# mx-mark/VideoTransformer-pytorch

Measured on AMD Instinct MI355X. Metric: clips/sec TimeSformer-B divided_space_time 8x3x224x224 fwd+bwd (whole job), higher is better.
Workload: dtype bf16

## Files before the change

__graft_entry__.py:

```python
import os
import subprocess
import sys

ROOT = os.path.dirname(os.path.abspath(__file__))
PKG = os.path.join(ROOT, 'videotransformer-pytorch_amd')
for p in (ROOT, PKG):
    if p not in sys.path:
        sys.path.insert(0, p)


def _build_oracle_c():
    src = os.path.join(ROOT, 'oracle', 'hog_ref.c')
    out_dir = os.path.join(ROOT, 'oracle', '_build')
    os.makedirs(out_dir, exist_ok=True)
    so = os.path.join(out_dir, 'libhogref.so')
    if not os.path.exists(so) or os.path.getmtime(so) < os.path.getmtime(src):
        subprocess.run(['gcc', '-O2', '-ffp-contract=off', '-shared', '-fPIC', '-o', so, src, '-lm'], check=True)
    return so


def ensure_built():
    so = os.path.join(PKG, 'libvtx.so')
    hipcc = os.environ.get('HIPCC', '/opt/rocm/bin/hipcc')
    if os.path.exists(so) and not os.path.exists(hipcc):
        return so
    sys.path.insert(0, os.path.join(PKG, 'csrc'))
    import build as vtx_build
    return vtx_build.build(verbose=False)


def build():
    sys.path.insert(0, os.path.join(PKG, 'csrc'))
    import build as vtx_build
    vtx_build.build(force=False, verbose=True)
    _build_oracle_c()
    import vtx
    lib = vtx.load()
    assert lib.vtx_version() >= 100
    import transformer, video_transformer
    print('libvtx', lib.vtx_version(), 'symbols bound:', len(vtx._lib.SIGNATURES))
    assert vtx._lib.load_ragged().vtx_ragged_version() >= 100
    print('libvtx_ragged', vtx._lib.load_ragged().vtx_ragged_version(), 'symbols bound:', len(vtx._lib.RAGGED_SIGNATURES))
    assert vtx._lib.load_dropout().vtx_dropout_version() >= 100
    print('libvtx_dropout', vtx._lib.load_dropout().vtx_dropout_version(), 'symbols bound:', len(vtx._lib.DROPOUT_SIGNATURES))


def smoke():
    import ctypes
    import numpy as np
    import torch
    ensure_built()
    import vtx
    import video_transformer as V
    from oracle import synth, vt_oracle as O, hog_oracle as H
    assert torch.cuda.is_available(), 'smoke() needs a GPU'
    buf = ctypes.create_string_buffer(16384)
    fails = vtx.load().vtx_selftest(buf, len(buf))
    print(buf.value.decode())
    assert fails == 0, 'instruction layout self-test failed'
    dev = torch.device('cuda:0')
    cfg = dict(num_frames=4, img_size=64, patch_size=16, embed_dims=128, num_heads=2, num_transformer_layers=2)
    m = V.TimeSformer(**cfg)
    sd = synth.synth_state_dict(synth.shapes_of(m), 3)
    m.load_state_dict(sd)
    m.to(dev).train()
    x = synth.synth_clip(2, 4, 3, 64, 64, seed=2)
    sdo = {k: v.clone().requires_grad_(True) for k, v in sd.items()}
    torch.manual_seed(1)
    yo = O.timesformer_forward(sdo, x, 4, heads=2, layers=2, training=True)
    yo.sum().backward()
    for prec, tol, gtol in (('fp32', 1e-3, 1e-3), ('bf16', 1.5e-2, 2e-2), ('bf16 + exact stream', 1.5e-2, 2e-2)):
        vtx.set_precision(prec.split()[0])
        vtx.set_stream('fp32+grad' if 'exact' in prec else 'bf16')
        m.zero_grad()
        torch.manual_seed(1)
        y = m(x.to(dev))
        y.sum().backward()
        torch.cuda.synchronize()
        e = (y.cpu() - yo.detach()).abs().max().item() / yo.abs().max().item()
        g = m.transformer_layers.layers[1].attentions[0].temporal_fc.weight.grad.cpu()
        go = sdo['transformer_layers.layers.1.attentions.0.temporal_fc.weight'].grad
        eg = (g - go).abs().max().item() / go.abs().max().item()
        print(f'smoke {prec}: out rel err {e:.2e}, temporal_fc grad rel err {eg:.2e}')
        assert e < tol and eg < gtol, (prec, e, eg)
    vtx.set_precision('auto')
    vtx.set_stream('bf16')
    frame = np.random.RandomState(5).randint(0, 256, (1, 224, 224, 3)).astype(np.uint8)
    f = vtx.ops.hog_fwd(torch.from_numpy(frame).to(dev)).cpu().numpy()[0]
    assert np.array_equal(f, H.extract_hog_features(frame[0])), 'HOG not bit-exact'
    rs = np.random.RandomState(6)
    clips = [torch.from_numpy(rs.randint(0, 256, shp).astype(np.uint8)).to(dev) for shp in ((5, 40, 56, 3), (3, 56, 40, 3))]
    ev, fr = vtx.aug.ClipEval(img_size=32), [[4, 0], [2, 1]]
    both = ev(clips, frames=fr)
    assert both.shape == (2, 2, 32, 32, 3) and all(torch.equal(both[b], ev(clips[b][None], frames=[fr[b]])[0]) for b in range(2)), 'ragged views differ'
    print('smoke ok')


if __name__ == '__main__':
    build()
    if len(sys.argv) > 1 and sys.argv[1] == 'smoke':
        smoke()
```

include/vtx.h:

```cpp
#ifndef VTX_H_
#define VTX_H_

#include <stddef.h>
#include <stdint.h>

#ifdef __cplusplus
extern "C" {
#endif

#define VTX_OK 0
#define VTX_EINVAL (-1)
#define VTX_EALIGN (-2)
#define VTX_ELAUNCH (-3)
#define VTX_EWS (-4)

#define VTX_F32 0
#define VTX_BF16 1
#define VTX_BF16_X32 3

typedef struct {
  int grp;
  int skip;
  int base;
  const int* tab;
} vtx_rowmap;

int vtx_version(void);
const char* vtx_last_error_string(void);
int vtx_set_option(const char* name, const char* value);

int vtx_layernorm_fwd(int dtype, int rows, int D, const void* x, long ldx, vtx_rowmap xmap,
                      const float* gamma, const float* beta, float eps,
                      void* y, long ldy, vtx_rowmap ymap, float* mean, float* rstd, void* stream);
int vtx_layernorm_acc_fwd(int rows, int D, const float* xs, const void* d, long lds, vtx_rowmap smap, float* xo, long ldo,
                          vtx_rowmap omap, const float* gamma, const float* beta, float eps, void* y, long ldy, vtx_rowmap ymap,
                          float* mean, float* rstd, void* stream);
size_t vtx_layernorm_bwd_workspace(int rows, int D);
int vtx_layernorm_bwd(int dtype, int rows, int D, const void* dy, long lddy, vtx_rowmap dymap,
                      const void* x, long ldx, vtx_rowmap xmap, const float* mean, const float* rstd,
                      const float* gamma, const void* dres, void* dx, long lddx,
                      float* dgamma, float* dbeta, void* workspace, size_t ws_bytes, void* stream);
int vtx_layernorm_bwd_g32(int rows, int D, const void* dy, long lddy, vtx_rowmap dymap, const float* x, long ldx, vtx_rowmap xmap,
                          const float* mean, const float* rstd, const float* gamma, const float* dres32, float* dx32,
                          void* dx, long lddx, float* dgamma, float* dbeta, void* workspace, size_t ws_bytes, void* stream);

typedef struct {
  int dtype;
  int M, N, K;
  const void* A; long lda; vtx_rowmap amap;
  const void* B; long ldb;
  void* C; long ldc; vtx_rowmap cmap;
  const float* bias;
  int act;
  void* C2; long ldc2;
  const void* dgelu_in; long ld_dgelu;
  int dgelu_kind;
  const float* row_scale;
  int rs_d1, rs_m1, rs_d2, rs_m2;
  const void* R; long ldr; vtx_rowmap rmap; int r_period;
  int split_row; void* Csplit; long ldsplit;
  void* workspace; size_t ws_bytes;
} vtx_gemm_desc;
size_t vtx_gemm_nt_workspace(void);
int vtx_gemm_nt(const vtx_gemm_desc* d, void* stream);

typedef struct {
  int dtype;
  int M, N1, N2;
  const void* A; long lda; vtx_rowmap amap;
  const void* B; long ldb; vtx_rowmap bmap;
  float* C; long ldc; int accumulate;
  void* workspace; size_t ws_bytes;
  float* colsum; int colsum_accumulate;
} vtx_gemm_tn_desc;
size_t vtx_gemm_tn_workspace(int M, int N1, int N2);
int vtx_gemm_tn(const vtx_gemm_tn_desc* d, void* stream);

typedef struct {
  int N1, N2, K;
  const float* A; long a_rs, a_ks;
  const float* B; long b_ks, b_cs;
  float alpha;
  float* C; long ldc; int accumulate;
  const float* u; const float* v;
  const float* x; float* y;
  float alpha_y; const float* z; float beta_z; int y_accumulate;
} vtx_wprod_desc;
int vtx_wprod(const vtx_wprod_desc* d, void* stream);

size_t vtx_colsum_workspace(int M, int N);
int vtx_colsum(int dtype, int M, int N, const void* A, long lda, vtx_rowmap amap,
               float* out, int accumulate, void* workspace, size_t ws_bytes, void* stream);

#define VTX_ATTN_CONTIG 0
#define VTX_ATTN_SPACE 1
#define VTX_ATTN_TIME_CLS 2
#define VTX_ATTN_SPACE_NOCLS 3
typedef struct {
  int dtype, mode;
  int S, L, H, hd;
  int B, T, P;
  const void* qkv; long ld_qkv;
  void* out; long ld_out;
  float* lse;
  float* probs;
  float scale;
} vtx_attn_desc;
int vtx_attn_fwd(const vtx_attn_desc* d, void* stream);

typedef struct {
  vtx_attn_desc f;
  const void* dout; long ld_dout;
  void* dqkv; long ld_dqkv;
  void* dqkv_cls;
  float* delta;
} vtx_attn_bwd_desc;
int vtx_attn_bwd(const vtx_attn_bwd_desc* d, void* stream);

int vtx_cls_mean_fwd(int dtype, int B, int T, int D, const void* a_cls, long lda,
                     const void* x, void* out, long ld_tok, long rows_per_clip, void* stream);
int vtx_fact_glue_fwd(int dtype, int B, int T, int P, int D, const void* x, const float* time_embed, void* h, void* stream);
int vtx_fact_glue_bwd(int dtype, int B, int T, int P, int D, const void* dh, void* dx, float* d_time_embed, int accumulate,
                      void* stream);
int vtx_space_grad_prep(int dtype, int B, int T, int P, int D, const void* dout, long ld,
                        const float* s, void* da, long ldda, void* stream);
int vtx_cls_qkv_reduce(int dtype, int B, int T, int W, const void* dqkv_cls, long ldc,
                       void* dqkv, long ld, long rows_per_clip, void* stream);
int vtx_row_scale_copy(int dtype, int rows, int D, const void* src, long lds, vtx_rowmap smap,
                       void* dst, long ldd, vtx_rowmap dmap, const float* s,
                       int rs_d1, int rs_m1, int rs_d2, int rs_m2, void* stream);
int vtx_dropped_rows_fix(int dtype, long M, int D, int group_rows, const float* s, const void* x, long ldx,
                         vtx_rowmap xmap, const float* bias, void* out, long ldo, vtx_rowmap omap, void* zero,
                         long ldz, void* stream);
int vtx_dropped_rows_colsum(int dtype, long M, int D, int group_rows, const float* s, const void* src, long lds,
                            vtx_rowmap smap, float* part, int nparts, void* stream);
int vtx_reduce_rows(int in_dtype, int nj, int ni, int D, const void* in, long ld, long base,
                    long si, long sj, float* out, long ldo, float scale, int accumulate, void* stream);
int vtx_gelu_grad_mul(int dtype, size_t n, const void* dy, const void* h, void* out, void* stream);
int vtx_cast_transpose(int dtype, int R, int C, const float* W, void* Wc, void* WcT, void* stream);
typedef struct {
  const float* src;
  void* dst_c;
  void* dst_t;
  int rows, cols;
} vtx_ct_tensor;
int vtx_mt_cast_transpose(int dtype, const vtx_ct_tensor* tab, const int* tile_start, int n_tensors, int n_tiles, void* stream);
int vtx_cast_from_f32(int dtype, size_t n, const float* src, void* dst, void* stream);
int vtx_cast_to_f32(int dtype, size_t n, const void* src, float* dst, void* stream);

int vtx_patch_rows(int dtype, int B, int T, int C, int H, int W, int ps, int ts,
                   const float* clip, void* rows, long ldr, int frame_major, void* stream);
int vtx_patch_rows_u8(int dtype, int B, int T, int H, int W, int ps, int ts,
                      const unsigned char* clip, const float* host_mean3, const float* host_std3,
                      void* rows, long ldr, int frame_major, void* stream);
int vtx_embed_table(int dtype, int P, int T, int D, const float* bias, const float* pos,
                    const float* time_embed, const float* cls, void* E, void* cls_row,
                    int frame_major, void* stream);

size_t vtx_hog_table_bytes(void);
int vtx_hog_build_table(double* host_table);
int vtx_hog_fwd(const uint8_t* frames, int F, int H, int W, const double* table, size_t table_bytes,
                double* out, int32_t* bins, void* stream);

int vtx_maskfeat_blend_fwd(int dtype, int B, int Tq, int Hq, int Wq, int C, int g,
                           const void* x, const uint8_t* mask, const float* mask_token,
                           void* out, void* stream);
int vtx_maskfeat_blend_bwd(int dtype, int B, int Tq, int Hq, int Wq, int C, int g,
                           const void* dy, const uint8_t* mask, void* dx, float* dtoken,
                           void* stream);
int vtx_maskfeat_loss_fwd(int dtype, int B, int Tq, int ts, int g, int Cf, const void* pred, long ldp,
                          const double* target, const uint8_t* cmask, double* loss_out, void* stream);
int vtx_maskfeat_loss_bwd(int dtype, int B, int Tq, int ts, int g, int Cf, const void* pred, long ldp,
                          const double* target, const uint8_t* cmask, const double* loss_out,
                          float gloss, void* dpred, long lddp, void* stream);

typedef struct { int dtype, B, T, H, W, heads, hd, sh, sw; } vtx_pool_desc;
int vtx_pool_conv_ln_fwd(const vtx_pool_desc* d, const void* x, const float* w, const float* gamma, const float* beta,
                         float eps, void* pre, void* y, float* mean, float* rstd, void* stream);
size_t vtx_pool_conv_ln_bwd_workspace(const vtx_pool_desc* d);
int vtx_pool_conv_ln_bwd(const vtx_pool_desc* d, const void* dy, const void* x, const void* pre, const float* mean,
                         const float* rstd, const float* w, const float* gamma, void* dpre, void* dx, float* dw,
                         float* dgamma, float* dbeta, void* workspace, size_t ws_bytes, void* stream);
int vtx_maxpool_skip_fwd(int dtype, int B, int T, int H, int W, int C, const void* x, void* y, uint8_t* arg, void* stream);
int vtx_maxpool_skip_bwd(int dtype, int B, int T, int H, int W, int C, const void* dy, const uint8_t* arg, void* dx, void* stream);
int vtx_pos_encoding_fwd(int dtype, int B, int T, int HW, int C, const void* x, const float* cls, const float* pos_class,
                         const float* spatial, const float* temporal, void* out, void* stream);
int vtx_im2col3d(int dtype, int B, int T, int C, int H, int W, const int* k3, const int* s3, const int* p3, int Kp,
                 const float* clip, void* rows, void* stream);
typedef struct {
  int dtype, B, Lq, Lk, heads, hd;
  float scale;
  const void* q; const void* k; const void* v;
  void* out; float* lse;
} vtx_xattn_desc;
int vtx_xattn_fwd(const vtx_xattn_desc* d, void* stream);
size_t vtx_xattn_bwd_workspace(const vtx_xattn_desc* d);
int vtx_xattn_bwd(const vtx_xattn_desc* d, const void* dout, float* delta, void* dq, void* dk, void* dv, void* workspace,
                  size_t ws_bytes, void* stream);

int vtx_mixup_batch(float* x, int B, long per_clip, float lam, float one_minus_lam, void* stream);
int vtx_cutmix_batch(float* x, int B, int planes, int H, int W, int yl, int yh, int xl, int xh, void* stream);
int vtx_mixup_target(const long* labels, int B, int C, float on_value, float off_value, float lam, float one_minus_lam,
                     float* out, void* stream);
int vtx_softmax_xent_fwd(const float* logits, const float* soft_targets, const long* labels, int B, int C, float* loss_rows,
                         float* lse, float* loss_mean, void* stream);
int vtx_softmax_xent_bwd(const float* logits, const float* soft_targets, const long* labels, const float* lse, int B, int C,
                         float grad_scale, const float* grad_loss, const float* count, float* dlogits, void* stream);
int vtx_topk_correct(const float* scores, const long* labels, int B, int C, int k, int* correct, void* stream);

typedef struct {
  void* p;
  const void* g;
  void* s1;
  void* s2;
  long n;
  float lr, wd;
} vtx_mt_tensor;
int vtx_mt_chunks(long numel);
int vtx_mt_grad_norms(const vtx_mt_tensor* tab, const int* chunk_start, int n_tensors, int n_chunks,
                      float* partial, float* norms, void* stream);
int vtx_mt_sgd_step(const vtx_mt_tensor* tab, const int* chunk_start, int n_tensors, int n_chunks, const float* norms,
                    float clip, float momentum, int nesterov, int first_step, void* stream);
int vtx_mt_adamw_step(const vtx_mt_tensor* tab, const int* chunk_start, int n_tensors, int n_chunks, const float* norms,
                      float clip, float beta1, float beta2, float eps, int step, void* stream);


int vtx_selftest(char* report, size_t report_bytes);

#ifdef __cplusplus
}
#endif
#endif
```

videotransformer-pytorch_amd/csrc/api.hip:

```cpp
#include <limits.h>
#include <stdarg.h>
#include <stdlib.h>
#include <string.h>
#include <string>
#include <vector>
#include "common.h"

namespace vtx {

static thread_local char g_err[512] = "";

void set_error(const char* fmt, ...) {
  va_list ap;
  va_start(ap, fmt);
  vsnprintf(g_err, sizeof(g_err), fmt, ap);
  va_end(ap);
}

int check_launch(const char* what) {
  hipError_t e = hipGetLastError();
  if (e != hipSuccess) {
    set_error("%s: launch failed: %s", what, hipGetErrorString(e));
    return VTX_ELAUNCH;
  }
  return VTX_OK;
}

static const char* const kNtNames[] = {"auto", "pp256", "dma2", "ring128x3", "ring128x4k32", "ring256x3", "ring256x3k32", "ring256x4k32"};
static const char* const kAttnF32Names[] = {"valu", "mfma"};
static const char* const kTnNames[] = {"auto", "pp256", "ring", "dma2", "w4"};

enum OptKind { OPT_FLAG, OPT_INT, OPT_CLAMP, OPT_ENUM, OPT_ADDR };
struct OptRow { const char* id[2]; OptKind kind; int Options::*field; int lo, hi, mult; const char* const* names; };
#define VTX_ENUM(names) 0, (int)(sizeof(names) / sizeof(*names)) - 1, 1, names
static const OptRow kOptions[] = {
    {{"VTX_GEMM_NT", "gemm_nt"}, OPT_ENUM, &Options::gemm_nt, VTX_ENUM(kNtNames)},
    {{"VTX_GEMM_TN", "gemm_tn"}, OPT_ENUM, &Options::gemm_tn, VTX_ENUM(kTnNames)},
    {{"VTX_GEMM_NODMA", "gemm_nodma"}, OPT_FLAG, &Options::gemm_nodma},
    {{"VTX_TN_SAFE", "tn_safe"}, OPT_FLAG, &Options::tn_safe},
    {{"VTX_TN_CUS", "tn_cus"}, OPT_INT, &Options::tn_cus, 32, 1024, 1},
    {{"VTX_ATTN_VALU", "attn_valu"}, OPT_FLAG, &Options::attn_valu},
    {{"VTX_ATTN_LONG", "attn_long"}, OPT_FLAG, &Options::attn_long},
    {{"VTX_ATTN_F32", "attn_f32"}, OPT_ENUM, &Options::attn_f32, VTX_ENUM(kAttnF32Names)},
    {{"VTX_ATTN_HW_FWD", "attn_hw_fwd"}, OPT_INT, &Options::attn_hw_fwd, 0, INT_MAX, 1},
    {{"VTX_ATTN_HW_BWD", "attn_hw_bwd"}, OPT_INT, &Options::attn_hw_bwd, 0, INT_MAX, 1},
    {{"VTX_ATTN_FUSED", "attn_fused"}, OPT_CLAMP, &Options::attn_fused, 0, 2},
    {{"VTX_ATTN_FWD_STREAM", "attn_fwd_stream"}, OPT_FLAG, &Options::attn_fwd_stream},
    {{"VTX_ATTN_DKV", "attn_dkv"}, OPT_INT, &Options::attn_dkv, 0, 4, 1},
    {{"VTX_GEMM_PP_GRID", "pp_grid"}, OPT_INT, &Options::pp_grid, 8, 4096, 8},
    {{"VTX_GEMM_PP_CG", "pp_cg"}, OPT_INT, &Options::pp_cg, 0, INT_MAX, 1},
    {{"VTX_GEMM_PP_EPI", "pp_epi"}, OPT_INT, &Options::pp_epi, INT_MIN, INT_MAX, 1},
    {{"VTX_GEMM_PP_CONT", "pp_cont"}, OPT_FLAG, &Options::pp_cont},
    {{"VTX_LN_ROWS", "ln_rows"}, OPT_INT, &Options::ln_rows, 1, 4, 1},
    {{nullptr, "pp_trace"}, OPT_ADDR, nullptr}};
#undef VTX_ENUM

static int set_option(Options& o, const char* name, const char* value) {
  if (!name || !value) return VTX_EINVAL;
  for (const OptRow& r : kOptions) {
    if (strcmp(name, r.id[1]) != 0) continue;
    if (r.kind == OPT_ADDR) { o.pp_trace = strtoull(value, nullptr, 0); return VTX_OK; }
    int v = atoi(value);
    if (r.kind == OPT_ENUM)
      for (v = r.hi; v >= 0 && strcmp(value, r.names[v]) != 0;) --v;
    if (r.kind == OPT_FLAG) v = v != 0;
    if (r.kind == OPT_CLAMP) v = v < r.lo ? r.lo : v > r.hi ? r.hi : v;
    if ((r.kind == OPT_INT || r.kind == OPT_ENUM) && (v < r.lo || v > r.hi || v % r.mult)) return VTX_EINVAL;
    o.*r.field = v;
    return VTX_OK;
  }
  return VTX_EINVAL;
}

Options& options() {
  static Options o = [] {
    Options d;
    for (const OptRow& r : kOptions) {
      const char* v = r.id[0] ? getenv(r.id[0]) : nullptr;
      if (v && *v) set_option(d, r.id[1], v);
    }
    return d;
  }();
  return o;
}

__global__ void probe_mfma_bf16(const float* A, const float* B, float* D) {
  const int l = threadIdx.x;
  union { bf16x8 v; bf16raw s[8]; } a, b;
  for (int j = 0; j < 8; ++j) {
    a.s[j] = f2bf(A[(l & 31) * 16 + 8 * (l >> 5) + j]);
    b.s[j] = f2bf(B[(8 * (l >> 5) + j) * 32 + (l & 31)]);
  }
  f32x16 acc;
  for (int r = 0; r < 16; ++r) acc[r] = 0.f;
  acc = __builtin_amdgcn_mfma_f32_32x32x16_bf16(a.v, b.v, acc, 0, 0, 0);
  for (int r = 0; r < 16; ++r) D[((r & 3) + 8 * (r >> 2) + 4 * (l >> 5)) * 32 + (l & 31)] = acc[r];
}
__global__ void probe_mfma_f32(const float* A, const float* B, float* D) {
  const int l = threadIdx.x;
  f32x16 acc;
  for (int r = 0; r < 16; ++r) acc[r] = 0.f;
  acc = __builtin_amdgcn_mfma_f32_32x32x2f32(A[(l & 31) * 2 + (l >> 5)], B[(l >> 5) * 32 + (l & 31)], acc, 0, 0, 0);
  for (int r = 0; r < 16; ++r) D[((r & 3) + 8 * (r >> 2) + 4 * (l >> 5)) * 32 + (l & 31)] = acc[r];
}
__global__ void probe_tr(unsigned short* out) {
  __shared__ __attribute__((aligned(16))) unsigned short lds[16 * 160];
  const int l = threadIdx.x;
  for (int e = l; e < 16 * 160; e += 64) lds[e] = (unsigned short)e;
  __syncthreads();
  const int row = 8 * (l >> 5) + ((l & 15) >> 2), col = 16 * ((l >> 4) & 1) + 4 * (l & 3);
  s16x4 v = __builtin_amdgcn_ds_read_tr16_b64_v4i16((s16x4 __attribute__((address_space(3)))*)(lds + row * 160 + col));
  for (int j = 0; j < 4; ++j) out[l * 4 + j] = (unsigned short)v[j];
}

int hog_selftest(int* bad_mag, int* bad_bin);

}

using namespace vtx;

extern "C" int vtx_version(void) { return 230; }

extern "C" int vtx_set_option(const char* name, const char* value) {
  const int rc = set_option(options(), name, value);
  if (rc) set_error("vtx_set_option: unknown option or bad value: %s=%s", name ? name : "(null)", value ? value : "(null)");
  return rc;
}
extern "C" const char* vtx_last_error_string(void) { return g_err; }

extern "C" int vtx_selftest(char* report, size_t report_bytes) {
  std::string rep;
  int fails = 0;
  auto say = [&](const char* fmt, ...) {
    char buf[512];
    va_list ap; va_start(ap, fmt); vsnprintf(buf, sizeof(buf), fmt, ap); va_end(ap);
    rep += buf;
  };
  float *dA = nullptr, *dB = nullptr, *dD = nullptr;
  unsigned short* dT = nullptr;
  if (hipMalloc(&dA, 32 * 16 * 4) != hipSuccess || hipMalloc(&dB, 16 * 32 * 4) != hipSuccess ||
      hipMalloc(&dD, 32 * 32 * 4) != hipSuccess || hipMalloc(&dT, 256 * 2) != hipSuccess) {
    set_error("selftest: hipMalloc failed");
    return VTX_ELAUNCH;
  }
  std::vector<float> A(32 * 16), B(16 * 32), D(32 * 32);
  unsigned s = 12345u;
  auto rnd = [&]() { s = s * 1664525u + 1013904223u; return (float)((int)((s >> 24) % 15) - 7); };
  for (auto& v : A) v = rnd();
  for (auto& v : B) v = rnd();
  hipMemcpy(dA, A.data(), A.size() * 4, hipMemcpyHostToDevice);
  hipMemcpy(dB, B.data(), B.size() * 4, hipMemcpyHostToDevice);
  hipLaunchKernelGGL(probe_mfma_bf16, dim3(1), dim3(64), 0, 0, dA, dB, dD);
  hipMemcpy(D.data(), dD, D.size() * 4, hipMemcpyDeviceToHost);
  int bad = 0;
  for (int i = 0; i < 32; ++i)
    for (int j = 0; j < 32; ++j) {
      float r = 0.f;
      for (int k = 0; k < 16; ++k) r += A[i * 16 + k] * B[k * 32 + j];
      if (r != D[i * 32 + j]) ++bad;
    }
  say("mfma_f32_32x32x16_bf16 layout: %s (%d/1024 mismatches)\n", bad ? "FAIL" : "ok", bad);
  fails += bad != 0;
  std::vector<float> A2(32 * 2), B2(2 * 32);
  for (auto& v : A2) v = rnd();
  for (auto& v : B2) v = rnd();
  hipMemcpy(dA, A2.data(), A2.size() * 4, hipMemcpyHostToDevice);
  hipMemcpy(dB, B2.data(), B2.size() * 4, hipMemcpyHostToDevice);
  hipLaunchKernelGGL(probe_mfma_f32, dim3(1), dim3(64), 0, 0, dA, dB, dD);
  hipMemcpy(D.data(), dD, D.size() * 4, hipMemcpyDeviceToHost);
  bad = 0;
  for (int i = 0; i < 32; ++i)
    for (int j = 0; j < 32; ++j) {
      const float r = A2[i * 2] * B2[j] + A2[i * 2 + 1] * B2[32 + j];
      if (r != D[i * 32 + j]) ++bad;
    }
  say("mfma_f32_32x32x2_f32 layout: %s (%d/1024 mismatches)\n", bad ? "FAIL" : "ok", bad);
  fails += bad != 0;
  std::vector<unsigned short> T(256);
  hipLaunchKernelGGL(probe_tr, dim3(1), dim3(64), 0, 0, dT);
  hipMemcpy(T.data(), dT, 512, hipMemcpyDeviceToHost);
  bad = 0;
  for (int l = 0; l < 64; ++l)
    for (int j = 0; j < 4; ++j) {
      const int want = (8 * (l >> 5) + j) * 160 + (l & 31);
      if (T[l * 4 + j] != want) ++bad;
    }
  say("ds_read_b64_tr_b16 gather: %s (%d/256 mismatches)\n", bad ? "FAIL" : "ok", bad);
  if (bad) {
    say("  observed (lane: row,col x4):\n");
    for (int l = 0; l < 64; ++l) {
      say("  %2d:", l);
      for (int j = 0; j < 4; ++j) say(" %d,%d", T[l * 4 + j] / 160, T[l * 4 + j] % 160);
      say("\n");
    }
  }
  fails += bad != 0;
  {
    int bad_mag = -1, bad_bin = -1;
    const int rc = hog_selftest(&bad_mag, &bad_bin);
    say("hog magnitudes, all 65536 gradient pairs vs host hypot: %s (%d mismatches)\n", (rc || bad_mag) ? "FAIL" : "ok", bad_mag);
    say("hog integer bin rule, all 261121 gradient pairs vs the float64 sign tests: %s (%d mismatches)\n", (rc || bad_bin) ? "FAIL" : "ok", bad_bin);
    fails += (rc != 0 || bad_mag != 0) + (rc != 0 || bad_bin != 0);
  }
  hipError_t e = hipDeviceSynchronize();
  if (e != hipSuccess) { say("device error: %s\n", hipGetErrorString(e)); ++fails; }
  hipFree(dA); hipFree(dB); hipFree(dD); hipFree(dT);
// ... 7 lines not shown
```

videotransformer-pytorch_amd/csrc/build.py:

```python
import os
import subprocess
import sys
from concurrent.futures import ThreadPoolExecutor

HERE = os.path.dirname(os.path.abspath(__file__))
PKG = os.path.dirname(HERE)
OUT = os.path.join(PKG, 'libvtx.so')
OBJ = os.path.join(HERE, '_obj')
HIPCC = os.environ.get('HIPCC', '/opt/rocm/bin/hipcc')
SOURCES = ['api.hip', 'ln.hip', 'gemm_nt.hip', 'gemm_tn.hip', 'attn.hip', 'attn_mfma.hip', 'attn_long.hip', 'attn_f32.hip', 'elementwise.hip', 'hog.hip', 'optim.hip', 'head.hip', 'mvit.hip', 'wprod.hip', 'xattn_mfma.hip']

SIDE = ['aug',
        'randaug',
        'views',
        'mix',
        'stem',
        'ragged',
        'dropout']
FLAGS = ['--offload-arch=gfx950', '-O3', '-std=c++17', '-fPIC', '-fno-gpu-rdc', '-Wno-unused-result', '-Wno-unused-value', '-Wno-inline-asm',
         '-Wno-cuda-compat']
EXTRA = {'hog.hip': ['-ffp-contract=off'],
         'aug.hip': ['-ffp-contract=off'],
         'randaug.hip': ['-ffp-contract=off'],
         'views.hip': ['-ffp-contract=off'],
         'mix.hip': ['-ffp-contract=off'],
         'stem.hip': ['-ffp-contract=off'],
         'ragged.hip': ['-ffp-contract=off'],
         'dropout.hip': ['-ffp-contract=off']}
LIBRARIES = [(OUT, SOURCES, [])] + [(os.path.join(PKG, f'libvtx_{n}.so'), [n + '.hip'], ['-Wl,-Bsymbolic']) for n in SIDE]


def _deps():
    inc = os.path.join(PKG, '..', 'include')
    hdrs = [os.path.join(d, f) for d in (HERE, inc) for f in os.listdir(d) if f.endswith('.h')]
    hdrs.append(os.path.abspath(__file__))
    return max(os.path.getmtime(h) for h in hdrs)


def _compile(src, force):
    obj = os.path.join(OBJ, src.replace('.hip', '.o'))
    spath = os.path.join(HERE, src)
    if (not force and os.path.exists(obj)
            and os.path.getmtime(obj) > max(os.path.getmtime(spath), _deps())):
        return obj, False
    cmd = [HIPCC] + FLAGS + EXTRA.get(src, []) + ['-c', spath, '-o', obj]
    r = subprocess.run(cmd, capture_output=True, text=True)
    if r.returncode != 0:
        raise RuntimeError(f'hipcc failed on {src}:\n{r.stdout}\n{r.stderr}')
    if r.stderr.strip():
        sys.stderr.write(r.stderr)
    return obj, True


def build_variant(name, defines):
    obj_dir = os.path.join(OBJ, name)
    os.makedirs(obj_dir, exist_ok=True)
    out = os.path.join(PKG, f'libvtx_{name}.so')

    def one(src):
        obj = os.path.join(obj_dir, src.replace('.hip', '.o'))
        cmd = ([HIPCC] + FLAGS + EXTRA.get(src, []) + [d if d.startswith('-') else '-D' + d for d in defines] +
               ['-c', os.path.join(HERE, src), '-o', obj])
        r = subprocess.run(cmd, capture_output=True, text=True)
        if r.returncode != 0:
            raise RuntimeError(f'hipcc failed on {src}:\n{r.stderr}')
        return obj
    with ThreadPoolExecutor(max_workers=min(8, len(SOURCES))) as ex:
        objs = list(ex.map(one, SOURCES))
    r = subprocess.run([HIPCC, '--offload-arch=gfx950', '-shared', '-fPIC', '-o', out] + objs, capture_output=True, text=True)
    if r.returncode != 0:
        raise RuntimeError(f'link failed:\n{r.stderr}')
    return out


def build(force=False, verbose=True):
    import fcntl
    os.makedirs(OBJ, exist_ok=True)
    with open(os.path.join(OBJ, '.lock'), 'w') as lock:
        fcntl.flock(lock, fcntl.LOCK_EX)
        try:
            return _build_locked(force, verbose)
        finally:
            fcntl.flock(lock, fcntl.LOCK_UN)


def _link(out, res, extra, verbose):
    if any(c for _, c in res) or not os.path.exists(out):
        cmd = [HIPCC, '--offload-arch=gfx950', '-shared', '-fPIC'] + extra + ['-o', out] + [o for o, _ in res]
        r = subprocess.run(cmd, capture_output=True, text=True)
        if r.returncode != 0:
            raise RuntimeError(f'link failed:\n{r.stdout}\n{r.stderr}')
        if verbose:
            print(f'built {out}')
    elif verbose:
        print(f'{out} up to date')


def _build_locked(force, verbose):
    every = [src for _, sources, _ in LIBRARIES for src in sources]
    with ThreadPoolExecutor(max_workers=min(8, len(every))) as ex:
        res = dict(zip(every, ex.map(lambda s: _compile(s, force), every)))
    for out, sources, flags in LIBRARIES:
        _link(out, [res[src] for src in sources], flags, verbose)
    return OUT


if __name__ == '__main__':
    if '--variant' in sys.argv:
        i = sys.argv.index('--variant')
        print(build_variant(sys.argv[i + 1], sys.argv[i + 2:]))
    else:
        build(force='--force' in sys.argv)
```

videotransformer-pytorch_amd/csrc/common.h:

```cpp
#pragma once
#include <hip/hip_runtime.h>
#include <stdint.h>
#include <atomic>
#include <stdio.h>
#include "../../include/vtx.h"

namespace vtx {

typedef __attribute__((ext_vector_type(8))) __bf16 bf16x8;
typedef __attribute__((ext_vector_type(4))) __bf16 bf16x4;
typedef __attribute__((ext_vector_type(4))) float f32x4;
typedef __attribute__((ext_vector_type(4))) unsigned int u32x4;
typedef __attribute__((ext_vector_type(16))) float f32x16;
typedef __attribute__((ext_vector_type(4))) short s16x4;
typedef unsigned short bf16raw;

__host__ __device__ inline float bf2f(bf16raw v) {
  union { uint32_t u; float f; } c; c.u = ((uint32_t)v) << 16; return c.f;
}
__host__ __device__ inline bf16raw f2bf(float f) {
#if defined(__HIP_DEVICE_COMPILE__)
  union { __bf16 b; bf16raw r; } c; c.b = (__bf16)f; return c.r;
#else
  union { uint32_t u; float f; } c; c.f = f;
  uint32_t u = c.u;
  if ((u & 0x7fffffffu) > 0x7f800000u) return (bf16raw)((u >> 16) | 0x40);
  u += 0x7fffu + ((u >> 16) & 1u);
  return (bf16raw)(u >> 16);
#endif
}

template <typename T> struct ET;
template <> struct ET<float> {
  static constexpr int VEC = 4;
  __device__ static inline float ld(const float* p) { return *p; }
  __device__ static inline void st(float* p, float v) { *p = v; }
  __device__ static inline void st4(float* p, const float (&v)[4]) { *reinterpret_cast<float4*>(p) = make_float4(v[0], v[1], v[2], v[3]); }
};
template <> struct ET<bf16raw> {
  static constexpr int VEC = 8;
  __device__ static inline float ld(const bf16raw* p) { return bf2f(*p); }
  __device__ static inline void st(bf16raw* p, float v) { *p = f2bf(v); }
  __device__ static inline void st4(bf16raw* p, const float (&v)[4]) {
    uint2 r;
    r.x = (uint32_t)f2bf(v[0]) | ((uint32_t)f2bf(v[1]) << 16);
    r.y = (uint32_t)f2bf(v[2]) | ((uint32_t)f2bf(v[3]) << 16);
    *reinterpret_cast<uint2*>(p) = r;
  }
};

__device__ inline void load8(const float* p, float (&v)[8]) {
  float4 a = *reinterpret_cast<const float4*>(p);
  float4 b = *reinterpret_cast<const float4*>(p + 4);
  v[0] = a.x; v[1] = a.y; v[2] = a.z; v[3] = a.w; v[4] = b.x; v[5] = b.y; v[6] = b.z; v[7] = b.w;
}
__device__ inline void load8(const bf16raw* p, float (&v)[8]) {
  uint4 r = *reinterpret_cast<const uint4*>(p);
  uint32_t w[4] = {r.x, r.y, r.z, r.w};
#pragma unroll
  for (int i = 0; i < 4; ++i) {
    v[2 * i] = __uint_as_float(w[i] << 16);
    v[2 * i + 1] = __uint_as_float(w[i] & 0xffff0000u);
  }
}
__device__ inline void store8(float* p, const float (&v)[8]) {
  *reinterpret_cast<float4*>(p) = make_float4(v[0], v[1], v[2], v[3]);
  *reinterpret_cast<float4*>(p + 4) = make_float4(v[4], v[5], v[6], v[7]);
}
__device__ inline void store8(bf16raw* p, const float (&v)[8]) {
  bf16x8 o;
#pragma unroll
  for (int i = 0; i < 8; ++i) o[i] = (__bf16)v[i];
  *reinterpret_cast<bf16x8*>(p) = o;
}

__device__ inline void store8_nt(bf16raw* p, const float (&v)[8]) {
  bf16x8 o;
#pragma unroll
  for (int i = 0; i < 8; ++i) o[i] = (__bf16)v[i];
  __builtin_nontemporal_store(o, reinterpret_cast<bf16x8*>(p));
}

__host__ __device__ inline long map_row(const vtx_rowmap& m, long r) {
#if defined(__HIP_DEVICE_COMPILE__)
  if (m.tab != nullptr) return (long)m.base + r + (long)m.tab[(unsigned)r / (unsigned)m.grp];
#endif
  const long q = (m.grp > 0) ? (long)((unsigned)r / (unsigned)m.grp) * (long)m.skip : 0;
  return (long)m.base + r + q;
}
inline vtx_rowmap ident_map() { vtx_rowmap m; m.grp = 0; m.skip = 0; m.base = 0; m.tab = nullptr; return m; }
inline bool closed_form(const vtx_rowmap& m) { return m.tab == nullptr; }

__device__ inline float wave_sum(float v) {
#pragma unroll
  for (int o = 32; o > 0; o >>= 1) v += __shfl_xor(v, o, 64);
  return v;
}
__device__ inline float wave_max(float v) {
#pragma unroll
  for (int o = 32; o > 0; o >>= 1) v = fmaxf(v, __shfl_xor(v, o, 64));
  return v;
}

__device__ inline void gelu_parts(float x, float& cdf, float& gauss) {
#pragma clang fp contract(off)
  const float u = fabsf(x) * 0.70710678118654752f;
  const float t = __builtin_amdgcn_rcpf(fmaf(0.3275911f, u, 1.0f));
  float p = fmaf(1.061405429f, t, -1.453152027f);
  p = fmaf(p, t, 1.421413741f);
  p = fmaf(p, t, -0.284496736f);
  p = fmaf(p, t, 0.254829592f);
  const float uu = u * u;
  const float e2 = uu * -1.4426950408889634f;
  const bool deep = e2 < -126.0f;
  gauss = __builtin_amdgcn_exp2f(e2 + (deep ? 64.0f : 0.0f)) * (deep ? 0x1p-64f : 1.0f);
  const float q = (0.5f * p) * t;
  const float half_tail = q * gauss;
  const float upper = 1.0f - half_tail;
  cdf = x >= 0.f ? upper : half_tail;
}
__device__ inline float gelu_erf(float x) {
#pragma clang fp contract(off)
  float cdf, g;
  gelu_parts(x, cdf, g);
  return x * cdf;
}
__device__ inline float gelu_erf_grad(float x) {
#pragma clang fp contract(off)
  float cdf, g;
  gelu_parts(x, cdf, g);
  const float xs = x * 0.3989422804014327f;
  return fmaf(xs, g, cdf);
}
__device__ inline void gelu_erf_both(float x, float& val, float& grad) {
#pragma clang fp contract(off)
  float cdf, g;
  gelu_parts(x, cdf, g);
  const float xs = x * 0.3989422804014327f;
  grad = fmaf(xs, g, cdf);
  val = x * cdf;
}

enum { NT_AUTO = 0, NT_PP256, NT_DMA2, NT_RING128X3, NT_RING128X4K32, NT_RING256X3, NT_RING256X3K32, NT_RING256X4K32,
       NT_REG, NT_F32 };
enum { TN_AUTO = 0, TN_PP256, TN_RING, TN_DMA2, TN_W4 };
struct Options {
  int gemm_nt = NT_AUTO;
  int gemm_tn = TN_AUTO;
  int gemm_nodma = 0;
  int tn_safe = 0;
  int tn_cus = 256;
  int attn_valu = 0;
  int attn_long = 1;
  int attn_f32 = 1;
  int attn_hw_fwd = 16;
  int attn_hw_bwd = 4;
  int attn_fused = 2;
  int attn_fwd_stream = 1;
  int attn_dkv = 3;
  int ln_rows = 3;
  int pp_grid = 256;
  int pp_cg = 0;
  int pp_epi = 0;
  int pp_cont = 1;
  unsigned long long pp_trace = 0;
};
Options& options();

void set_error(const char* fmt, ...);
int check_launch(const char* what);
int launch_reduce_partials(const float* part, int nslabs, long stride, long N, float* out, int accumulate, float scale,
                           hipStream_t st, float* out2 = nullptr, long split = 0, int accumulate2 = 0, int fold = 1,
                           long fold_stride = 0);
inline bool aligned16(const void* p) { return (reinterpret_cast<uintptr_t>(p) & 15u) == 0; }

#define VTX_REQUIRE(cond, code, ...)        \
  do {                                      \
    if (!(cond)) {                          \
      ::vtx::set_error(__VA_ARGS__);        \
      return (code);                        \
    }                                       \
  } while (0)

inline bool first_launch_on_device(std::atomic<unsigned long long>& seen) {
  int dev = 0;
  (void)hipGetDevice(&dev);
  const unsigned long long bit = 1ull << (dev & 63);
  return (seen.fetch_or(bit, std::memory_order_relaxed) & bit) == 0;
}

template <auto Kernel>
static void allow_lds(size_t needed, size_t cap = 160 * 1024) {
  static std::atomic<unsigned long long> seen{0};
  if (needed > 64 * 1024 && first_launch_on_device(seen))
    (void)hipFuncSetAttribute(reinterpret_cast<const void*>(Kernel), hipFuncAttributeMaxDynamicSharedMemorySize, (int)cap);
}

inline int device_cus() {
  static std::atomic<int> cached[64];
  int dev = 0;
  (void)hipGetDevice(&dev);
  int v = cached[dev & 63].load(std::memory_order_relaxed);
  if (v <= 0) {
    if (hipDeviceGetAttribute(&v, hipDeviceAttributeMultiprocessorCount, dev) != hipSuccess || v <= 0) v = 256;
    cached[dev & 63].store(v, std::memory_order_relaxed);
  }
  return v;
}
inline unsigned persistent_grid(int items) { const int cus = device_cus(); return (unsigned)(items < cus ? items : cus); }

inline hipStream_t as_stream(void* s) { return reinterpret_cast<hipStream_t>(s); }
inline int cdiv(long a, long b) { return (int)((a + b - 1) / b); }

}
```

videotransformer-pytorch_amd/csrc/elementwise.hip:

```cpp
#include "common.h"

namespace vtx {

template <typename T>
__global__ __launch_bounds__(256) void cast_transpose_kernel(int R, int C, const float* __restrict__ W,
                                                             T* __restrict__ Wc, T* __restrict__ WcT) {
  __shared__ float tile[64][65];
  const int r0 = blockIdx.y * 64, c0 = blockIdx.x * 64;
  const int tx = threadIdx.x & 63, ty = threadIdx.x >> 6;
  for (int rr = ty; rr < 64; rr += 4) {
    const int r = r0 + rr, c = c0 + tx;
    float v = 0.f;
    if (r < R && c < C) {
      v = W[(long)r * C + c];
      if (Wc) ET<T>::st(Wc + (long)r * C + c, v);
    }
    tile[rr][tx] = v;
  }
  if (!WcT) return;
  __syncthreads();
  for (int cc = ty; cc < 64; cc += 4) {
    const int c = c0 + cc, r = r0 + tx;
    if (r < R && c < C) ET<T>::st(WcT + (long)c * R + r, tile[tx][cc]);
  }
// ... 270 lines not shown
    const int b = (int)r;
    const float* src = clip + ((((long)b * Tn + (tq * ts + kt)) * C + c) * H + (ph * ps + kh)) * W + pw * ps;
    const int p = ph * gw + pw;
    const long row = frame_major ? ((long)b * Tq + tq) * P + p : ((long)b * P + p) * Tq + tq;
    T* dst = rows + row * ldr + ((long)(c * ts + kt) * ps + kh) * ps;
    if (vec8) {
      for (int kw = 0; kw < ps; kw += 8) {
        float v[8];
        load8(src + kw, v);
        store8(dst + kw, v);
      }
    } else {
      for (int kw = 0; kw < ps; kw += 4) {
        const float4 v = *reinterpret_cast<const float4*>(src + kw);
        ET<T>::st(dst + kw, v.x); ET<T>::st(dst + kw + 1, v.y); ET<T>::st(dst + kw + 2, v.z); ET<T>::st(dst + kw + 3, v.w);
      }
    }
  }
}

template <typename T>
__global__ void patch_rows_u8_kernel(int B, int Tn, int H, int W, int ps, int ts, const uint8_t* __restrict__ clip,
                                     float m0, float m1, float m2, float s0, float s1, float s2,
                                     T* __restrict__ rows, long ldr, int frame_major) {
#pragma clang fp contract(off)
  const int gh = H / ps, gw = W / ps, P = gh * gw, Tq = Tn / ts;
  const long total = (long)B * Tq * P * ts * ps;
  const float mean[3] = {m0, m1, m2}, sd[3] = {s0, s1, s2};
  for (long idx = (long)blockIdx.x * blockDim.x + threadIdx.x; idx < total; idx += (long)gridDim.x * blockDim.x) {
    long r = idx;
    const int pw = (int)(r % gw); r /= gw;
    const int kh = (int)(r % ps); r /= ps;
    const int kt = (int)(r % ts); r /= ts;
    const int ph = (int)(r % gh); r /= gh;
    const int tq = (int)(r % Tq); r /= Tq;
    const int b = (int)r;
    const uint8_t* src = clip + ((((long)b * Tn + (tq * ts + kt)) * H + (ph * ps + kh)) * W + pw * ps) * 3;
    const int p = ph * gw + pw;
    const long row = frame_major ? ((long)b * Tq + tq) * P + p : ((long)b * P + p) * Tq + tq;
    T* dst = rows + row * ldr + ((long)kt * ps + kh) * ps;
    for (int kw = 0; kw < ps; kw += 4) {
      const uint32_t w0 = *reinterpret_cast<const uint32_t*>(src + kw * 3);
      const uint32_t w1 = *reinterpret_cast<const uint32_t*>(src + kw * 3 + 4);
      const uint32_t w2 = *reinterpret_cast<const uint32_t*>(src + kw * 3 + 8);
      const uint32_t by[12] = {w0 & 255, (w0 >> 8) & 255, (w0 >> 16) & 255, w0 >> 24, w1 & 255, (w1 >> 8) & 255,
                               (w1 >> 16) & 255, w1 >> 24, w2 & 255, (w2 >> 8) & 255, (w2 >> 16) & 255, w2 >> 24};
#pragma unroll
      for (int c = 0; c < 3; ++c)
#pragma unroll
        for (int j = 0; j < 4; ++j) {
          const float x = (float)by[3 * j + c] / 255.0f;
          ET<T>::st(dst + (long)c * ts * ps * ps + kw + j, (x - mean[c]) / sd[c]);
        }
    }
  }
}

template <typename T>
__global__ void embed_table_kernel(int P, int Tn, int D, const float* __restrict__ bias, const float* __restrict__ pos,
                                   const float* __restrict__ time_embed, const float* __restrict__ cls,
                                   T* __restrict__ E, T* __restrict__ cls_row, int frame_major) {
  const long total = ((long)P * Tn + 1) * D;
  for (long idx = (long)blockIdx.x * blockDim.x + threadIdx.x; idx < total; idx += (long)gridDim.x * blockDim.x) {
    const long row = idx / D;
    const int d = (int)(idx - row * D);
    if (row == (long)P * Tn) {
      if (cls_row) ET<T>::st(cls_row + d, cls[d] + pos[d]);
      continue;
    }
    int p, t;
    if (frame_major) { t = (int)(row / P); p = (int)(row - (long)t * P); }
    else { p = (int)(row / Tn); t = (int)(row - (long)p * Tn); }
    float v = pos[(long)(1 + p) * D + d];
    if (bias) v += bias[d];
    if (time_embed) v += time_embed[(long)t * D + d];
    ET<T>::st(E + row * D + d, v);
  }
}

static inline int grid_for(long work, int block, int cap = 4096) {
  long g = (work + block - 1) / block;
  return (int)(g > cap ? cap : (g < 1 ? 1 : g));
}


template <typename T>
__global__ __launch_bounds__(256) void dropped_rows_fix_kernel(long M, int D, int group_rows, const float* __restrict__ s,
                                                               const T* __restrict__ x, long ldx, vtx_rowmap xmap,
                                                               const float* __restrict__ bias, T* __restrict__ out, long ldo,
                                                               vtx_rowmap omap, T* __restrict__ zero, long ldz) {
  const long g = (long)blockIdx.x * 4 + (threadIdx.x >> 6);
  const long m0 = g * group_rows;
  if (m0 >= M || s[g] != 0.f) return;
  const int lane = threadIdx.x & 63;
  const float z8[8] = {0, 0, 0, 0, 0, 0, 0, 0};
  for (int r = 0; r < group_rows && m0 + r < M; ++r) {
    const long m = m0 + r;
    for (int c = lane * 8; c < D; c += 512) {
      if (out) {
        float v[8] = {0, 0, 0, 0, 0, 0, 0, 0}, b[8];
        if (x != nullptr) load8(x + map_row(xmap, m) * ldx + c, v);
        load8(bias + c, b);
#pragma unroll
        for (int j = 0; j < 8; ++j) v[j] += b[j];
        store8(out + map_row(omap, m) * ldo + c, v);
      }
      if (zero) store8(zero + m * ldz + c, z8);
    }
  }
}

template <typename T>
__global__ __launch_bounds__(256) void dropped_rows_colsum_kernel(long M, int D, int group_rows, const float* __restrict__ s,
                                                                  const T* __restrict__ src, long lds_, vtx_rowmap smap,
                                                                  float* __restrict__ part, long n_groups) {
  __shared__ float red[8][128 + 4];
  __shared__ float flag[256];
  const int cl = threadIdx.x & 31, rl = threadIdx.x >> 5;
  const int c = blockIdx.x * 128 + cl * 4;
  const long per = (n_groups + gridDim.y - 1) / gridDim.y;
  const long g0 = (long)blockIdx.y * per, g1 = g0 + per < n_groups ? g0 + per : n_groups;
  float a[4] = {0, 0, 0, 0};
  for (long gb = g0; gb < g1; gb += 256) {
    __syncthreads();
    flag[threadIdx.x] = gb + threadIdx.x < g1 ? s[gb + threadIdx.x] : 1.f;
    __syncthreads();
    const int n = g1 - gb < 256 ? (int)(g1 - gb) : 256;
    for (int i = 0; i < n; ++i) {
      if (flag[i] != 0.f) continue;
      if (c < D)
        for (int r = rl; r < group_rows; r += 8) {
          const long m = (gb + i) * group_rows + r;
          if (m >= M) break;
          const T* p = src + map_row(smap, m) * lds_ + c;
#pragma unroll
          for (int e = 0; e < 4; ++e) a[e] += ET<T>::ld(p + e);
        }
    }
  }
#pragma unroll
  for (int e = 0; e < 4; ++e) red[rl][cl * 4 + e] = a[e];
  __syncthreads();
  if (rl == 0 && c < D) {
#pragma unroll
    for (int e = 0; e < 4; ++e) {
      float t = 0.f;
#pragma unroll
      for (int i = 0; i < 8; ++i) t += red[i][cl * 4 + e];
      part[(long)blockIdx.y * D + c + e] = t;
    }
  }
}

}

using namespace vtx;

#define DISPATCH_T(dtype, CALL_F32, CALL_BF16, name)              \
  if ((dtype) == VTX_F32) { CALL_F32; }                           \
  else if ((dtype) == VTX_BF16) { CALL_BF16; }                    \
  else VTX_REQUIRE(false, VTX_EINVAL, name ": bad dtype %d", (int)(dtype))

template <typename T>
__global__ __launch_bounds__(256) void gelu_grad_mul_kernel(size_t n8, const T* __restrict__ dy, const T* __restrict__ h, T* __restrict__ out) {
  for (size_t i = (size_t)blockIdx.x * 256 + threadIdx.x; i < n8; i += (size_t)gridDim.x * 256) {
    float a[8], b[8];
    load8(dy + i * 8, a);
    load8(h + i * 8, b);
#pragma unroll
    for (int j = 0; j < 8; ++j) a[j] *= gelu_erf_grad(b[j]);
    store8(out + i * 8, a);
  }
}

extern "C" int vtx_gelu_grad_mul(int dtype, size_t n, const void* dy, const void* h, void* out, void* stream) {
  VTX_REQUIRE(n % 8 == 0 && dy && h && out && aligned16(dy) && aligned16(h) && aligned16(out), VTX_EINVAL,
              "gelu_grad_mul: n must be a multiple of 8 and the pointers 16-byte aligned");
  if (n == 0) return VTX_OK;
  const size_t n8 = n / 8;
  const int grid = (int)((n8 + 255) / 256 > 16384 ? 16384 : (n8 + 255) / 256);
  hipStream_t st = as_stream(stream);
  if (dtype == VTX_F32)
    hipLaunchKernelGGL(gelu_grad_mul_kernel<float>, dim3(grid), dim3(256), 0, st, n8, (const float*)dy, (const float*)h, (float*)out);
  else if (dtype == VTX_BF16)
    hipLaunchKernelGGL(gelu_grad_mul_kernel<bf16raw>, dim3(grid), dim3(256), 0, st, n8, (const bf16raw*)dy, (const bf16raw*)h, (bf16raw*)out);
  else
    VTX_REQUIRE(false, VTX_EINVAL, "gelu_grad_mul: bad dtype %d", dtype);
  return check_launch("gelu_grad_mul");
}

extern "C" int vtx_cast_transpose(int dtype, int R, int C, const float* W, void* Wc, void* WcT, void* stream) {
  VTX_REQUIRE(R > 0 && C > 0 && W && (Wc || WcT), VTX_EINVAL, "cast_transpose: bad arguments");
  dim3 grid(cdiv(C, 64), cdiv(R, 64)), block(256);
  hipStream_t st = as_stream(stream);
  DISPATCH_T(dtype,
             hipLaunchKernelGGL(cast_transpose_kernel<float>, grid, block, 0, st, R, C, W, (float*)Wc, (float*)WcT),
             hipLaunchKernelGGL(cast_transpose_kernel<bf16raw>, grid, block, 0, st, R, C, W, (bf16raw*)Wc, (bf16raw*)WcT),
             "cast_transpose");
  return check_launch("cast_transpose");
}

extern "C" int vtx_mt_cast_transpose(int dtype, const vtx_ct_tensor* tab, const int* tile_start, int n_tensors, int n_tiles,
                                     void* stream) {
  VTX_REQUIRE(tab && tile_start && n_tensors > 0 && n_tiles >= 0, VTX_EINVAL, "mt_cast_transpose: bad arguments");
  if (n_tiles == 0) return VTX_OK;
  hipStream_t st = as_stream(stream);
  DISPATCH_T(dtype,
             hipLaunchKernelGGL(mt_cast_transpose_kernel<float>, dim3(n_tiles), dim3(256), 0, st, tab, tile_start, n_tensors),
             hipLaunchKernelGGL(mt_cast_transpose_kernel<bf16raw>, dim3(n_tiles), dim3(256), 0, st, tab, tile_start, n_tensors),
             "mt_cast_transpose");
  return check_launch("mt_cast_transpose");
}

extern "C" int vtx_cast_from_f32(int dtype, size_t n, const float* src, void* dst, void* stream) {
  VTX_REQUIRE(src && dst, VTX_EINVAL, "cast_from_f32: null pointer");
  if (n == 0) return VTX_OK;
  dim3 grid(grid_for((long)n, 256)), block(256);
  hipStream_t st = as_stream(stream);
  DISPATCH_T(dtype, hipLaunchKernelGGL(cast_from_f32_kernel<float>, grid, block, 0, st, n, src, (float*)dst),
             hipLaunchKernelGGL(cast_from_f32_kernel<bf16raw>, grid, block, 0, st, n, src, (bf16raw*)dst), "cast_from_f32");
  return check_launch("cast_from_f32");
}

extern "C" int vtx_cast_to_f32(int dtype, size_t n, const void* src, float* dst, void* stream) {
  VTX_REQUIRE(src && dst, VTX_EINVAL, "cast_to_f32: null pointer");
  if (n == 0) return VTX_OK;
  dim3 grid(grid_for((long)n, 256)), block(256);
  hipStream_t st = as_stream(stream);
  DISPATCH_T(dtype, hipLaunchKernelGGL(cast_to_f32_kernel<float>, grid, block, 0, st, n, (const float*)src, dst),
             hipLaunchKernelGGL(cast_to_f32_kernel<bf16raw>, grid, block, 0, st, n, (const bf16raw*)src, dst), "cast_to_f32");
  return check_launch("cast_to_f32");
}

extern "C" int vtx_cls_mean_fwd(int dtype, int B, int T, int D, const void* a_cls, long lda, const void* x, void* out,
                                long ld_tok, long rows_per_clip, void* stream) {
  VTX_REQUIRE(B > 0 && T > 0 && D > 0 && D % 8 == 0 && a_cls && out, VTX_EINVAL, "cls_mean_fwd: bad arguments");
  dim3 grid(cdiv((long)B * D / 8, 256)), block(256);
  hipStream_t st = as_stream(stream);
  DISPATCH_T(dtype,
             hipLaunchKernelGGL(cls_mean_fwd_kernel<float>, grid, block, 0, st, B, T, D, (const float*)a_cls, lda, (const float*)x, (float*)out, ld_tok, rows_per_clip),
             hipLaunchKernelGGL(cls_mean_fwd_kernel<bf16raw>, grid, block, 0, st, B, T, D, (const bf16raw*)a_cls, lda, (const bf16raw*)x, (bf16raw*)out, ld_tok, rows_per_clip),
             "cls_mean_fwd");
  return check_launch("cls_mean_fwd");
}

extern "C" int vtx_fact_glue_fwd(int dtype, int B, int T, int P, int D, const void* x, const float* time_embed, void* h, void* stream) {
  VTX_REQUIRE(B > 0 && T > 0 && P > 0 && D > 0 && D % 8 == 0 && D <= 1024 && x && time_embed && h, VTX_EINVAL, "fact_glue_fwd: bad arguments");
  VTX_REQUIRE(aligned16(x) && aligned16(h), VTX_EALIGN, "fact_glue_fwd: 16-byte alignment required");
  dim3 grid(B * (1 + T)), block(256);
  hipStream_t st = as_stream(stream);
  DISPATCH_T(dtype,
             hipLaunchKernelGGL(fact_glue_fwd_kernel<float>, grid, block, 0, st, B, T, P, D, (const float*)x, time_embed, (float*)h),
             hipLaunchKernelGGL(fact_glue_fwd_kernel<bf16raw>, grid, block, 0, st, B, T, P, D, (const bf16raw*)x, time_embed, (bf16raw*)h),
             "fact_glue_fwd");
  return check_launch("fact_glue_fwd");
}

extern "C" int vtx_fact_glue_bwd(int dtype, int B, int T, int P, int D, const void* dh, void* dx, float* d_time_embed, int accumulate,
                                 void* stream) {
  VTX_REQUIRE(B > 0 && T > 0 && P > 0 && D > 0 && D % 8 == 0 && dh && dx, VTX_EINVAL, "fact_glue_bwd: bad arguments");
  VTX_REQUIRE(aligned16(dh) && aligned16(dx), VTX_EALIGN, "fact_glue_bwd: 16-byte alignment required");
  const long total = (long)B * T * (1 + P) * (D / 8);
  dim3 grid(grid_for(total, 256)), block(256);
  hipStream_t st = as_stream(stream);
  DISPATCH_T(dtype,
             hipLaunchKernelGGL(fact_glue_bwd_kernel<float>, grid, block, 0, st, B, T, P, D, (const float*)dh, (float*)dx),
             hipLaunchKernelGGL(fact_glue_bwd_kernel<bf16raw>, grid, block, 0, st, B, T, P, D, (const bf16raw*)dh, (bf16raw*)dx),
             "fact_glue_bwd");
  int rc = check_launch("fact_glue_bwd");
  if (rc || !d_time_embed) return rc;
  dim3 g2(cdiv((long)(1 + T) * D, 256));
  DISPATCH_T(dtype,
             hipLaunchKernelGGL(fact_glue_de_kernel<float>, g2, block, 0, st, B, T, D, (const float*)dh, d_time_embed, accumulate),
             hipLaunchKernelGGL(fact_glue_de_kernel<bf16raw>, g2, block, 0, st, B, T, D, (const bf16raw*)dh, d_time_embed, accumulate),
             "fact_glue_de");
  return check_launch("fact_glue_de");
}

extern "C" int vtx_space_grad_prep(int dtype, int B, int T, int P, int D, const void* dout, long ld, const float* s,
                                   void* da, long ldda, void* stream) {
  const bool seq_major = P < 0;
  if (seq_major) P = -P;
  VTX_REQUIRE(B > 0 && T > 0 && P > 0 && D % 8 == 0 && dout && da, VTX_EINVAL, "space_grad_prep: bad arguments");
  const long work = ((long)B * P * T + (long)B * T) * (D / 8);
  dim3 grid(grid_for(work, 256)), block(256);
  hipStream_t st = as_stream(stream);
  if (seq_major) {
    DISPATCH_T(dtype,
               hipLaunchKernelGGL((space_grad_prep_kernel<float, true>), grid, block, 0, st, B, T, P, D, (const float*)dout, ld, s, (float*)da, ldda),
               hipLaunchKernelGGL((space_grad_prep_kernel<bf16raw, true>), grid, block, 0, st, B, T, P, D, (const bf16raw*)dout, ld, s, (bf16raw*)da, ldda),
               "space_grad_prep");
  } else {
    DISPATCH_T(dtype,
               hipLaunchKernelGGL((space_grad_prep_kernel<float, false>), grid, block, 0, st, B, T, P, D, (const float*)dout, ld, s, (float*)da, ldda),
               hipLaunchKernelGGL((space_grad_prep_kernel<bf16raw, false>), grid, block, 0, st, B, T, P, D, (const bf16raw*)dout, ld, s, (bf16raw*)da, ldda),
               "space_grad_prep");
  }
  return check_launch("space_grad_prep");
}

extern "C" int vtx_cls_qkv_reduce(int dtype, int B, int T, int W, const void* dqkv_cls, long ldc, void* dqkv, long ld,
                                  long rows_per_clip, void* stream) {
  VTX_REQUIRE(B > 0 && T > 0 && W % 8 == 0 && dqkv_cls && dqkv, VTX_EINVAL, "cls_qkv_reduce: bad arguments");
  dim3 grid(cdiv((long)B * W / 8, 256)), block(256);
  hipStream_t st = as_stream(stream);
  DISPATCH_T(dtype,
             hipLaunchKernelGGL(cls_qkv_reduce_kernel<float>, grid, block, 0, st, B, T, W, (const float*)dqkv_cls, ldc, (float*)dqkv, ld, rows_per_clip),
             hipLaunchKernelGGL(cls_qkv_reduce_kernel<bf16raw>, grid, block, 0, st, B, T, W, (const bf16raw*)dqkv_cls, ldc, (bf16raw*)dqkv, ld, rows_per_clip),
             "cls_qkv_reduce");
  return check_launch("cls_qkv_reduce");
}

extern "C" int vtx_row_scale_copy(int dtype, int rows, int D, const void* src, long lds, vtx_rowmap smap, void* dst,
                                  long ldd, vtx_rowmap dmap, const float* s, int rs_d1, int rs_m1, int rs_d2, int rs_m2,
                                  void* stream) {
  VTX_REQUIRE(rows > 0 && D > 0 && D % 8 == 0 && src && dst, VTX_EINVAL, "row_scale_copy: bad arguments");
  VTX_REQUIRE(!s || (rs_d1 > 0 && rs_d2 > 0), VTX_EINVAL, "row_scale_copy: divisors must be > 0");
  dim3 grid(grid_for((long)rows * (D / 8), 256)), block(256);
  hipStream_t st = as_stream(stream);
  DISPATCH_T(dtype,
             hipLaunchKernelGGL(row_scale_copy_kernel<float>, grid, block, 0, st, rows, D, (const float*)src, lds, smap, (float*)dst, ldd, dmap, s, rs_d1, rs_m1, rs_d2, rs_m2),
             hipLaunchKernelGGL(row_scale_copy_kernel<bf16raw>, grid, block, 0, st, rows, D, (const bf16raw*)src, lds, smap, (bf16raw*)dst, ldd, dmap, s, rs_d1, rs_m1, rs_d2, rs_m2),
             "row_scale_copy");
  return check_launch("row_scale_copy");
}

extern "C" int vtx_dropped_rows_fix(int dtype, long M, int D, int group_rows, const float* s, const void* x, long ldx,
                                    vtx_rowmap xmap, const float* bias, void* out, long ldo, vtx_rowmap omap, void* zero,
                                    long ldz, void* stream) {
  VTX_REQUIRE(M > 0 && D > 0 && D % 8 == 0 && group_rows > 0 && s, VTX_EINVAL, "dropped_rows_fix: bad arguments");
  VTX_REQUIRE(out || zero, VTX_EINVAL, "dropped_rows_fix: nothing to do");
  VTX_REQUIRE(!out || bias, VTX_EINVAL, "dropped_rows_fix: out needs the bias");
  const long groups = (M + group_rows - 1) / group_rows;
  dim3 grid((unsigned)((groups + 3) / 4)), block(256);
  hipStream_t st = as_stream(stream);
  DISPATCH_T(dtype,
             hipLaunchKernelGGL(dropped_rows_fix_kernel<float>, grid, block, 0, st, M, D, group_rows, s, (const float*)x, ldx, xmap, bias, (float*)out, ldo, omap, (float*)zero, ldz),
             hipLaunchKernelGGL(dropped_rows_fix_kernel<bf16raw>, grid, block, 0, st, M, D, group_rows, s, (const bf16raw*)x, ldx, xmap, bias, (bf16raw*)out, ldo, omap, (bf16raw*)zero, ldz),
             "dropped_rows_fix");
  return check_launch("dropped_rows_fix");
}

extern "C" int vtx_dropped_rows_colsum(int dtype, long M, int D, int group_rows, const float* s, const void* src, long lds,
                                       vtx_rowmap smap, float* part, int nparts, void* stream) {
  VTX_REQUIRE(M > 0 && D > 0 && D % 4 == 0 && group_rows > 0 && s && src && part && nparts > 0 && nparts <= 65535, VTX_EINVAL,
              "dropped_rows_colsum: bad arguments");
  const long groups = (M + group_rows - 1) / group_rows;
  dim3 grid((unsigned)((D + 127) / 128), (unsigned)nparts), block(256);
  hipStream_t st = as_stream(stream);
  DISPATCH_T(dtype,
             hipLaunchKernelGGL(dropped_rows_colsum_kernel<float>, grid, block, 0, st, M, D, group_rows, s, (const float*)src, lds, smap, part, groups),
             hipLaunchKernelGGL(dropped_rows_colsum_kernel<bf16raw>, grid, block, 0, st, M, D, group_rows, s, (const bf16raw*)src, lds, smap, part, groups),
             "dropped_rows_colsum");
  return check_launch("dropped_rows_colsum");
}

extern "C" int vtx_reduce_rows(int in_dtype, int nj, int ni, int D, const void* in, long ld, long base, long si, long sj,
                               float* out, long ldo, float scale, int accumulate, void* stream) {
  VTX_REQUIRE(nj > 0 && ni > 0 && D > 0 && D % 4 == 0 && in && out, VTX_EINVAL, "reduce_rows: bad arguments");
  dim3 grid(cdiv(D, 128), nj), block(256);
  hipStream_t st = as_stream(stream);
  DISPATCH_T(in_dtype,
             hipLaunchKernelGGL(reduce_rows_kernel<float>, grid, block, 0, st, ni, D, (const float*)in, ld, base, si, sj, out, ldo, scale, accumulate),
             hipLaunchKernelGGL(reduce_rows_kernel<bf16raw>, grid, block, 0, st, ni, D, (const bf16raw*)in, ld, base, si, sj, out, ldo, scale, accumulate),
             "reduce_rows");
  return check_launch("reduce_rows");
}

extern "C" int vtx_patch_rows(int dtype, int B, int T, int C, int H, int W, int ps, int ts, const float* clip, void* rows,
                              long ldr, int frame_major, void* stream) {
  VTX_REQUIRE(B > 0 && T > 0 && C > 0 && ps > 0 && ts > 0 && clip && rows, VTX_EINVAL, "patch_rows: bad arguments");
  VTX_REQUIRE(H % ps == 0 && W % ps == 0 && T % ts == 0 && ps % 4 == 0 && W % 4 == 0, VTX_EINVAL,
              "patch_rows: H,W must be multiples of ps (itself a multiple of 4), T of ts");
  const long work = (long)B * (T / ts) * (H / ps) * (W / ps) * C * ts * ps;
  dim3 grid(grid_for(work, 256, 16384)), block(256);
  hipStream_t st = as_stream(stream);
  DISPATCH_T(dtype,
             hipLaunchKernelGGL(patch_rows_kernel<float>, grid, block, 0, st, B, T, C, H, W, ps, ts, clip, (float*)rows, ldr, frame_major),
             hipLaunchKernelGGL(patch_rows_kernel<bf16raw>, grid, block, 0, st, B, T, C, H, W, ps, ts, clip, (bf16raw*)rows, ldr, frame_major),
             "patch_rows");
  return check_launch("patch_rows");
}

extern "C" int vtx_patch_rows_u8(int dtype, int B, int T, int H, int W, int ps, int ts, const unsigned char* clip,
                                 const float* mean3, const float* std3, void* rows, long ldr, int frame_major, void* stream) {
  VTX_REQUIRE(B > 0 && T > 0 && ps > 0 && ts > 0 && clip && rows && mean3 && std3, VTX_EINVAL, "patch_rows_u8: bad arguments");
  VTX_REQUIRE(H % ps == 0 && W % ps == 0 && T % ts == 0 && ps % 4 == 0, VTX_EINVAL,
              "patch_rows_u8: H,W must be multiples of ps (itself a multiple of 4), T of ts");
  VTX_REQUIRE((reinterpret_cast<uintptr_t>(clip) & 3u) == 0, VTX_EALIGN, "patch_rows_u8: clip must be 4-byte aligned");
  VTX_REQUIRE(std3[0] != 0.f && std3[1] != 0.f && std3[2] != 0.f, VTX_EINVAL, "patch_rows_u8: zero std");
  const long work = (long)B * (T / ts) * (H / ps) * (W / ps) * ts * ps;
  dim3 grid(grid_for(work, 256, 16384)), block(256);
  hipStream_t st = as_stream(stream);
  DISPATCH_T(dtype,
             hipLaunchKernelGGL(patch_rows_u8_kernel<float>, grid, block, 0, st, B, T, H, W, ps, ts, clip, mean3[0], mean3[1], mean3[2], std3[0], std3[1], std3[2], (float*)rows, ldr, frame_major),
             hipLaunchKernelGGL(patch_rows_u8_kernel<bf16raw>, grid, block, 0, st, B, T, H, W, ps, ts, clip, mean3[0], mean3[1], mean3[2], std3[0], std3[1], std3[2], (bf16raw*)rows, ldr, frame_major),
             "patch_rows_u8");
  return check_launch("patch_rows_u8");
}

extern "C" int vtx_embed_table(int dtype, int P, int T, int D, const float* bias, const float* pos, const float* time_embed,
                               const float* cls, void* E, void* cls_row, int frame_major, void* stream) {
  VTX_REQUIRE(P > 0 && T > 0 && D > 0 && pos && E, VTX_EINVAL, "embed_table: bad arguments");
  VTX_REQUIRE(!cls_row || cls, VTX_EINVAL, "embed_table: cls_row needs cls");
  dim3 grid(grid_for(((long)P * T + 1) * D, 256)), block(256);
  hipStream_t st = as_stream(stream);
  DISPATCH_T(dtype,
             hipLaunchKernelGGL(embed_table_kernel<float>, grid, block, 0, st, P, T, D, bias, pos, time_embed, cls, (float*)E, (float*)cls_row, frame_major),
             hipLaunchKernelGGL(embed_table_kernel<bf16raw>, grid, block, 0, st, P, T, D, bias, pos, time_embed, cls, (bf16raw*)E, (bf16raw*)cls_row, frame_major),
             "embed_table");
  return check_launch("embed_table");
}
```

videotransformer-pytorch_amd/csrc/wprod.hip:

```cpp
#include "common.h"

namespace vtx {

#ifndef VTX_WP_PAD_KB
#define VTX_WP_PAD_KB 0
#endif
#ifndef VTX_WP_NACC
#define VTX_WP_NACC 2
#endif
#ifndef VTX_WP_D
#define VTX_WP_D 4
#endif
constexpr int WP_T = 32, WP_THREADS = 256, WP_D = VTX_WP_D;

struct WprodParams {
  int N1, N2, K;
  const float* A; long a_rs, a_ks;
  const float* B; long b_ks, b_cs;
  float alpha;
  float* C; long ldc; int accumulate;
  const float* u; const float* v;
  const float* x; float* y; float alpha_y; const float* z; float beta_z; int y_accumulate;
  long long* trace;
};

#ifdef VTX_WP_TRACE
#define WP_STAMP(e_) if (p.trace != nullptr && lane == 0) { \
    long long* sl__ = p.trace + ((long)(blockIdx.y * gridDim.x + blockIdx.x) * 4 + h) * 8; \
    sl__[e_] = (long long)__builtin_amdgcn_s_memrealtime(); if ((e_) == 0 || (e_) == 3) sl__[(e_) == 0 ? 6 : 7] = (long long)__builtin_amdgcn_s_memtime(); }
#else
#define WP_STAMP(e_)
#endif

template <bool A_KCONT, bool B_KCONT, bool FULL, bool WITH_X>
__global__ __launch_bounds__(WP_THREADS) void wprod_kernel(WprodParams p) {
  __shared__ float red[3][16][64];
  __shared__ float yred[4][32];
  const int tid = threadIdx.x, lane = tid & 63;
  const int h = __builtin_amdgcn_readfirstlane(tid >> 6);
  const int li = lane & 31, kh = lane >> 5;
  WP_STAMP(0)
  const int i0 = blockIdx.y * WP_T, j0 = blockIdx.x * WP_T;
  const int row = i0 + li, col = j0 + li;
  const bool row_ok = row < p.N1, col_ok = col < p.N2;
  const bool with_y = WITH_X && blockIdx.x == 0;
  const int nb = (p.K + 7) >> 3;
  const int per = (((nb + 3) >> 2) + WP_D - 1) / WP_D * WP_D;
  const int b_lo = 0, b_hi = per;
  const float* const arow = p.A + (A_KCONT ? (long)(row_ok ? row : 0) * p.a_rs : (long)(row_ok ? row : 0));
  const float* const bcol = p.B + (B_KCONT ? (long)(col_ok ? col : 0) * p.b_cs : (long)(col_ok ? col : 0));

  const float* const xbase = WITH_X ? p.x : p.A;
  float a[WP_D][4], b[WP_D][4], xv[WP_D][4];
  auto load = [&](int blk, float (&va)[4], float (&vb)[4], float (&vx)[4]) {
    const int kk = (blk * 4 + h) * 8 + kh * 4;
    const int ks = kk < p.K ? kk : 0;
    if (A_KCONT) {
      const float4 t = *reinterpret_cast<const float4*>(arow + ks);
      va[0] = t.x; va[1] = t.y; va[2] = t.z; va[3] = t.w;
    } else {
#pragma unroll
      for (int s = 0; s < 4; ++s) va[s] = arow[(long)(ks + s) * p.a_ks];
    }
    if (B_KCONT) {
      const float4 t = *reinterpret_cast<const float4*>(bcol + ks);
      vb[0] = t.x; vb[1] = t.y; vb[2] = t.z; vb[3] = t.w;
    } else {
#pragma unroll
      for (int s = 0; s < 4; ++s) vb[s] = bcol[(long)(ks + s) * p.b_ks];
    }
    if constexpr (WITH_X) {
      const float4 t = *reinterpret_cast<const float4*>(xbase + ks);
      vx[0] = t.x; vx[1] = t.y; vx[2] = t.z; vx[3] = t.w;
    }
  };

  f32x16 accs[VTX_WP_NACC];
#pragma unroll
  for (int c = 0; c < VTX_WP_NACC; ++c)
#pragma unroll
    for (int r = 0; r < 16; ++r) accs[c][r] = 0.f;
  float yacc = 0.f;
#pragma unroll
  for (int d = 0; d < WP_D; ++d) { load(b_lo + d, a[d], b[d], xv[d]); __builtin_amdgcn_sched_barrier(0); }
  WP_STAMP(1)
  bool first_trip = true;
  for (int blk = b_lo; blk < b_hi; blk += WP_D) {
#pragma unroll
    for (int d = 0; d < WP_D; ++d) {
      const bool kok = FULL || ((blk + d) * 4 + h) * 8 + kh * 4 < p.K;
      const bool aok = FULL || (kok && row_ok), bok = FULL || (kok && col_ok);
#pragma unroll
      for (int s = 0; s < 4; ++s) {
        const float av = aok ? a[d][s] : 0.f, bv = bok ? b[d][s] : 0.f;
        accs[s % VTX_WP_NACC] = __builtin_amdgcn_mfma_f32_32x32x2f32(av, bv, accs[s % VTX_WP_NACC], 0, 0, 0);
        if constexpr (WITH_X) yacc = fmaf(av, xv[d][s], yacc);
      }
      load(blk + d + WP_D, a[d], b[d], xv[d]);
      __builtin_amdgcn_sched_barrier(0);
    }
#ifdef VTX_WP_TRACE
    if (first_trip) { WP_STAMP(2) first_trip = false; }
#endif
  }
  WP_STAMP(3)
  f32x16 acc = accs[0];
#pragma unroll
  for (int c = 1; c < VTX_WP_NACC; ++c)
#pragma unroll
    for (int r = 0; r < 16; ++r) acc[r] += accs[c][r];
  if (h > 0) {
#pragma unroll
    for (int r = 0; r < 16; ++r) red[h - 1][r][lane] = acc[r];
  }
  if (with_y) {
    const float other = __shfl_xor(yacc, 32, 64);
    if (kh == 0) yred[h][li] = yacc + other;
  }
  __syncthreads();
  WP_STAMP(4)
  if (h == 0) {
    const float vj = (p.u && col_ok) ? p.v[col] : 0.f;
#pragma unroll
    for (int r = 0; r < 16; ++r) {
      const int orow = i0 + (r & 3) + 8 * (r >> 2) + 4 * kh;
      if (orow < p.N1 && col_ok) {
        float val = p.alpha * (((acc[r] + red[0][r][lane]) + red[1][r][lane]) + red[2][r][lane]);
        if (p.u) val = fmaf(p.u[orow], vj, val);
        float* dst = p.C + (long)orow * p.ldc + col;
        if (p.accumulate) val += *dst;
        *dst = val;
      }
    }
    if (with_y && kh == 0 && row_ok) {
      float val = p.alpha_y * (((yred[0][li] + yred[1][li]) + yred[2][li]) + yred[3][li]);
      if (p.z) val = fmaf(p.beta_z, p.z[row], val);
      if (p.y_accumulate) val += p.y[row];
      p.y[row] = val;
    }
  }
  WP_STAMP(5)
}

}

using namespace vtx;

extern "C" int vtx_wprod(const vtx_wprod_desc* d, void* stream) {
  VTX_REQUIRE(d != nullptr, VTX_EINVAL, "wprod: null descriptor");
  VTX_REQUIRE(d->N1 > 0 && d->N2 > 0 && d->K > 0, VTX_EINVAL, "wprod: bad shape N1=%d N2=%d K=%d", d->N1, d->N2, d->K);
  VTX_REQUIRE(d->N1 % 4 == 0 && d->N2 % 4 == 0 && d->K % 4 == 0, VTX_EINVAL, "wprod: N1, N2, K must be multiples of 4");
  VTX_REQUIRE(d->A && d->B && d->C, VTX_EINVAL, "wprod: null operand");
  VTX_REQUIRE((d->a_rs == 1) != (d->a_ks == 1), VTX_EINVAL, "wprod: exactly one stride of A must be 1 (a_rs=%ld a_ks=%ld)",
              d->a_rs, d->a_ks);
  VTX_REQUIRE((d->b_ks == 1) != (d->b_cs == 1), VTX_EINVAL, "wprod: exactly one stride of B must be 1 (b_ks=%ld b_cs=%ld)",
              d->b_ks, d->b_cs);
  const long a_ld = d->a_ks == 1 ? d->a_rs : d->a_ks, b_ld = d->b_ks == 1 ? d->b_cs : d->b_ks;
  VTX_REQUIRE(aligned16(d->A) && aligned16(d->B) && a_ld % 4 == 0 && b_ld % 4 == 0 && (!d->x || aligned16(d->x)), VTX_EALIGN,
              "wprod: operands (and x) must be 16-byte aligned with leading dimensions that are multiples of 4");
  VTX_REQUIRE(d->ldc >= d->N2, VTX_EINVAL, "wprod: ldc=%ld < N2=%d", d->ldc, d->N2);
  VTX_REQUIRE((d->u == nullptr) == (d->v == nullptr), VTX_EINVAL, "wprod: the rank-1 term needs both u and v");
  VTX_REQUIRE((d->y == nullptr) == (d->x == nullptr), VTX_EINVAL, "wprod: the vector product needs both x and y");
  WprodParams p;
  p.N1 = d->N1; p.N2 = d->N2; p.K = d->K;
  p.A = d->A; p.a_rs = d->a_rs; p.a_ks = d->a_ks;
  p.B = d->B; p.b_ks = d->b_ks; p.b_cs = d->b_cs;
  p.alpha = d->alpha; p.C = d->C; p.ldc = d->ldc; p.accumulate = d->accumulate;
  p.u = d->u; p.v = d->v;
  p.trace = nullptr;
#ifdef VTX_WP_TRACE
  p.trace = reinterpret_cast<long long*>(options().pp_trace);
#endif
  p.x = d->x; p.y = d->y; p.alpha_y = d->alpha_y; p.z = d->z; p.beta_z = d->beta_z; p.y_accumulate = d->y_accumulate;
  const dim3 grid(cdiv(d->N2, WP_T), cdiv(d->N1, WP_T)), block(WP_THREADS);
  hipStream_t st = as_stream(stream);
  const bool ak = d->a_ks == 1, bk = d->b_ks == 1;
  const size_t pad = (size_t)VTX_WP_PAD_KB * 1024;
  const bool full = d->N1 % 32 == 0 && d->N2 % 32 == 0 && d->K % (32 * WP_D) == 0, wx = d->x != nullptr;
#define WP_LAUNCH(AK_, BK_)                                                                                          \
  {                                                                                                                  \
    if (full && wx) hipLaunchKernelGGL((wprod_kernel<AK_, BK_, true, true>), grid, block, pad, st, p);               \
    else if (full) hipLaunchKernelGGL((wprod_kernel<AK_, BK_, true, false>), grid, block, pad, st, p);               \
    else if (wx) hipLaunchKernelGGL((wprod_kernel<AK_, BK_, false, true>), grid, block, pad, st, p);                 \
    else hipLaunchKernelGGL((wprod_kernel<AK_, BK_, false, false>), grid, block, pad, st, p);                        \
  }
  if (ak && bk) WP_LAUNCH(true, true)
  else if (ak) WP_LAUNCH(true, false)
  else if (bk) WP_LAUNCH(false, true)
  else WP_LAUNCH(false, false)
#undef WP_LAUNCH
  return check_launch("wprod");
}
```

videotransformer-pytorch_amd/vtx/_lib.py:

```python
import ctypes as C
import os
from functools import partial

_HERE = os.path.dirname(os.path.abspath(__file__))
_PKG = os.path.dirname(_HERE)
LIB_PATH = os.environ.get('VTX_LIB', os.path.join(_PKG, 'libvtx.so'))

VTX_F32, VTX_BF16, VTX_BF16_X32 = 0, 1, 3
ATTN_CONTIG, ATTN_SPACE, ATTN_TIME_CLS, ATTN_SPACE_NOCLS = 0, 1, 2, 3
RESAMPLE_BILINEAR, RESAMPLE_BICUBIC = 0, 1
JIT_BRIGHTNESS, JIT_CONTRAST, JIT_SATURATION = 0, 1, 2


class RowMap(C.Structure):
    _fields_ = [('grp', C.c_int), ('skip', C.c_int), ('base', C.c_int), ('tab', C.c_void_p)]


IDENT = RowMap(0, 0, 0, None)


class GemmDesc(C.Structure):
    _fields_ = [
        ('dtype', C.c_int), ('M', C.c_int), ('N', C.c_int), ('K', C.c_int),
        ('A', C.c_void_p), ('lda', C.c_long), ('amap', RowMap),
        ('B', C.c_void_p), ('ldb', C.c_long),
        ('C', C.c_void_p), ('ldc', C.c_long), ('cmap', RowMap),
        ('bias', C.c_void_p),
        ('act', C.c_int), ('C2', C.c_void_p), ('ldc2', C.c_long),
        ('dgelu_in', C.c_void_p), ('ld_dgelu', C.c_long), ('dgelu_kind', C.c_int),
        ('row_scale', C.c_void_p),
        ('rs_d1', C.c_int), ('rs_m1', C.c_int), ('rs_d2', C.c_int), ('rs_m2', C.c_int),
        ('R', C.c_void_p), ('ldr', C.c_long), ('rmap', RowMap), ('r_period', C.c_int),
        ('split_row', C.c_int), ('Csplit', C.c_void_p), ('ldsplit', C.c_long),
        ('workspace', C.c_void_p), ('ws_bytes', C.c_size_t),
    ]


class GemmTnDesc(C.Structure):
    _fields_ = [
        ('dtype', C.c_int), ('M', C.c_int), ('N1', C.c_int), ('N2', C.c_int),
        ('A', C.c_void_p), ('lda', C.c_long), ('amap', RowMap),
        ('B', C.c_void_p), ('ldb', C.c_long), ('bmap', RowMap),
        ('C', C.c_void_p), ('ldc', C.c_long), ('accumulate', C.c_int),
        ('workspace', C.c_void_p), ('ws_bytes', C.c_size_t),
        ('colsum', C.c_void_p), ('colsum_accumulate', C.c_int),
    ]


class WprodDesc(C.Structure):
    _fields_ = [
        ('N1', C.c_int), ('N2', C.c_int), ('K', C.c_int),
        ('A', C.c_void_p), ('a_rs', C.c_long), ('a_ks', C.c_long),
        ('B', C.c_void_p), ('b_ks', C.c_long), ('b_cs', C.c_long),
        ('alpha', C.c_float),
        ('C', C.c_void_p), ('ldc', C.c_long), ('accumulate', C.c_int),
        ('u', C.c_void_p), ('v', C.c_void_p),
        ('x', C.c_void_p), ('y', C.c_void_p),
        ('alpha_y', C.c_float), ('z', C.c_void_p), ('beta_z', C.c_float), ('y_accumulate', C.c_int),
    ]


class CtTensor(C.Structure):
    _fields_ = [('src', C.c_void_p), ('dst_c', C.c_void_p), ('dst_t', C.c_void_p), ('rows', C.c_int), ('cols', C.c_int)]


class MtTensor(C.Structure):
    _fields_ = [('p', C.c_void_p), ('g', C.c_void_p), ('s1', C.c_void_p), ('s2', C.c_void_p), ('n', C.c_long),
                ('lr', C.c_float), ('wd', C.c_float)]


class PoolDesc(C.Structure):
    _fields_ = [(n, C.c_int) for n in ('dtype', 'B', 'T', 'H', 'W', 'heads', 'hd', 'sh', 'sw')]


class XAttnDesc(C.Structure):
    _fields_ = [('dtype', C.c_int), ('B', C.c_int), ('Lq', C.c_int), ('Lk', C.c_int), ('heads', C.c_int), ('hd', C.c_int),
                ('scale', C.c_float), ('q', C.c_void_p), ('k', C.c_void_p), ('v', C.c_void_p), ('out', C.c_void_p),
                ('lse', C.c_void_p)]


class AttnDesc(C.Structure):
    _fields_ = [
        ('dtype', C.c_int), ('mode', C.c_int),
        ('S', C.c_int), ('L', C.c_int), ('H', C.c_int), ('hd', C.c_int),
        ('B', C.c_int), ('T', C.c_int), ('P', C.c_int),
        ('qkv', C.c_void_p), ('ld_qkv', C.c_long),
        ('out', C.c_void_p), ('ld_out', C.c_long),
        ('lse', C.c_void_p), ('probs', C.c_void_p), ('scale', C.c_float),
    ]


class AttnBwdDesc(C.Structure):
    _fields_ = [
        ('f', AttnDesc),
        ('dout', C.c_void_p), ('ld_dout', C.c_long),
        ('dqkv', C.c_void_p), ('ld_dqkv', C.c_long),
        ('dqkv_cls', C.c_void_p), ('delta', C.c_void_p),
    ]


vp, ci, cl, cf, sz = C.c_void_p, C.c_int, C.c_long, C.c_float, C.c_size_t

SIGNATURES = {
    'vtx_version': (ci, []),
    'vtx_last_error_string': (C.c_char_p, []),
    'vtx_set_option': (ci, [C.c_char_p, C.c_char_p]),
    'vtx_layernorm_fwd': (ci, [ci, ci, ci, vp, cl, RowMap, vp, vp, cf, vp, cl, RowMap, vp, vp, vp]),
    'vtx_layernorm_acc_fwd': (ci, [ci, ci, vp, vp, cl, RowMap, vp, cl, RowMap, vp, vp, cf, vp, cl, RowMap, vp, vp, vp]),
    'vtx_layernorm_bwd_workspace': (sz, [ci, ci]),
    'vtx_layernorm_bwd': (ci, [ci, ci, ci, vp, cl, RowMap, vp, cl, RowMap, vp, vp, vp, vp, vp, cl,
                               vp, vp, vp, sz, vp]),
    'vtx_layernorm_bwd_g32': (ci, [ci, ci, vp, cl, RowMap, vp, cl, RowMap, vp, vp, vp, vp, vp, vp, cl, vp, vp, vp, sz, vp]),
    'vtx_gemm_nt_workspace': (sz, []),
    'vtx_gemm_nt': (ci, [C.POINTER(GemmDesc), vp]),
    'vtx_gemm_tn_workspace': (sz, [ci, ci, ci]),
    'vtx_gemm_tn': (ci, [C.POINTER(GemmTnDesc), vp]),
    'vtx_wprod': (ci, [C.POINTER(WprodDesc), vp]),
    'vtx_colsum_workspace': (sz, [ci, ci]),
    'vtx_colsum': (ci, [ci, ci, ci, vp, cl, RowMap, vp, ci, vp, sz, vp]),
    'vtx_attn_fwd': (ci, [C.POINTER(AttnDesc), vp]),
    'vtx_attn_bwd': (ci, [C.POINTER(AttnBwdDesc), vp]),
    'vtx_cls_mean_fwd': (ci, [ci, ci, ci, ci, vp, cl, vp, vp, cl, cl, vp]),
    'vtx_fact_glue_fwd': (ci, [ci, ci, ci, ci, ci, vp, vp, vp, vp]),
    'vtx_fact_glue_bwd': (ci, [ci, ci, ci, ci, ci, vp, vp, vp, ci, vp]),
    'vtx_space_grad_prep': (ci, [ci, ci, ci, ci, ci, vp, cl, vp, vp, cl, vp]),
    'vtx_cls_qkv_reduce': (ci, [ci, ci, ci, ci, vp, cl, vp, cl, cl, vp]),
    'vtx_dropped_rows_fix': (ci, [ci, cl, ci, ci, vp, vp, cl, RowMap, vp, vp, cl, RowMap, vp, cl, vp]),
    'vtx_dropped_rows_colsum': (ci, [ci, cl, ci, ci, vp, vp, cl, RowMap, vp, ci, vp]),
    'vtx_row_scale_copy': (ci, [ci, ci, ci, vp, cl, RowMap, vp, cl, RowMap, vp, ci, ci, ci, ci, vp]),
    'vtx_reduce_rows': (ci, [ci, ci, ci, ci, vp, cl, cl, cl, cl, vp, cl, cf, ci, vp]),
    'vtx_gelu_grad_mul': (ci, [ci, sz, vp, vp, vp, vp]),
    'vtx_cast_transpose': (ci, [ci, ci, ci, vp, vp, vp, vp]),
    'vtx_mt_cast_transpose': (ci, [ci, vp, vp, ci, ci, vp]),
    'vtx_cast_from_f32': (ci, [ci, sz, vp, vp, vp]),
    'vtx_cast_to_f32': (ci, [ci, sz, vp, vp, vp]),
    'vtx_patch_rows': (ci, [ci, ci, ci, ci, ci, ci, ci, ci, vp, vp, cl, ci, vp]),
    'vtx_patch_rows_u8': (ci, [ci, ci, ci, ci, ci, ci, ci, vp, C.POINTER(C.c_float), C.POINTER(C.c_float), vp, cl, ci, vp]),
    'vtx_embed_table': (ci, [ci, ci, ci, ci, vp, vp, vp, vp, vp, vp, ci, vp]),
    'vtx_hog_table_bytes': (sz, []),
    'vtx_hog_build_table': (ci, [vp]),
    'vtx_hog_fwd': (ci, [vp, ci, ci, ci, vp, sz, vp, vp, vp]),
    'vtx_maskfeat_blend_fwd': (ci, [ci, ci, ci, ci, ci, ci, ci, vp, vp, vp, vp, vp]),
    'vtx_maskfeat_blend_bwd': (ci, [ci, ci, ci, ci, ci, ci, ci, vp, vp, vp, vp, vp]),
    'vtx_maskfeat_loss_fwd': (ci, [ci, ci, ci, ci, ci, ci, vp, cl, vp, vp, vp, vp]),
    'vtx_maskfeat_loss_bwd': (ci, [ci, ci, ci, ci, ci, ci, vp, cl, vp, vp, vp, cf, vp, cl, vp]),
    'vtx_pool_conv_ln_fwd': (ci, [C.POINTER(PoolDesc), vp, vp, vp, vp, cf, vp, vp, vp, vp, vp]),
    'vtx_pool_conv_ln_bwd_workspace': (sz, [C.POINTER(PoolDesc)]),
    'vtx_pool_conv_ln_bwd': (ci, [C.POINTER(PoolDesc), vp, vp, vp, vp, vp, vp, vp, vp, vp, vp, vp, vp, vp, sz, vp]),
    'vtx_maxpool_skip_fwd': (ci, [ci, ci, ci, ci, ci, ci, vp, vp, vp, vp]),
    'vtx_maxpool_skip_bwd': (ci, [ci, ci, ci, ci, ci, ci, vp, vp, vp, vp]),
    'vtx_pos_encoding_fwd': (ci, [ci, ci, ci, ci, ci, vp, vp, vp, vp, vp, vp, vp]),
    'vtx_im2col3d': (ci, [ci, ci, ci, ci, ci, ci, C.POINTER(C.c_int), C.POINTER(C.c_int), C.POINTER(C.c_int), ci, vp, vp, vp]),
    'vtx_xattn_fwd': (ci, [C.POINTER(XAttnDesc), vp]),
    'vtx_xattn_bwd_workspace': (sz, [C.POINTER(XAttnDesc)]),
    'vtx_xattn_bwd': (ci, [C.POINTER(XAttnDesc), vp, vp, vp, vp, vp, vp, sz, vp]),
    'vtx_mixup_batch': (ci, [vp, ci, cl, cf, cf, vp]),
    'vtx_cutmix_batch': (ci, [vp, ci, ci, ci, ci, ci, ci, ci, ci, vp]),
    'vtx_mixup_target': (ci, [vp, ci, ci, cf, cf, cf, cf, vp, vp]),
    'vtx_softmax_xent_fwd': (ci, [vp, vp, vp, ci, ci, vp, vp, vp, vp]),
    'vtx_softmax_xent_bwd': (ci, [vp, vp, vp, vp, ci, ci, cf, vp, vp, vp, vp]),
    'vtx_topk_correct': (ci, [vp, vp, ci, ci, ci, vp, vp]),
    'vtx_mt_chunks': (ci, [cl]),
    'vtx_mt_grad_norms': (ci, [vp, vp, ci, ci, vp, vp, vp]),
    'vtx_mt_sgd_step': (ci, [vp, vp, ci, ci, vp, cf, cf, ci, ci, vp]),
    'vtx_mt_adamw_step': (ci, [vp, vp, ci, ci, vp, cf, cf, cf, cf, ci, vp]),
    'vtx_selftest': (ci, [C.c_char_p, sz]),
}

AUG_LIB_PATH = os.environ.get('VTX_AUG_LIB', os.path.join(_PKG, 'libvtx_aug.so'))
AUG_SIGNATURES = {
    'vtx_aug_version': (ci, []),
    'vtx_aug_last_error_string': (C.c_char_p, []),
    'vtx_resample_max_taps': (ci, [ci, ci, ci, ci]),
    'vtx_resample_build_table': (ci, [ci, ci, ci, ci, ci, ci, ci, ci, vp, vp, vp]),
    'vtx_clip_resample_u8': (ci, [ci, ci, ci, ci, ci, ci, vp, vp, vp, vp, vp, ci, vp, vp, vp, ci, vp]),
    'vtx_clip_jitter_workspace': (sz, [ci, ci]),
    'vtx_clip_jitter_u8': (ci, [ci, ci, ci, ci, vp, vp, vp, vp, sz, vp]),
}

RANDAUG_LIB_PATH = os.environ.get('VTX_RANDAUG_LIB', os.path.join(_PKG, 'libvtx_randaug.so'))
PW_NONE, PW_POSTERIZE, PW_SOLARIZE = 0, 1, 2
RANDAUG_SIGNATURES = {
    'vtx_randaug_version': (ci, []),
    'vtx_randaug_last_error_string': (C.c_char_p, []),
    'vtx_clip_warp_nearest_u8': (ci, [ci, ci, ci, ci, vp, vp, vp, vp, vp]),
    'vtx_clip_sharpness_u8': (ci, [ci, ci, ci, ci, vp, vp, vp, vp, vp]),
    'vtx_clip_pointwise_u8': (ci, [ci, ci, ci, ci, vp, vp, vp]),
    'vtx_clip_autocontrast_workspace': (sz, [ci, ci]),
    'vtx_clip_autocontrast_u8': (ci, [ci, ci, ci, ci, vp, vp, vp, sz, vp]),
    'vtx_clip_equalize_workspace': (sz, [ci, ci]),
    'vtx_clip_equalize_u8': (ci, [ci, ci, ci, ci, vp, vp, vp, sz, vp]),
}

VIEWS_LIB_PATH = os.environ.get('VTX_VIEWS_LIB', os.path.join(_PKG, 'libvtx_views.so'))
VIEWS_MAX = 8
VIEWS_SIGNATURES = {
    'vtx_views_version': (ci, []),
    'vtx_views_last_error_string': (C.c_char_p, []),
    'vtx_clip_views_u8': (ci, [ci, ci, ci, ci, ci, ci, ci, ci, ci, vp, vp, vp, vp, vp, vp, vp, ci, vp, vp, vp, ci, vp]),
}

MIX_LIB_PATH = os.environ.get('VTX_MIX_LIB', os.path.join(_PKG, 'libvtx_mix.so'))
MIX_SIGNATURES = {
    'vtx_mix_version': (ci, []),
    'vtx_mix_last_error_string': (C.c_char_p, []),
    'vtx_cutmix_batch_u8': (ci, [ci, ci, ci, ci, vp, ci, ci, ci, ci, vp]),
    'vtx_patch_rows_mix_u8': (ci, [ci, ci, ci, ci, ci, ci, ci, vp, C.POINTER(C.c_float), C.POINTER(C.c_float), cf, cf, vp, cl, ci, vp]),
}

STEM_LIB_PATH = os.environ.get('VTX_STEM_LIB', os.path.join(_PKG, 'libvtx_stem.so'))
STEM_SIGNATURES = {
    'vtx_stem_version': (ci, []),
    'vtx_stem_last_error_string': (C.c_char_p, []),
    'vtx_im2col3d_u8': (ci, [ci, ci, ci, ci, ci, C.POINTER(C.c_int), C.POINTER(C.c_int), C.POINTER(C.c_int), ci, vp,
                             C.POINTER(C.c_float), C.POINTER(C.c_float), vp, vp]),
    'vtx_hog_fwd_sel': (ci, [vp, ci, ci, ci, vp, ci, vp, sz, vp, vp]),
}

RAGGED_LIB_PATH = os.environ.get('VTX_RAGGED_LIB', os.path.join(_PKG, 'libvtx_ragged.so'))
RAGGED_SIGNATURES = {
    'vtx_ragged_version': (ci, []),
    'vtx_ragged_last_error_string': (C.c_char_p, []),
    'vtx_clips_views_u8': (ci, [ci, ci, ci, ci, ci, ci, vp, vp, vp, vp, vp, vp, vp, vp, ci, vp, vp, vp, ci, vp]),
}

DROPOUT_LIB_PATH = os.environ.get('VTX_DROPOUT_LIB', os.path.join(_PKG, 'libvtx_dropout.so'))
DROPOUT_SIGNATURES = {
    'vtx_dropout_version': (ci, []),
    'vtx_dropout_last_error_string': (C.c_char_p, []),
    'vtx_dropout_rows': (ci, [ci, ci, ci, vp, cl, RowMap, vp, cl, RowMap, vp, cl, RowMap, vp, ci, vp, ci, ci, ci, ci,
                              C.c_ulonglong, cf, C.c_ulonglong, C.c_uint, C.c_ulonglong, vp]),
}

_SIDE = {
    'aug': ('AUG_LIB_PATH', AUG_SIGNATURES),
    'randaug': ('RANDAUG_LIB_PATH', RANDAUG_SIGNATURES),
    'views': ('VIEWS_LIB_PATH', VIEWS_SIGNATURES),
    'mix': ('MIX_LIB_PATH', MIX_SIGNATURES),
    'stem': ('STEM_LIB_PATH', STEM_SIGNATURES),
    'ragged': ('RAGGED_LIB_PATH', RAGGED_SIGNATURES),
    'dropout': ('DROPOUT_LIB_PATH', DROPOUT_SIGNATURES),
}
_lib = None
_side = {}


class VtxError(RuntimeError):
    pass


def _bind(path, soname, signatures):
    if not os.path.isfile(path):
        raise VtxError(f'{soname} not found at {path}: build it with '
                       f'`python videotransformer-pytorch_amd/csrc/build.py` (there is no CPU/PyTorch fallback)')
    lib = C.CDLL(path)
    for name, (res, args) in signatures.items():
        try:
            fn = getattr(lib, name)
        except AttributeError as e:
            raise VtxError(f'{soname} does not export {name}') from e
        fn.restype = res
        fn.argtypes = args
    return lib


def _load_side(key):
    if key not in _side:
        path_name, signatures = _SIDE[key]
        _side[key] = _bind(globals()[path_name], f'libvtx_{key}.so', signatures)
    return _side[key]


def _side_check(key, rc, what=''):
    msg = getattr(_load_side(key), f'vtx_{key}_last_error_string')()
    raise VtxError(f'{what} failed (code {rc}): {msg.decode() if msg else "?"}')


def _side_call(key, name, *args):
    rc = getattr(_load_side(key), name)(*args)
    if rc != 0:
        _side_check(key, rc, name)


load_aug, aug_call = partial(_load_side, 'aug'), partial(_side_call, 'aug')
load_randaug, randaug_call = partial(_load_side, 'randaug'), partial(_side_call, 'randaug')
load_views, views_call = partial(_load_side, 'views'), partial(_side_call, 'views')
load_mix, mix_call = partial(_load_side, 'mix'), partial(_side_call, 'mix')
load_stem, stem_call = partial(_load_side, 'stem'), partial(_side_call, 'stem')
load_ragged, ragged_call = partial(_load_side, 'ragged'), partial(_side_call, 'ragged')
load_dropout, dropout_call = partial(_load_side, 'dropout'), partial(_side_call, 'dropout')
aug_check = partial(_side_check, 'aug')


def load():
    global _lib
    if _lib is None:
        _lib = _bind(LIB_PATH, 'libvtx.so', SIGNATURES)
    return _lib


def check(rc, what=''):
    if rc != 0:
        msg = load().vtx_last_error_string()
        raise VtxError(f'{what} failed (code {rc}): {msg.decode() if msg else "?"}')


def set_option(name, value):
    rc = load().vtx_set_option(str(name).encode(), str(value).encode())
    if rc != 0:
        check(rc, f'vtx_set_option({name}={value})')


_TRACE = os.environ.get('VTX_TRACE_CALLS', '0') == '1'


def call(name, *args):
    if _TRACE:
        import sys
        import torch
        sys.stderr.write(f'[vtx] {name}\n')
        sys.stderr.flush()
    rc = getattr(load(), name)(*args)
    if rc != 0:
        check(rc, name)
    if _TRACE:
        torch.cuda.synchronize()
```

videotransformer-pytorch_amd/vtx/functions.py:

```python
import collections
import functools
import weakref

import torch

from . import ops
from ._lib import IDENT, ATTN_CONTIG, ATTN_SPACE, ATTN_TIME_CLS, ATTN_SPACE_NOCLS

_wcache = {}


def weights(p, dtype, need_t=None):
    if need_t is None:
        need_t = torch.is_grad_enabled()
    key = (id(p), dtype)
    stamp = (p._version, p.data_ptr(), p.device)
    hit = _wcache.get(key)
    if hit is not None and hit[0]() is p and hit[1] == stamp and (hit[3] is not None or not need_t):
        return hit[2], hit[3]
    w2d = p.detach().reshape(p.shape[0], -1)
    wc, wt = ops.cast_transpose(w2d, dtype, want_c=True, want_t=need_t)
    if len(_wcache) > 4096:
        for k in [k for k, v in _wcache.items() if v[0]() is None]:
            del _wcache[k]
    _wcache[key] = (weakref.ref(p), stamp, wc, wt)
    return wc, wt


_restage_tables = {}


def restage_weights(params):
    groups = {}
    for p in params:
        for dtype in (torch.bfloat16, torch.float32):
            hit = _wcache.get((id(p), dtype))
            if hit is None or hit[0]() is not p or not p.is_cuda:
                continue
            wc, wt = hit[2], hit[3]
            if dtype == torch.float32:
                wc = None
            if wc is None and wt is None:
                continue
            if (p._version, p.data_ptr(), p.device) == hit[1]:
                continue
            groups.setdefault((dtype, p.device), []).append((p, hit, wc, wt))
    for (dtype, dev), ents in groups.items():
        key = (dtype, dev, tuple((p.data_ptr(), 0 if wc is None else wc.data_ptr(), 0 if wt is None else wt.data_ptr())
                                 for p, _, wc, wt in ents))
        tabs = _restage_tables.get((dtype, dev))
        if tabs is None or tabs[0] != key:
            tab_dev, starts_dev, n_tiles = ops.ct_table([(p.detach().reshape(p.shape[0], -1), wc, wt) for p, _, wc, wt in ents], dev)
            tabs = (key, tab_dev, starts_dev, n_tiles)
            _restage_tables[(dtype, dev)] = tabs
        ops.mt_cast_transpose(dtype, tabs[1], tabs[2], len(ents), tabs[3])
        for p, hit, wc, wt in ents:
            _wcache[(id(p), dtype)] = (hit[0], (p._version, p.data_ptr(), p.device), hit[2], hit[3])
            for t in (wc, wt):
                if t is not None:
                    t.view(-1)[:0].zero_()


_mcache = {}
_merge_tfc = True


def set_merge_temporal_fc(on):
    global _merge_tfc
    _merge_tfc = bool(on)


def merged_proj(proj_w, proj_b, tfc_w, tfc_b, dtype, need_t, c=1.0):
    ps = (proj_w, proj_b, tfc_w, tfc_b)
    key = (id(proj_w), id(tfc_w), dtype)
    stamp = tuple((p._version, p.data_ptr(), p.device) for p in ps) + (float(c),)
    hit = _mcache.get(key)
    if hit is not None and all(r() is p for r, p in zip(hit[0], ps)) and hit[1] == stamp and (hit[3] is not None or not need_t):
        return hit[2], hit[3], hit[4]
    wc32, bias = ops.wprod(tfc_w.detach(), proj_w.detach(), x=proj_b.detach(), z=tfc_b.detach(), beta_z=1.0 / float(c))
    wc, wt = ops.cast_transpose(wc32, dtype, want_c=True, want_t=need_t)
    if len(_mcache) > 1024:
        for k in [k for k, v in _mcache.items() if any(r() is None for r in v[0])]:
            del _mcache[k]
    _mcache[key] = (tuple(weakref.ref(p) for p in ps), stamp, wc, wt, bias)
    return wc, wt, bias


def clear_weight_cache():
    _wcache.clear()
    _mcache.clear()
    _restage_tables.clear()


_direct = False


def set_direct_grads(on):
    global _direct
    _direct = bool(on)


def direct_grads_enabled():
    return _direct


def _sink(p):
    if not _direct or p is None:
        return None
    g = p.grad
    if g is None or g.dtype != torch.float32 or not g.is_cuda or not g.is_contiguous() or g.shape != p.shape:
        return None
    return g


_firing = False


def _fire(*params):
    global _firing
    _firing = True
    try:
        for p in params:
            hooks = getattr(p, '_post_accumulate_grad_hooks', None)
            if hooks:
                for h in list(hooks.values()):
                    h(p)
    finally:
        _firing = False


def firing():
    return _firing


def _weight_grads(params, A, Bm, M, N1, N2, bias=True, amap=IDENT):
    if params is not None:
        gw, gb = _sink(params[0]), _sink(params[1])
        if gw is not None and gb is not None:
            ops.gemm_tn(A, Bm, M, N1, N2, out=gw.view(N1, N2), accumulate=True, colsum_out=gb, colsum_accumulate=True, amap=amap)
            _fire(*params)
            return None, None
    if bias:
        return ops.gemm_tn(A, Bm, M, N1, N2, want_colsum=True, amap=amap)
    return ops.gemm_tn(A, Bm, M, N1, N2, amap=amap), None


def _ln_grad_buffers(params, D, device):
    if params is not None:
        gw, gb = _sink(params[0]), _sink(params[1])
        if gw is not None and gb is not None:
            return gw, gb, True
    return (torch.zeros(D, dtype=torch.float32, device=device), torch.zeros(D, dtype=torch.float32, device=device), False)


_exact = False


def set_exact_stream(on):
    global _exact
    _exact = bool(on)


def exact_stream():
    return _exact


_exact_grad = False


def set_exact_grad_stream(on):
    global _exact_grad
    _exact_grad = bool(on)


def exact_grad_stream():
    return _exact_grad


def _grad_stream(dout, x_stream):
    if not _exact_grad or x_stream.dtype != torch.float32 or dout.dtype != torch.bfloat16:
        return None
    h = getattr(dout, '_vtx_g32', None)
    if h is not None and h[1] == dout._version and h[0].shape == dout.shape and h[0].device == dout.device:
        return h[0]
    return ops.cast_to_f32(dout)


def _hand_on(dx, dx32):
    if dx32 is not None:
        dx._vtx_g32 = (dx32, dx._version)
    return dx


def _ln_bwd_res(dxn, x_stream, xmap, rows, D, mean, rstd, ln_w, dout, dx, d_ln_w, d_ln_b, g32, dx32):
    if g32 is not None:
        ops.layernorm_bwd(dxn, D, IDENT, x_stream, D, xmap, rows, D, mean, rstd, ln_w, None, dx, D, d_ln_w, d_ln_b, dres32=g32, dx32=dx32)
    else:
        ops.layernorm_bwd(dxn, D, IDENT, x_stream, D, xmap, rows, D, mean, rstd, ln_w, dout, dx, D, d_ln_w, d_ln_b)


def _copy_rows_res(dout, dx, g32, dx32, rows, D, rowmap):
    ops.row_scale_copy(dout, dx, rows, D, smap=rowmap, dmap=rowmap)
    if g32 is not None:
        ops.row_scale_copy(g32, dx32, rows, D, smap=rowmap, dmap=rowmap)


_zero1 = {}


def _zero_rows(finite_src, dst, rows, D, rowmap):
    z = _zero1.get(dst.device)
    if z is None:
        z = _zero1[dst.device] = torch.zeros(1, dtype=torch.float32, device=dst.device)
    ops.row_scale_copy(finite_src, dst, rows, D, smap=rowmap, dmap=rowmap, s=z, rs=(1, 0, 1, 0))


def _empty(shape, like, dtype=None):
    return torch.empty(shape, dtype=dtype or like.dtype, device=like.device)


def _chk(x):
    ops.need_cuda(x)
    if not x.is_contiguous():
        x = x.contiguous()
    return x


def _prenorm_fwd(x, xs, exact, ln_w, ln_b, eps, rows, xmap):
    D = x.shape[-1]
    xn = _empty((rows, D), x)
    mean = _empty((rows,), x, torch.float32)
    rstd = _empty((rows,), x, torch.float32)
    if exact:
        x32 = torch.empty(x.shape, dtype=torch.float32, device=x.device)
        ops.layernorm_acc_fwd(xs, x, rows, D, D, xmap, x32, D, xmap, ln_w, ln_b, eps, xn, D, IDENT, mean, rstd)
        return xn, mean, rstd, x32, None
    ops.layernorm_fwd(x, rows, D, D, xmap, ln_w, ln_b, eps, xn, D, IDENT, mean, rstd)
    return xn, mean, rstd, None, x


def _prenorm_save(ctx, out, x, x32, saved, scale_vec, wts):
    ctx.save_for_backward(x if x32 is None else x32, *saved, scale_vec if scale_vec is not None else x.new_empty(0),
                          *[t for t in wts if t is not None])
    if x32 is None:
        return out
    ctx.mark_non_differentiable(x32)
    ctx.set_materialize_grads(False)
    return out, x32


def _prenorm_bwd(dout, dxn, x_stream, xmap, ln_w, mean, rstd, params, skip=None):
    D = dout.shape[-1]
    dx = torch.empty_like(dout)
    g32 = _grad_stream(dout, x_stream)
    dx32 = torch.empty_like(g32) if g32 is not None else None
    d_ln_w, d_ln_b, direct = _ln_grad_buffers(params, D, dout.device)
    _ln_bwd_res(dxn, x_stream, xmap, mean.numel(), D, mean, rstd, ln_w, dout, dx, d_ln_w, d_ln_b, g32, dx32)
    if direct:
        _fire(*params)
        d_ln_w = d_ln_b = None
    if skip is not None:
        _copy_rows_res(dout, dx, g32, dx32, skip[0], D, skip[1])
    _hand_on(dx, dx32)
    return dx, d_ln_w, d_ln_b


def _qkv_fwd(xn, qkv_w, qkv_b, rows, D, need_t, qmap=IDENT, qrows=None):
    wq, wqT = weights(qkv_w, xn.dtype, need_t)
    qkv = _empty((rows if qrows is None else qrows, 3 * D), xn)
    ops.gemm_nt(xn, wq, qkv, rows, 3 * D, D, bias=qkv_b, cmap=qmap)
    return qkv, wqT


def _qkv_bwd(params, dqkv, xn, wqT, rows, D, qmap=IDENT):
    d_qkv_w, d_qkv_b = _weight_grads(params, dqkv, xn, rows, 3 * D, D, amap=qmap)
    dxn = _empty((rows, D), dqkv)
    ops.gemm_nt(dqkv, wqT, dxn, rows, D, 3 * D, amap=qmap)
    return d_qkv_w, d_qkv_b, dxn


def _cls_rows(shape):
    return shape[0], ops.clsmap(shape[1] - 1)


def _cls_pass_acc(x, xs, x32):
    rows, cm = _cls_rows(x.shape)
    ops.layernorm_acc_fwd(xs, x, rows, x.shape[-1], x.shape[-1], cm, x32, x.shape[-1], cm)


def _cls_pass_out(x, out, exact):
    rows, cm = _cls_rows(x.shape)
    if exact:
        _zero_rows(x, out, rows, x.shape[-1], cm)
    else:
        ops.row_scale_copy(x, out, rows, x.shape[-1], smap=cm, dmap=cm)


class TimeAttnFn(torch.autograd.Function):

    @staticmethod
    def forward(ctx, x, ln_w, ln_b, qkv_w, qkv_b, proj_w, proj_b, tfc_w, tfc_b, T, heads, scale_vec, eps=1e-5,
                keep_scale=None, xs=None, exact=False, proj_drop=None):
        x = _chk(x)
        B, N1, D = x.shape
        N = N1 - 1
        M = B * N
        hd = D // heads
        tm = ops.tokmap(N)
        dtp = x.dtype
        need_t = any(ctx.needs_input_grad)
        merged = _merge_tfc and (scale_vec is None or keep_scale is not None) and proj_b is not None and tfc_b is not None
        merged = merged and proj_drop is None
        xn, mean, rstd, x32, res = _prenorm_fwd(x, xs, exact, ln_w, ln_b, eps, M, tm)
        if exact:
            _cls_pass_acc(x, xs, x32)
        qkv, wqT = _qkv_fwd(xn, qkv_w, qkv_b, M, D, need_t)
        o = _empty((M, D), x)
        S = M // T
        lse = _empty((S * heads * T,), x, torch.float32)
        scale = hd ** -0.5
        ops.attn_fwd(qkv, o, lse, ATTN_CONTIG, S, T, heads, hd, scale)
        out = torch.empty_like(x)
        if merged:
            c = 1.0 if scale_vec is None else float(keep_scale)
            wc, wcT, bias = merged_proj(proj_w, proj_b, tfc_w, tfc_b, dtp, need_t, c)
            ops.gemm_nt(o, wc, out, M, D, D, cmap=tm, bias=bias, R=res, rmap=tm, row_scale=scale_vec, rs=(T, 1, 1, 0))
            if scale_vec is not None:
                ops.dropped_rows_fix(scale_vec, M, D, T, x=res, xmap=tm, bias=tfc_b.detach(), out=out, omap=tm, zero=o)
            a = x.new_empty(0)
            wts = (wqT, wcT)
        else:
            wp, wpT = weights(proj_w, dtp, need_t)
            a = _empty((M, D), x)
            if proj_drop is None:
                ops.gemm_nt(o, wp, a, M, D, D, bias=proj_b, row_scale=scale_vec, rs=(T, 1, 1, 0))
            else:
                ops.gemm_nt(o, wp, a, M, D, D, bias=proj_b)
                ops.dropout_rows(a, a, M, D, proj_drop[0], proj_drop[1], 0, s=scale_vec, rs=(T, 1, 1, 0))
            wt, wtT = weights(tfc_w, dtp, need_t)
            ops.gemm_nt(a, wt, out, M, D, D, cmap=tm, bias=tfc_b, R=res, rmap=tm)
            wts = (wqT, wpT, wtT)
        _cls_pass_out(x, out, exact)
        ctx.cfg = (T, heads, scale_vec is not None, merged, keep_scale)
        ctx.proj_drop = proj_drop
        ctx.params = (ln_w, ln_b, qkv_w, qkv_b, proj_w, proj_b, tfc_w, tfc_b)
        return _prenorm_save(ctx, out, x, x32, (ln_w, mean, rstd, xn, qkv, o, lse, a), scale_vec, wts)

    @staticmethod
    def backward(ctx, dout, _dstream=None):
        x, ln_w, mean, rstd, xn, qkv, o, lse, a, sv, wqT, *wrest = ctx.saved_tensors
        p_ln_w, p_ln_b, p_qkv_w, p_qkv_b, p_proj_w, p_proj_b, p_tfc_w, p_tfc_b = ctx.params
        T, heads, has_scale, merged, keep_scale = ctx.cfg
        sv = sv if has_scale else None
        dout = _chk(dout)
        B, N1, D = x.shape
        N = N1 - 1
        M = B * N
        hd = D // heads
        S = M // T
        tm = ops.tokmap(N)
        x_stream, x = x, dout
        do = _empty((M, D), x)
        if merged:
            wcT, = wrest
            c = float(keep_scale) if has_scale else 1.0
            G, cs_all = ops.gemm_tn(dout, o, M, D, D, amap=tm, want_colsum=True)
            ops.gemm_nt(dout, wcT, do, M, D, D, amap=tm, row_scale=sv, rs=(T, 1, 1, 0))
            if has_scale:
                part = ops.dropped_rows_colsum(dout, sv, M, D, T, smap=tm)
                u = ops.reduce_rows(cs_all, 1, 1, D, D, 0, 1, 0, scale=c)
                ops.reduce_rows(part, 1, part.shape[0], D, D, 0, 1, 0, out=u, scale=-c, accumulate=True)
                u = u.view(-1)
            else:
                u = cs_all
            pw, pb, tw = p_proj_w.detach(), p_proj_b.detach(), p_tfc_w.detach()
            sinks = [_sink(p) for p in (p_tfc_w, p_tfc_b, p_proj_w, p_proj_b)]
            if all(g is not None for g in sinks):
                ops.wprod(G, pw, tb=True, alpha=c, u=u, v=pb, out=sinks[0], accumulate=True)
                ops.wprod(tw, G, ta=True, alpha=c, out=sinks[2], accumulate=True, x=u, y=sinks[3], y_accumulate=True)
                ops.reduce_rows(cs_all, 1, 1, D, D, 0, 1, 0, out=sinks[1].view(1, D), accumulate=True)
                _fire(p_tfc_w, p_tfc_b, p_proj_w, p_proj_b)
                d_tfc_w = d_tfc_b = d_proj_w = d_proj_b = None
            else:
                d_tfc_w = ops.wprod(G, pw, tb=True, alpha=c, u=u, v=pb)
                d_proj_w, d_proj_b = ops.wprod(tw, G, ta=True, alpha=c, x=u)
                d_tfc_b = cs_all
        else:
            wpT, wtT = wrest
            d_tfc_w, d_tfc_b = _weight_grads((p_tfc_w, p_tfc_b), dout, a, M, D, D, amap=tm)
            da = _empty((M, D), x)
            if ctx.proj_drop is None:
                ops.gemm_nt(dout, wtT, da, M, D, D, amap=tm, row_scale=sv, rs=(T, 1, 1, 0))
            else:
                ops.gemm_nt(dout, wtT, da, M, D, D, amap=tm)
                ops.dropout_rows(da, da, M, D, ctx.proj_drop[0], ctx.proj_drop[1], 0, s=sv, rs=(T, 1, 1, 0))
            d_proj_w, d_proj_b = _weight_grads((p_proj_w, p_proj_b), da, o, M, D, D)
            ops.gemm_nt(da, wpT, do, M, D, D)
        dqkv = _empty((M, 3 * D), x)
        ops.attn_bwd(qkv, o, lse, do, dqkv, ATTN_CONTIG, S, T, heads, hd, hd ** -0.5)
        d_qkv_w, d_qkv_b, dxn = _qkv_bwd((p_qkv_w, p_qkv_b), dqkv, xn, wqT, M, D)
        dx, d_ln_w, d_ln_b = _prenorm_bwd(dout, dxn, x_stream, tm, ln_w, mean, rstd, (p_ln_w, p_ln_b), skip=_cls_rows(dout.shape))
        return (dx, d_ln_w, d_ln_b, d_qkv_w, d_qkv_b, d_proj_w, d_proj_b, d_tfc_w, d_tfc_b, None, None, None, None, None, None, None, None)


CLS_NONE, CLS_MEAN, CLS_PASS = 0, 1, 2
AttnLayout = collections.namedtuple('AttnLayout', (
    'mode', 'S', 'L', 'B', 'T', 'P',
    'rows', 'xmap',
    'qrows', 'qmap',
    'Mo', 'tok', 'ncls', 'groups',
    'rs', 'omap',
    'cls', 'direct'))


@functools.lru_cache(maxsize=64)
def _attn_layout(kind, shape, T):
    Bc, N1, _ = shape
    if kind == 'self':
        M = Bc * N1
        return AttnLayout(ATTN_CONTIG, Bc, N1, 0, 0, 0, rows=M, xmap=IDENT, qrows=M, qmap=IDENT, Mo=M, tok=M, ncls=0,
                          groups=0, rs=(N1, 1, 1, 0), omap=IDENT, cls=CLS_NONE, direct=False)
    N = N1 - 1
    P = N // T
    M, M1, tm = Bc * N, Bc * N1, ops.tokmap(N)
    if kind == 'space':
        return AttnLayout(ATTN_SPACE, Bc * T, P + 1, Bc, T, P, rows=M1, xmap=IDENT, qrows=M1, qmap=IDENT, Mo=M + Bc * T, tok=M,
                          ncls=Bc * T, groups=T, rs=(N, T, T, 1), omap=tm, cls=CLS_MEAN, direct=True)
    if kind == 'time_cls':
        return AttnLayout(ATTN_TIME_CLS, Bc * P, T + 1, Bc, T, P, rows=M1, xmap=IDENT, qrows=M1, qmap=IDENT, Mo=M + Bc * P, tok=M,
                          ncls=Bc * P, groups=P, rs=(T, 1, 1, 0), omap=tm, cls=CLS_MEAN, direct=True)
    if kind == 'space_nocls':
        return AttnLayout(ATTN_SPACE_NOCLS, Bc * T, P, Bc, T, P, rows=M, xmap=tm, qrows=M1, qmap=tm, Mo=M, tok=M, ncls=0,
                          groups=0, rs=(N, T, T, 1), omap=tm, cls=CLS_PASS, direct=True)
    raise ValueError(f'AttnFn: unknown kind {kind!r}')


class AttnFn(torch.autograd.Function):

    @staticmethod
    def forward(ctx, x, ln_w, ln_b, qkv_w, qkv_b, proj_w, proj_b, kind, T, heads, scale_vec, want_probs, eps=1e-5, xs=None,
                exact=False, proj_drop=None):
        x = _chk(x)
        lay = _attn_layout(kind, x.shape, T)
        D = x.shape[-1]
        hd = D // heads
        Mo = lay.Mo
        need_t = any(ctx.needs_input_grad)
        xn, mean, rstd, x32, res = _prenorm_fwd(x, xs, exact, ln_w, ln_b, eps, lay.rows, lay.xmap)
        if exact and lay.cls == CLS_PASS:
            _cls_pass_acc(x, xs, x32)
        qkv, wqT = _qkv_fwd(xn, qkv_w, qkv_b, lay.rows, D, need_t, qmap=lay.qmap, qrows=lay.qrows)
        o = _empty((Mo, D), x)
        lse = _empty((lay.S * heads * lay.L,), x, torch.float32)
        probs = _empty((lay.S, heads, lay.L, lay.L), x, torch.float32) if want_probs else None
        ops.attn_fwd(qkv, o, lse, lay.mode, lay.S, lay.L, heads, hd, hd ** -0.5, lay.B, lay.T, lay.P, probs=probs)
        if want_probs:
            ctx.mark_non_differentiable(probs)
            return probs
        wp, wpT = weights(proj_w, x.dtype, need_t)
        out = torch.empty_like(x)
        a_cls = _empty((lay.ncls, D), x) if lay.ncls else None
        if proj_drop is None:
            ops.gemm_nt(o, wp, out, Mo, D, D, cmap=lay.omap, bias=proj_b, row_scale=scale_vec, rs=lay.rs, R=res, rmap=lay.omap,
                        split_row=lay.tok if lay.ncls else 0, Csplit=a_cls)
        else:
            ops.gemm_nt(o, wp, out, Mo, D, D, cmap=lay.omap, bias=proj_b, split_row=lay.tok if lay.ncls else 0, Csplit=a_cls)
            ops.dropout_rows(out, out, lay.tok, D, proj_drop[0], proj_drop[1], 0, xmap=lay.omap, ymap=lay.omap, post=res,
                             pmap=lay.omap, s=scale_vec, rs=lay.rs)
            if lay.ncls:
                ops.dropout_rows(a_cls, a_cls, lay.ncls, D, proj_drop[0], proj_drop[1], 0, e0=lay.tok * D, s=scale_vec,
                                 rs=(1, 1, 1, 0))
        if lay.cls == CLS_MEAN:
            ops.cls_mean_fwd(a_cls, res, out, lay.B, lay.groups, D, x.shape[1])
        elif lay.cls == CLS_PASS:
            _cls_pass_out(x, out, exact)
        ctx.cfg = (kind, T, heads, scale_vec is not None)
        ctx.proj_drop = proj_drop
        ctx.params = ((ln_w, ln_b), (qkv_w, qkv_b), (proj_w, proj_b)) if lay.direct else (None, None, None)
        return _prenorm_save(ctx, out, x, x32, (ln_w, mean, rstd, xn, qkv, o, lse), scale_vec, (wqT, wpT))

    @staticmethod
    def backward(ctx, dout, _dstream=None):
        x, ln_w, mean, rstd, xn, qkv, o, lse, sv, wqT, wpT = ctx.saved_tensors
        p_ln, p_qkv, p_proj = ctx.params
        kind, T, heads, has_scale = ctx.cfg
        lay = _attn_layout(kind, x.shape, T)
        dout = _chk(dout)
        D = x.shape[-1]
        hd = D // heads
        Mo = lay.Mo
        x_stream, x = x, dout
        amap = IDENT
        if lay.cls == CLS_MEAN:
            da = _empty((Mo, D), x)
            prep = ops.time_cls_grad_prep if lay.mode == ATTN_TIME_CLS else ops.space_grad_prep
            prep(dout, sv if has_scale else None, da, lay.B, lay.T, lay.P, D)
            if ctx.proj_drop is not None:
                ops.dropout_rows(da, da, Mo, D, ctx.proj_drop[0], ctx.proj_drop[1], 0)
        elif ctx.proj_drop is not None:
            da = _empty((Mo, D), x)
            ops.dropout_rows(dout, da, Mo, D, ctx.proj_drop[0], ctx.proj_drop[1], 0, xmap=lay.omap, s=sv if has_scale else None,
                             rs=lay.rs)
        elif has_scale:
            da = _empty((Mo, D), x)
            ops.row_scale_copy(dout, da, Mo, D, smap=lay.omap, s=sv, rs=lay.rs)
        else:
            da, amap = dout, lay.omap
        d_proj_w, d_proj_b = _weight_grads(p_proj, da, o, Mo, D, D, amap=amap)
        do = _empty((Mo, D), x)
        ops.gemm_nt(da, wpT, do, Mo, D, D, amap=amap)
        dqkv = _empty((lay.qrows, 3 * D), x)
        dqkv_cls = _empty((lay.ncls, 3 * D), x) if lay.ncls else None
        ops.attn_bwd(qkv, o, lse, do, dqkv, lay.mode, lay.S, lay.L, heads, hd, hd ** -0.5, lay.B, lay.T, lay.P, dqkv_cls=dqkv_cls)
        if lay.cls == CLS_MEAN:
            ops.cls_qkv_reduce(dqkv_cls, dqkv, lay.B, lay.groups, 3 * D, x.shape[1])
        d_qkv_w, d_qkv_b, dxn = _qkv_bwd(p_qkv, dqkv, xn, wqT, lay.rows, D, qmap=lay.qmap)
        dx, d_ln_w, d_ln_b = _prenorm_bwd(dout, dxn, x_stream, lay.xmap, ln_w, mean, rstd, p_ln,
                                          skip=_cls_rows(x.shape) if lay.cls == CLS_PASS else None)
        return (dx, d_ln_w, d_ln_b, d_qkv_w, d_qkv_b, d_proj_w, d_proj_b, None, None, None, None, None, None, None, None, None)


_compact = True


def set_compact_droppath(on):
    global _compact
    _compact = bool(on)


def _compaction_plan(scale_vec, n_units, rows_per, device):
    host = getattr(scale_vec, '_vtx_host', None) if scale_vec is not None else None
    if not _compact or host is None or host.numel() != n_units or rows_per < 256:
        return None
    hv = host.numpy()
    kept = [i for i in range(n_units) if hv[i] != 0.0]
    drop = [i for i in range(n_units) if hv[i] == 0.0]
    if not drop:
        return None
# ... 873 lines not shown
```

videotransformer-pytorch_amd/vtx/ops.py:

```python
import ctypes as C

import torch

from . import _lib
from ._lib import RowMap, IDENT, GemmDesc, GemmTnDesc, AttnDesc, AttnBwdDesc, call

_DT = {torch.float32: _lib.VTX_F32, torch.bfloat16: _lib.VTX_BF16}


def dt(t):
    try:
        return _DT[t.dtype]
    except KeyError:
        raise TypeError(f'vtx: unsupported activation dtype {t.dtype} (float32 or bfloat16)')


def need_cuda(*ts):
    cur = None
    for t in ts:
        if t is None:
            continue
        if not t.is_cuda:
            raise RuntimeError('vtx: the HIP path needs CUDA/HIP tensors (no CPU fallback); '
                               f'got a tensor on {t.device}')
# ... 53 lines not shown
        for e0, e1, key, fl, by in recs:
            r = per.setdefault(key, [0, 0.0, 0.0, 0.0])
            r[0] += 1
            r[1] += e0.elapsed_time(e1)
            r[2] += fl
            r[3] += by
    _prof = None
    return out


def profile_totals(per_class):
    return {c: tuple(sum(v[i] for v in d.values()) for i in range(4)) for c, d in per_class.items()}


class _timed:
    def __init__(self, cls, flops=0.0, nbytes=0.0, key=''):
        self.on = _prof is not None and cls in _prof
        self.cls, self.rec = cls, (key, float(flops), float(nbytes))

    def __enter__(self):
        if self.on:
            self.e0 = torch.cuda.Event(enable_timing=True)
            self.e1 = torch.cuda.Event(enable_timing=True)
            self.e0.record()

    def __exit__(self, *a):
        if self.on:
            self.e1.record()
            _prof[self.cls].append((self.e0, self.e1) + self.rec)


def _f32(t):
    if t is not None and t.dtype != torch.float32:
        raise TypeError('vtx: parameter tensors must be float32')
    return t


def layernorm_fwd(x, rows, D, ldx, xmap, gamma, beta, eps, y, ldy, ymap=IDENT, mean=None, rstd=None):
    need_cuda(x, y, gamma, beta)
    with _timed('ln_fwd', nbytes=rows * D * (x.element_size() + y.element_size()), key=f'{rows}x{D}'):
        call('vtx_layernorm_fwd', dt(x), rows, D, ptr(x), ldx, xmap, ptr(_f32(gamma)), ptr(_f32(beta)), float(eps),
             ptr(y), ldy, ymap, ptr(mean), ptr(rstd), stream())


def layernorm_acc_fwd(xs, d, rows, D, lds, smap, xo, ldo, omap, gamma=None, beta=None, eps=1e-5, y=None, ldy=0, ymap=IDENT,
                      mean=None, rstd=None):
    need_cuda(d, xo, xs, y)
    if d.dtype != torch.bfloat16 or xo.dtype != torch.float32 or (xs is not None and xs.dtype != torch.float32):
        raise TypeError('layernorm_acc_fwd: d bfloat16, xs / xo float32')
    nb = rows * D * (2 + 4 + (4 if xs is not None else 0) + (2 if y is not None else 0))
    with _timed('ln_fwd', nbytes=nb, key=f'acc {rows}x{D}'):
        call('vtx_layernorm_acc_fwd', rows, D, ptr(xs), ptr(d), lds, smap, ptr(xo), ldo, omap, ptr(_f32(gamma)), ptr(_f32(beta)),
             float(eps), ptr(y), ldy, ymap, ptr(mean), ptr(rstd), stream())


def layernorm_bwd(dy, lddy, dymap, x, ldx, xmap, rows, D, mean, rstd, gamma, dres, dx, lddx, dgamma, dbeta, dres32=None, dx32=None):
    need_cuda(dy, x, dx)
    ws_bytes = _lib.load().vtx_layernorm_bwd_workspace(rows, D)
    ws = torch.empty(ws_bytes // 4, dtype=torch.float32, device=x.device)
    if dres32 is not None:
        need_cuda(dres32, dx32)
        if dy.dtype != torch.bfloat16 or x.dtype != torch.float32 or dres32.dtype != torch.float32 or dx32.dtype != torch.float32:
            raise TypeError('layernorm_bwd: the float32 gradient stream takes bf16 dy / dx and float32 x / dres32 / dx32')
        with _timed('ln_bwd', nbytes=(2 + 4 + 4 + 4 + 2) * rows * D, key=f'g32 {rows}x{D}'):
            call('vtx_layernorm_bwd_g32', rows, D, ptr(dy), lddy, dymap, ptr(x), ldx, xmap, ptr(mean), ptr(rstd), ptr(gamma), ptr(dres32),
                 ptr(dx32), ptr(dx), lddx, ptr(dgamma), ptr(dbeta), ptr(ws), ws_bytes, stream())
        return
    mixed = dy.dtype == torch.bfloat16 and x.dtype == torch.float32
    with _timed('ln_bwd', nbytes=((3.0 if dres is not None else 2.0) * dy.element_size() + x.element_size()) * rows * D, key=f'{rows}x{D}'):
        call('vtx_layernorm_bwd', _lib.VTX_BF16_X32 if mixed else dt(dy), rows, D, ptr(dy), lddy, dymap, ptr(x), ldx, xmap, ptr(mean), ptr(rstd),
             ptr(gamma), ptr(dres), ptr(dx), lddx, ptr(dgamma), ptr(dbeta), ptr(ws), ws_bytes, stream())


_nt_ws = {}


def _gemm_nt_workspace(device):
    key = (device.index, torch.cuda.current_stream(device).cuda_stream)
    ws = _nt_ws.get(key)
    if ws is None:
        ws = torch.zeros(_lib.load().vtx_gemm_nt_workspace() // 4, dtype=torch.int32, device=device)
        _nt_ws[key] = ws
    return ws


def gemm_nt(A, B, Cout, M, N, K, lda=None, ldb=None, ldc=None, amap=IDENT, cmap=IDENT, bias=None, act=0,
            C2=None, dgelu_in=None, dgelu_kind=0, row_scale=None, rs=(1, 0, 1, 0), R=None, ldr=None, rmap=IDENT,
            r_period=0, split_row=0, Csplit=None):
    need_cuda(A, B, Cout)
    if A.dtype != B.dtype or A.dtype != Cout.dtype:
        raise TypeError(f'gemm_nt: dtype mismatch {A.dtype} {B.dtype} {Cout.dtype}')
    d = GemmDesc()
    d.dtype = dt(A); d.M, d.N, d.K = int(M), int(N), int(K)
    d.A = ptr(A); d.lda = K if lda is None else lda; d.amap = amap
    d.B = ptr(B); d.ldb = K if ldb is None else ldb
    d.C = ptr(Cout); d.ldc = N if ldc is None else ldc; d.cmap = cmap
    d.bias = ptr(_f32(bias)); d.act = act
    d.C2 = ptr(C2); d.ldc2 = N
    d.dgelu_in = ptr(dgelu_in); d.ld_dgelu = N; d.dgelu_kind = int(dgelu_kind)
    d.row_scale = ptr(_f32(row_scale)); d.rs_d1, d.rs_m1, d.rs_d2, d.rs_m2 = [int(v) for v in rs]
    d.R = ptr(R); d.ldr = (N if ldr is None else ldr); d.rmap = rmap; d.r_period = int(r_period)
    d.split_row = int(split_row); d.Csplit = ptr(Csplit); d.ldsplit = N
    ws = _gemm_nt_workspace(A.device)
    d.workspace = ptr(ws); d.ws_bytes = ws.numel() * 4
    if _lib._TRACE:
        import sys
        sys.stderr.write(f'[vtx]   gemm_nt M={M} N={N} K={K} lda={d.lda} ldc={d.ldc} A={tuple(A.shape)} B={tuple(B.shape)} C={tuple(Cout.shape)} amap=({amap.grp},{amap.skip},{amap.base}) cmap=({cmap.grp},{cmap.skip},{cmap.base}) bias={bias is not None} rs={row_scale is not None} R={R is not None} split={split_row}\n')
    if _prof is not None and 'gemm_nt' in _prof:
        es = A.element_size()
        nb = (M * K + N * K + M * N) * es
        tags = ''
        if C2 is not None:
            nb += M * N * es
            tags += '+preact' if act == 1 else "+gelu'out"
        if dgelu_in is not None:
            nb += M * N * es
            tags += "+gelu'" if dgelu_kind == 0 else '+mul'
        if R is not None:
            nb += (min(M, r_period) if r_period else M) * N * es
            tags += '+res'
        if row_scale is not None:
            tags += '+scale'
        with _timed('gemm_nt', 2.0 * M * N * K, nb, f'{M}x{N}x{K}{tags}'):
            call('vtx_gemm_nt', C.byref(d), stream())
    else:
        call('vtx_gemm_nt', C.byref(d), stream())


def gemm_tn(A, B, M, N1, N2, out=None, lda=None, ldb=None, amap=IDENT, bmap=IDENT, accumulate=False,
            want_colsum=False, colsum_out=None, colsum_accumulate=False):
    need_cuda(A, B)
    if out is None:
        out = torch.empty(N1, N2, dtype=torch.float32, device=A.device)
    if colsum_out is not None:
        need_cuda(colsum_out)
        want_colsum = True
        cs = colsum_out
    else:
        cs = torch.empty(N1, dtype=torch.float32, device=A.device) if want_colsum else None
    ws_bytes = _lib.load().vtx_gemm_tn_workspace(M, N1, N2)
    ws = torch.empty(ws_bytes // 4, dtype=torch.float32, device=A.device)
    d = GemmTnDesc()
    d.dtype = dt(A); d.M, d.N1, d.N2 = int(M), int(N1), int(N2)
    d.A = ptr(A); d.lda = N1 if lda is None else lda; d.amap = amap
    d.B = ptr(B); d.ldb = N2 if ldb is None else ldb; d.bmap = bmap
    d.C = ptr(out); d.ldc = N2; d.accumulate = int(bool(accumulate))
    d.workspace = ptr(ws); d.ws_bytes = ws_bytes
    d.colsum = ptr(cs); d.colsum_accumulate = int(bool(colsum_accumulate and colsum_out is not None))
    with _timed('gemm_tn', 2.0 * M * N1 * N2, M * (N1 + N2) * A.element_size() + N1 * N2 * 4, f'{M}x{N1}x{N2}'):
        call('vtx_gemm_tn', C.byref(d), stream())
    return (out, cs) if want_colsum else out


def wprod(A, B, ta=False, tb=False, out=None, alpha=1.0, accumulate=False, u=None, v=None, x=None, y=None, alpha_y=1.0,
          z=None, beta_z=0.0, y_accumulate=False):
    need_cuda(A, B, out, u, v, x, y, z)
    for t in (A, B, out, u, v, x, y, z):
        if t is not None and (t.dtype != torch.float32 or not t.is_contiguous()):
            raise TypeError('wprod: contiguous float32 tensors expected')
    d = _lib.WprodDesc()
    ar, ac = A.shape
    br, bc = B.shape
    if ta:
        d.N1, K, d.a_rs, d.a_ks = ac, ar, 1, ac
    else:
        d.N1, K, d.a_rs, d.a_ks = ar, ac, ac, 1
    if tb:
        Kb, d.N2, d.b_ks, d.b_cs = bc, br, 1, bc
    else:
        Kb, d.N2, d.b_ks, d.b_cs = br, bc, bc, 1
    if K != Kb:
        raise ValueError(f'wprod: inner dimensions differ ({K} vs {Kb})')
    d.K = K
    if out is None:
        if accumulate:
            raise ValueError('wprod: accumulate needs an output tensor')
        out = torch.empty(d.N1, d.N2, dtype=torch.float32, device=A.device)
    if x is not None and y is None:
        if y_accumulate:
            raise ValueError('wprod: y_accumulate needs y')
        y = torch.empty(d.N1, dtype=torch.float32, device=A.device)
    d.A, d.B, d.C, d.ldc = ptr(A), ptr(B), ptr(out), d.N2
    d.alpha, d.accumulate = float(alpha), int(bool(accumulate))
    d.u, d.v, d.x, d.y, d.z = ptr(u), ptr(v), ptr(x), ptr(y), ptr(z)
    d.alpha_y, d.beta_z, d.y_accumulate = float(alpha_y), float(beta_z), int(bool(y_accumulate))
    with _timed('wprod', 2.0 * d.N1 * d.N2 * K, 4.0 * (d.N1 * K + K * d.N2 + d.N1 * d.N2), f'{d.N1}x{d.N2}x{K}'):
        call('vtx_wprod', C.byref(d), stream())
    return out if x is None else (out, y)


def colsum(A, M, N, lda=None, amap=IDENT, out=None, accumulate=False):
    need_cuda(A)
    if out is None:
        out = torch.empty(N, dtype=torch.float32, device=A.device)
    ws_bytes = _lib.load().vtx_colsum_workspace(M, N)
    ws = torch.empty(ws_bytes // 4, dtype=torch.float32, device=A.device)
    with _timed('colsum', nbytes=1.0 * M * N * A.element_size(), key=f'{M}x{N}'):
        call('vtx_colsum', dt(A), M, N, ptr(A), N if lda is None else lda, amap, ptr(out), int(bool(accumulate)),
             ptr(ws), ws_bytes, stream())
    return out


def _attn_desc(qkv, out, lse, mode, S, L, H, hd, scale, B=0, T=0, P=0, probs=None):
    d = AttnDesc()
    d.dtype = dt(qkv); d.mode = mode
    d.S, d.L, d.H, d.hd = int(S), int(L), int(H), int(hd)
    d.B, d.T, d.P = int(B), int(T), int(P)
    d.qkv = ptr(qkv); d.ld_qkv = 3 * H * hd
    d.out = ptr(out); d.ld_out = H * hd
    d.lse = ptr(lse); d.probs = ptr(probs); d.scale = float(scale)
    return d


def _attn_kind(mode, L):
    if mode in (_lib.ATTN_SPACE, _lib.ATTN_SPACE_NOCLS):
        return 'space'
    return 'time' if L <= 32 else 'seq' if L <= 256 else 'long'


def attn_fwd(qkv, out, lse, mode, S, L, H, hd, scale, B=0, T=0, P=0, probs=None):
    need_cuda(qkv, out, lse)
    d = _attn_desc(qkv, out, lse, mode, S, L, H, hd, scale, B, T, P, probs)
    kind = _attn_kind(mode, L)
    rows = S * L
    with _timed(f'attn_fwd_{kind}', 4.0 * S * H * L * L * hd, rows * H * hd * 4 * qkv.element_size() + rows * H * 4,
                f'{S}x{L}x{H}'):
        call('vtx_attn_fwd', C.byref(d), stream())


def attn_bwd(qkv, out, lse, dout, dqkv, mode, S, L, H, hd, scale, B=0, T=0, P=0, dqkv_cls=None):
    need_cuda(qkv, out, dout, dqkv)
    b = AttnBwdDesc()
    b.f = _attn_desc(qkv, out, lse, mode, S, L, H, hd, scale, B, T, P)
    b.dout = ptr(dout); b.ld_dout = H * hd
    b.dqkv = ptr(dqkv); b.ld_dqkv = 3 * H * hd
    b.dqkv_cls = ptr(dqkv_cls)
    delta = torch.empty(S * H * L, dtype=torch.float32, device=qkv.device)
    b.delta = ptr(delta)
    kind = _attn_kind(mode, L)
    rows = S * L
    with _timed(f'attn_bwd_{kind}', 10.0 * S * H * L * L * hd, rows * H * hd * 8 * qkv.element_size() + rows * H * 4,
                f'{S}x{L}x{H}'):
        call('vtx_attn_bwd', C.byref(b), stream())


def fact_glue_fwd(x, time_embed, B, T, P, D):
    need_cuda(x, time_embed)
    h = torch.empty(B, 1 + T, D, dtype=x.dtype, device=x.device)
    call('vtx_fact_glue_fwd', dt(x), B, T, P, D, ptr(x), ptr(_f32(time_embed)), ptr(h), stream())
    return h


def fact_glue_bwd(dh, B, T, P, D, d_time_embed=None, accumulate=False):
    need_cuda(dh)
    dx = torch.empty(B * T, 1 + P, D, dtype=dh.dtype, device=dh.device)
    call('vtx_fact_glue_bwd', dt(dh), B, T, P, D, ptr(dh), ptr(dx), ptr(d_time_embed), int(bool(accumulate)), stream())
    return dx


def cls_mean_fwd(a_cls, x, out, B, T, D, rows_per_clip):
    call('vtx_cls_mean_fwd', dt(out), B, T, D, ptr(a_cls), D, ptr(x), ptr(out), D, rows_per_clip, stream())


def space_grad_prep(dout, s, da, B, T, P, D):
    call('vtx_space_grad_prep', dt(dout), B, T, P, D, ptr(dout), D, ptr(s), ptr(da), D, stream())


def time_cls_grad_prep(dout, s, da, B, T, P, D):
    call('vtx_space_grad_prep', dt(dout), B, P, -T, D, ptr(dout), D, ptr(s), ptr(da), D, stream())


def cls_qkv_reduce(dqkv_cls, dqkv, B, T, W, rows_per_clip):
    call('vtx_cls_qkv_reduce', dt(dqkv), B, T, W, ptr(dqkv_cls), W, ptr(dqkv), W, rows_per_clip, stream())


def row_scale_copy(src, dst, rows, D, lds=None, smap=IDENT, ldd=None, dmap=IDENT, s=None, rs=(1, 0, 1, 0)):
    need_cuda(src, dst)
    call('vtx_row_scale_copy', dt(src), rows, D, ptr(src), D if lds is None else lds, smap, ptr(dst),
         D if ldd is None else ldd, dmap, ptr(s), int(rs[0]), int(rs[1]), int(rs[2]), int(rs[3]), stream())


DROPOUT_GRID_CAP, DROPOUT_BLOCK = 4096, 256
DROPOUT_TRIP = DROPOUT_GRID_CAP * DROPOUT_BLOCK * 8


def dropout_params(p):
    import fractions
    import numpy as np
    p = float(p)
    if not 0.0 <= p <= 1.0:
        raise ValueError(f'dropout probability has to be between 0 and 1, but got {p}')
    thr = int(fractions.Fraction(p) * (1 << 32))
    scale = 0.0 if p == 1.0 else float(np.float32(1.0) / np.float32(1 - p))
    return thr, scale


def dropout_rows(x, y, rows, D, p, seed, site, e0=0, ldx=None, xmap=IDENT, ldy=None, ymap=IDENT, post=None, ldp=None, pmap=IDENT,
                 pre=None, pre_period=0, s=None, rs=(1, 0, 1, 0)):
    need_cuda(x, y, post, pre, s)
    thr, scale = dropout_params(p)
    if post is not None and post.dtype != x.dtype:
        raise TypeError('dropout_rows: the residual must have the dtype of x')
    _lib.dropout_call('vtx_dropout_rows', dt(x), int(rows), int(D), ptr(x), D if ldx is None else ldx, xmap, ptr(y), D if ldy is None else ldy,
         ymap, ptr(post), D if ldp is None else ldp, pmap, ptr(_f32(pre)), int(pre_period), ptr(_f32(s)), int(rs[0]), int(rs[1]),
         int(rs[2]), int(rs[3]), thr, scale, int(seed), int(site), int(e0), stream())


def dropped_rows_fix(s, M, D, group_rows, x=None, xmap=IDENT, bias=None, out=None, omap=IDENT, zero=None, ldx=None, ldo=None):
    ref = out if out is not None else zero
    need_cuda(ref, s)
    call('vtx_dropped_rows_fix', dt(ref), M, D, group_rows, ptr(s), ptr(x), D if ldx is None else ldx, xmap, ptr(bias),
         ptr(out), D if ldo is None else ldo, omap, ptr(zero), D, stream())


def dropped_rows_colsum(src, s, M, D, group_rows, smap=IDENT, lds=None, nparts=96):
    need_cuda(src, s)
    part = torch.empty((nparts, D), dtype=torch.float32, device=src.device)
    call('vtx_dropped_rows_colsum', dt(src), M, D, group_rows, ptr(s), ptr(src), D if lds is None else lds, smap, ptr(part),
         nparts, stream())
    return part


def reduce_rows(inp, nj, ni, D, ld, base, si, sj, out=None, scale=1.0, accumulate=False):
    need_cuda(inp)
    if out is None:
        out = torch.empty(nj, D, dtype=torch.float32, device=inp.device)
    call('vtx_reduce_rows', dt(inp), nj, ni, D, ptr(inp), ld, base, si, sj, ptr(out), D, float(scale),
         int(bool(accumulate)), stream())
    return out


def cast_transpose(W, dtype, want_c=True, want_t=True):
    need_cuda(W)
    if W.dtype != torch.float32:
        raise TypeError(f'vtx: cast_transpose stages fp32 weights, got {W.dtype}')
    R, Cc = W.shape
    W = W.contiguous()
    code = _DT[dtype]
# ... 617 lines not shown
```

videotransformer-pytorch_amd/vtx/optim.py:

```python
import ctypes as C

import torch

from . import _lib, ops


class _Table:
    """One launch's device table: (param, grad, state) pointers, chunk starts, norm scratch."""


class _FusedBase(torch.optim.Optimizer):
    def __init__(self, params, defaults, clip_grad=None):
        if hasattr(params, 'buckets'):
            params = [p for b in params.buckets for p in b['params']]
        super().__init__(params, defaults)
        self.clip_grad = clip_grad
        self.last_grad_norm = None
        self._table_cache = {}
        self._skipped = frozenset()

    def _step_of(self, p):
        return int(self.state[p].get('step', 0))

    def set_skipped(self, params):
        self._skipped = frozenset(id(p) for p in params)

    def _entries(self):
        ent = []
        for gi, group in enumerate(self.param_groups):
            for p in group['params']:
                if p.grad is None or id(p) in self._skipped:
                    continue
                if p.dtype != torch.float32 or p.grad.dtype != torch.float32:
                    raise TypeError('vtx.optim: parameters and gradients must be float32')
                if not p.is_contiguous() or not p.grad.is_contiguous():
                    raise ValueError('vtx.optim: parameters and gradients must be contiguous')
                ent.append((p, gi))
        return ent

    def _state_tensors(self, p):
        raise NotImplementedError

    def _partition(self, ent):
        return [ent]

    def _build(self, ent):
        lib = _lib.load()
        dev = ent[0][0].device
        ops.need_cuda(*[p for p, _ in ent])
        t = _Table()
        tab = (_lib.MtTensor * len(ent))()
        starts = [0]
        for i, (p, gi) in enumerate(ent):
            s1, s2 = self._state_tensors(p)
            tab[i].p, tab[i].g = p.data_ptr(), p.grad.data_ptr()
            tab[i].s1, tab[i].s2 = s1.data_ptr(), (s2.data_ptr() if s2 is not None else None)
            tab[i].n = p.numel()
            starts.append(starts[-1] + lib.vtx_mt_chunks(p.numel()))
        t.params = [p for p, _ in ent]
        t.tab_host = tab
        t.groups_of = [gi for _, gi in ent]
        t.n_chunks = starts[-1]
        t.chunk_start = torch.tensor(starts, dtype=torch.int32).to(dev)
        t.tab_dev = torch.empty(C.sizeof(tab), dtype=torch.uint8, device=dev)
        t.partial = torch.empty(t.n_chunks, dtype=torch.float32, device=dev)
        t.norms = torch.zeros(len(ent) + 1, dtype=torch.float32, device=dev)
        t.hyper = None
        return t

    def _sync_tables(self):
        ent = self._entries()
        if not ent:
            return []
        tables = []
        for part in self._partition(ent):
            key = tuple((p.data_ptr(), p.grad.data_ptr(), p.numel(), gi) for p, gi in part)
            t = self._table_cache.get(key)
            if t is None:
                if len(self._table_cache) >= 16:
                    self._table_cache.pop(next(iter(self._table_cache)))
                t = self._build(part)
                self._table_cache[key] = t
            tables.append(t)
        hyper = tuple((float(g['lr']), float(g['weight_decay'])) for g in self.param_groups)
        for t in tables:
            if hyper != t.hyper:
                for i, gi in enumerate(t.groups_of):
                    t.tab_host[i].lr, t.tab_host[i].wd = hyper[gi]
                raw = bytes(t.tab_host)
                t.tab_dev.copy_(torch.frombuffer(bytearray(raw), dtype=torch.uint8), non_blocking=False)
                t.hyper = hyper
        return tables

    def grad_norm(self):
        tables = self._sync_tables()
        if not tables:
            return None
        for t in tables:
            _lib.call('vtx_mt_grad_norms', t.tab_dev.data_ptr(), t.chunk_start.data_ptr(), len(t.groups_of),
                      t.n_chunks, t.partial.data_ptr(), t.norms.data_ptr(), ops.stream())
        if len(tables) == 1:
            return tables[0].norms[-1]
        return torch.stack([t.norms[-1] for t in tables]).norm()

    @torch.no_grad()
    def step(self, closure=None):
        loss = None
        if closure is not None:
            with torch.enable_grad():
                loss = closure()
        tables = self._sync_tables()
        if not tables:
            return loss
        clip = float(self.clip_grad) if self.clip_grad else 0.0
        if clip > 0.0:
            self.last_grad_norm = self.grad_norm()
        for t in tables:
            for p in t.params:
                self.state[p]['step'] = self._step_of(p) + 1
            self._launch(t, clip, self._step_of(t.params[0]))
        self._bump_versions()
        from . import functions
        functions.restage_weights([p for g in self.param_groups for p in g['params']
                                   if p.grad is not None and p.ndim >= 2 and id(p) not in self._skipped])
        return loss

    def _bump_versions(self):
        for group in self.param_groups:
            for p in group['params']:
                if p.grad is not None:
                    p.view(-1)[:0].zero_()

    def _launch(self, table, clip, step):
        raise NotImplementedError

    def add_param_group(self, param_group):
        super().add_param_group(param_group)
        self._table_cache = {}

    def state_dict(self):
        sd = super().state_dict()
        sd['state'] = {k: {**v, 'step': torch.tensor(float(v.get('step', 0)))} for k, v in sd['state'].items()}
        return sd

    def load_state_dict(self, state_dict):
        super().load_state_dict(state_dict)
        for p, st in self.state.items():
            if 'step' in st:
                st['step'] = int(float(st['step']))
        self._table_cache = {}


class FusedSGD(_FusedBase):

    def __init__(self, params, lr=1e-3, momentum=0.9, nesterov=True, weight_decay=0.0, clip_grad=None):
        if nesterov and momentum <= 0:
            raise ValueError('Nesterov momentum requires a momentum')
        super().__init__(params, dict(lr=lr, momentum=momentum, dampening=0, weight_decay=weight_decay, nesterov=nesterov,
                                      maximize=False, foreach=None, differentiable=False, fused=None), clip_grad)

    def _state_tensors(self, p):
        st = self.state[p]
        if 'momentum_buffer' not in st:
            st['momentum_buffer'] = torch.zeros_like(p, memory_format=torch.contiguous_format)
        return st['momentum_buffer'], None

    def _launch(self, t, clip, step):
        g0 = self.param_groups[0]
        if any(g['momentum'] != g0['momentum'] or g['nesterov'] != g0['nesterov'] for g in self.param_groups):
            raise NotImplementedError('vtx.optim.FusedSGD: momentum / nesterov must be the same in every group')
        if any(g.get('dampening', 0) or g.get('maximize', False) for g in self.param_groups):
            raise NotImplementedError('vtx.optim.FusedSGD: dampening / maximize are not implemented')
        _lib.call('vtx_mt_sgd_step', t.tab_dev.data_ptr(), t.chunk_start.data_ptr(), len(t.groups_of),
                  t.n_chunks, t.norms.data_ptr(), clip, float(g0['momentum']), int(bool(g0['nesterov'])),
                  0, ops.stream())


class FusedAdamW(_FusedBase):

    def __init__(self, params, lr=1e-3, betas=(0.9, 0.999), eps=1e-8, weight_decay=1e-2, clip_grad=None):
        super().__init__(params, dict(lr=lr, betas=betas, eps=eps, weight_decay=weight_decay, amsgrad=False, maximize=False,
                                      foreach=None, capturable=False, differentiable=False, fused=None,
                                      decoupled_weight_decay=True), clip_grad)

    def _state_tensors(self, p):
        st = self.state[p]
        if 'exp_avg' not in st:
            st['exp_avg'] = torch.zeros_like(p, memory_format=torch.contiguous_format)
            st['exp_avg_sq'] = torch.zeros_like(p, memory_format=torch.contiguous_format)
        return st['exp_avg'], st['exp_avg_sq']

    def _partition(self, ent):
        by_step = {}
        for e in ent:
            by_step.setdefault(self._step_of(e[0]), []).append(e)
        return [by_step[k] for k in sorted(by_step, reverse=True)]

    def _launch(self, t, clip, step):
        g0 = self.param_groups[0]
        if any(g['betas'] != g0['betas'] or g['eps'] != g0['eps'] for g in self.param_groups):
            raise NotImplementedError('vtx.optim.FusedAdamW: betas / eps must be the same in every group')
        if any(g.get('amsgrad', False) or g.get('maximize', False) or not g.get('decoupled_weight_decay', True) for g in self.param_groups):
            raise NotImplementedError('vtx.optim.FusedAdamW: amsgrad / maximize / coupled weight decay are not implemented')
        _lib.call('vtx_mt_adamw_step', t.tab_dev.data_ptr(), t.chunk_start.data_ptr(), len(t.groups_of),
                  t.n_chunks, t.norms.data_ptr(), clip, float(g0['betas'][0]), float(g0['betas'][1]),
                  float(g0['eps']), step, ops.stream())
```

Measured before the change: 758.0.

## Batch side-path weight-product kernels and merge dropped-row reductions in temporal attention backward

Measured after the change: 761.0 (median of 6 runs). Within noise of the previous version (+0.4%).

```diff
diff --git a/__graft_entry__.py b/__graft_entry__.py
--- a/__graft_entry__.py
+++ b/__graft_entry__.py
@@ -43,6 +43,8 @@
     print('libvtx_ragged', vtx._lib.load_ragged().vtx_ragged_version(), 'symbols bound:', len(vtx._lib.RAGGED_SIGNATURES))
     assert vtx._lib.load_dropout().vtx_dropout_version() >= 100
     print('libvtx_dropout', vtx._lib.load_dropout().vtx_dropout_version(), 'symbols bound:', len(vtx._lib.DROPOUT_SIGNATURES))
+    assert vtx._lib.load_mside().vtx_mside_version() >= 100
+    print('libvtx_mside', vtx._lib.load_mside().vtx_mside_version(), 'symbols bound:', len(vtx._lib.MSIDE_SIGNATURES))
 
 
 def smoke():
diff --git a/include/vtx.h b/include/vtx.h
--- a/include/vtx.h
+++ b/include/vtx.h
@@ -85,6 +85,7 @@
   const float* u; const float* v;
   const float* x; float* y;
   float alpha_y; const float* z; float beta_z; int y_accumulate;
+  void* Cb; void* CbT; int cb_dtype;
 } vtx_wprod_desc;
 int vtx_wprod(const vtx_wprod_desc* d, void* stream);
 
diff --git a/include/vtx_mside.h b/include/vtx_mside.h
--- /dev/null
+++ b/include/vtx_mside.h
@@ -0,0 +1,22 @@
+#ifndef VTX_MSIDE_H_
+#define VTX_MSIDE_H_
+
+#include "vtx.h"
+
+#ifdef __cplusplus
+extern "C" {
+#endif
+
+int vtx_mside_version(void);
+const char* vtx_mside_last_error_string(void);
+
+int vtx_wprod_tiles(const vtx_wprod_desc* d, int* form);
+int vtx_wprod_batch(const vtx_wprod_desc* table_dev, const int* tile_start_dev, int n_problems, int n_tiles, void* stream);
+
+int vtx_merged_u(int D, const float* cs, const float* part, int nparts, float c, float* u, float* db, void* stream);
+
+#ifdef __cplusplus
+}
+#endif
+
+#endif
diff --git a/videotransformer-pytorch_amd/csrc/api.hip b/videotransformer-pytorch_amd/csrc/api.hip
--- a/videotransformer-pytorch_amd/csrc/api.hip
+++ b/videotransformer-pytorch_amd/csrc/api.hip
@@ -52,6 +52,7 @@
     {{"VTX_GEMM_PP_EPI", "pp_epi"}, OPT_INT, &Options::pp_epi, INT_MIN, INT_MAX, 1},
     {{"VTX_GEMM_PP_CONT", "pp_cont"}, OPT_FLAG, &Options::pp_cont},
     {{"VTX_LN_ROWS", "ln_rows"}, OPT_INT, &Options::ln_rows, 1, 4, 1},
+    {{"VTX_MERGED_SIDE", "merged_side"}, OPT_FLAG, &Options::merged_side},
     {{nullptr, "pp_trace"}, OPT_ADDR, nullptr}};
 #undef VTX_ENUM
 
diff --git a/videotransformer-pytorch_amd/csrc/build.py b/videotransformer-pytorch_amd/csrc/build.py
--- a/videotransformer-pytorch_amd/csrc/build.py
+++ b/videotransformer-pytorch_amd/csrc/build.py
@@ -16,7 +16,8 @@
         'mix',
         'stem',
         'ragged',
-        'dropout']
+        'dropout',
+        'mside']
 FLAGS = ['--offload-arch=gfx950', '-O3', '-std=c++17', '-fPIC', '-fno-gpu-rdc', '-Wno-unused-result', '-Wno-unused-value', '-Wno-inline-asm',
          '-Wno-cuda-compat']
 EXTRA = {'hog.hip': ['-ffp-contract=off'],
diff --git a/videotransformer-pytorch_amd/csrc/common.h b/videotransformer-pytorch_amd/csrc/common.h
--- a/videotransformer-pytorch_amd/csrc/common.h
+++ b/videotransformer-pytorch_amd/csrc/common.h
@@ -159,6 +159,7 @@
   int attn_fwd_stream = 1;
   int attn_dkv = 3;
   int ln_rows = 3;
+  int merged_side = 1;
   int pp_grid = 256;
   int pp_cg = 0;
   int pp_epi = 0;
diff --git a/videotransformer-pytorch_amd/csrc/elementwise.hip b/videotransformer-pytorch_amd/csrc/elementwise.hip
--- a/videotransformer-pytorch_amd/csrc/elementwise.hip
+++ b/videotransformer-pytorch_amd/csrc/elementwise.hip
@@ -446,6 +446,116 @@
   }
 }
 
+constexpr int DR_SCAN = 16, DR_U = 4, DR_MAX_GRID = 2048;
+template <typename T>
+__global__ __launch_bounds__(256) void dropped_rows_fix2_kernel(long M, int D, int group_rows, long n_groups, const float* __restrict__ s,
+                                                                const T* __restrict__ x, long ldx, vtx_rowmap xmap,
+                                                                const float* __restrict__ bias, T* __restrict__ out, long ldo,
+                                                                vtx_rowmap omap, T* __restrict__ zero, long ldz) {
+  const int tid = threadIdx.x, lane = tid & 63;
+  const int dv = D >> 3, vpg = group_rows * dv;
+  const float z8[8] = {0, 0, 0, 0, 0, 0, 0, 0};
+  for (long gb = (long)blockIdx.x * DR_SCAN; gb < n_groups; gb += (long)gridDim.x * DR_SCAN) {
+    const bool drop = lane < DR_SCAN && gb + lane < n_groups && s[gb + lane] == 0.f;
+    unsigned long long mask = __ballot(drop);
+    while (mask != 0) {
+      const long m0 = (gb + __builtin_ctzll(mask)) * group_rows;
+      mask &= mask - 1;
+      for (int base = 0; base < vpg; base += 256 * DR_U) {
+        float v[DR_U][8], b[DR_U][8];
+        long m[DR_U];
+        int c[DR_U];
+        bool ok[DR_U];
+#pragma unroll
+        for (int j = 0; j < DR_U; ++j) {
+          const int idx = base + tid + 256 * j;
+          ok[j] = idx < vpg && m0 + idx / dv < M;
+          const int idc = ok[j] ? idx : 0, r = idc / dv;
+          c[j] = (idc - r * dv) * 8;
+          m[j] = m0 + r;
+#pragma unroll
+          for (int e = 0; e < 8; ++e) v[j][e] = 0.f;
+        }
+        if (out != nullptr) {
+          if (x != nullptr) {
+#pragma unroll
+            for (int j = 0; j < DR_U; ++j) load8(x + map_row(xmap, m[j]) * ldx + c[j], v[j]);
+          }
+#pragma unroll
+          for (int j = 0; j < DR_U; ++j) load8(bias + c[j], b[j]);
+        }
+#pragma unroll
+        for (int j = 0; j < DR_U; ++j) {
+          if (!ok[j]) continue;
+          if (out != nullptr) {
+#pragma unroll
+            for (int e = 0; e < 8; ++e) v[j][e] += b[j][e];
+            store8(out + map_row(omap, m[j]) * ldo + c[j], v[j]);
+          }
+          if (zero) store8(zero + m[j] * ldz + c[j], z8);
+        }
+      }
+    }
+  }
+}
+
+constexpr int DC_U = 8;
+template <typename T>
+__global__ __launch_bounds__(256) void dropped_rows_colsum2_kernel(long M, int D, int group_rows, const float* __restrict__ s,
+                                                                   const T* __restrict__ src, long lds_, vtx_rowmap smap,
+                                                                   float* __restrict__ part, long n_groups) {
+#pragma clang fp contract(off)
+  __shared__ float red[8][128 + 4];
+  __shared__ int list[256];
+  __shared__ int wcnt[4];
+  const int cl = threadIdx.x & 31, rl = threadIdx.x >> 5, lane = threadIdx.x & 63, w = threadIdx.x >> 6;
+  const int c = blockIdx.x * 128 + cl * 4;
+  const long per = (n_groups + gridDim.y - 1) / gridDim.y;
+  const long g0 = (long)blockIdx.y * per, g1 = g0 + per < n_groups ? g0 + per : n_groups;
+  const bool lane_ok = c < D && rl < group_rows;
+  float a[4] = {0, 0, 0, 0};
+  for (long gb = g0; gb < g1; gb += 256) {
+    const bool drop = gb + threadIdx.x < g1 && s[gb + threadIdx.x] == 0.f;
+    const unsigned long long bal = __ballot(drop);
+    __syncthreads();
+    if (lane == 0) wcnt[w] = __popcll(bal);
+    __syncthreads();
+    int off = 0, n = 0;
+#pragma unroll
+    for (int i = 0; i < 4; ++i) { off += i < w ? wcnt[i] : 0; n += wcnt[i]; }
+    if (drop) list[off + __popcll(bal & ((1ull << lane) - 1ull))] = threadIdx.x;
+    __syncthreads();
+    for (int k = 0; k < n; k += DC_U) {
+      float v[DC_U][4];
+      bool ok[DC_U];
+#pragma unroll
+      for (int j = 0; j < DC_U; ++j) {
+        const long mg = (gb + list[k + j < n ? k + j : n - 1]) * group_rows;
+        ok[j] = lane_ok && k + j < n && mg + rl < M;
+        const T* p = src + map_row(smap, ok[j] ? mg + rl : mg) * lds_ + (ok[j] ? c : 0);
+#pragma unroll
+        for (int e = 0; e < 4; ++e) v[j][e] = ET<T>::ld(p + e);
+      }
+#pragma unroll
+      for (int j = 0; j < DC_U; ++j)
+#pragma unroll
+        for (int e = 0; e < 4; ++e) a[e] = ok[j] ? a[e] + v[j][e] : a[e];
+    }
+  }
+#pragma unroll
+  for (int e = 0; e < 4; ++e) red[rl][cl * 4 + e] = a[e];
+  __syncthreads();
+  if (rl == 0 && c < D) {
+#pragma unroll
+    for (int e = 0; e < 4; ++e) {
+      float t = 0.f;
+#pragma unroll
+      for (int i = 0; i < 8; ++i) t += red[i][cl * 4 + e];
+      part[(long)blockIdx.y * D + c + e] = t;
+    }
+  }
+}
+
 }
 
 using namespace vtx;
@@ -626,8 +736,17 @@
   VTX_REQUIRE(out || zero, VTX_EINVAL, "dropped_rows_fix: nothing to do");
   VTX_REQUIRE(!out || bias, VTX_EINVAL, "dropped_rows_fix: out needs the bias");
   const long groups = (M + group_rows - 1) / group_rows;
+  hipStream_t st = as_stream(stream);
+  if (options().merged_side) {
+    const long runs = (groups + DR_SCAN - 1) / DR_SCAN;
+    dim3 grid2((unsigned)(runs < DR_MAX_GRID ? runs : DR_MAX_GRID)), block2(256);
+    DISPATCH_T(dtype,
+               hipLaunchKernelGGL(dropped_rows_fix2_kernel<float>, grid2, block2, 0, st, M, D, group_rows, groups, s, (const float*)x, ldx, xmap, bias, (float*)out, ldo, omap, (float*)zero, ldz),
+               hipLaunchKernelGGL(dropped_rows_fix2_kernel<bf16raw>, grid2, block2, 0, st, M, D, group_rows, groups, s, (const bf16raw*)x, ldx, xmap, bias, (bf16raw*)out, ldo, omap, (bf16raw*)zero, ldz),
+               "dropped_rows_fix");
+    return check_launch("dropped_rows_fix");
+  }
   dim3 grid((unsigned)((groups + 3) / 4)), block(256);
-  hipStream_t st = as_stream(stream);
   DISPATCH_T(dtype,
              hipLaunchKernelGGL(dropped_rows_fix_kernel<float>, grid, block, 0, st, M, D, group_rows, s, (const float*)x, ldx, xmap, bias, (float*)out, ldo, omap, (float*)zero, ldz),
              hipLaunchKernelGGL(dropped_rows_fix_kernel<bf16raw>, grid, block, 0, st, M, D, group_rows, s, (const bf16raw*)x, ldx, xmap, bias, (bf16raw*)out, ldo, omap, (bf16raw*)zero, ldz),
@@ -642,6 +761,13 @@
   const long groups = (M + group_rows - 1) / group_rows;
   dim3 grid((unsigned)((D + 127) / 128), (unsigned)nparts), block(256);
   hipStream_t st = as_stream(stream);
+  if (options().merged_side && group_rows <= 8) {
+    DISPATCH_T(dtype,
+               hipLaunchKernelGGL(dropped_rows_colsum2_kernel<float>, grid, block, 0, st, M, D, group_rows, s, (const float*)src, lds, smap, part, groups),
+               hipLaunchKernelGGL(dropped_rows_colsum2_kernel<bf16raw>, grid, block, 0, st, M, D, group_rows, s, (const bf16raw*)src, lds, smap, part, groups),
+               "dropped_rows_colsum");
+    return check_launch("dropped_rows_colsum");
+  }
   DISPATCH_T(dtype,
              hipLaunchKernelGGL(dropped_rows_colsum_kernel<float>, grid, block, 0, st, M, D, group_rows, s, (const float*)src, lds, smap, part, groups),
              hipLaunchKernelGGL(dropped_rows_colsum_kernel<bf16raw>, grid, block, 0, st, M, D, group_rows, s, (const bf16raw*)src, lds, smap, part, groups),
diff --git a/videotransformer-pytorch_amd/csrc/mside.hip b/videotransformer-pytorch_amd/csrc/mside.hip
--- /dev/null
+++ b/videotransformer-pytorch_amd/csrc/mside.hip
@@ -0,0 +1,83 @@
+#include "side_lib.h"
+#include "wprod_tile.h"
+
+VTX_SIDE_LIB(mside)
+
+namespace vtx {
+
+__global__ __launch_bounds__(WP_THREADS) void wprod_batch_kernel(const vtx_wprod_desc* __restrict__ tab, const int* __restrict__ tile_start,
+                                                                 int n_problems) {
+  __shared__ WprodLds sm;
+  int lo = 0, hi = n_problems;
+  const int b = blockIdx.x;
+  while (hi - lo > 1) {
+    const int mid = (lo + hi) >> 1;
+    if (tile_start[mid] <= b) lo = mid; else hi = mid;
+  }
+  const vtx_wprod_desc d = tab[lo];
+  const WprodParams p = params_of(d);
+  const int l = b - tile_start[lo], ntx = (d.N2 + WP_T - 1) / WP_T;
+  const int by = l / ntx, bx = l - by * ntx;
+  if (l < 0 || by * WP_T >= d.N1) return;
+  switch (wprod_inst(d)) {
+#define WP_CASE(I_) case I_: wprod_tile<((I_) & 8) != 0, ((I_) & 4) != 0, ((I_) & 2) != 0, ((I_) & 1) != 0>(p, bx, by, sm); break;
+    WP_CASE(0) WP_CASE(1) WP_CASE(2) WP_CASE(3) WP_CASE(4) WP_CASE(5) WP_CASE(6) WP_CASE(7)
+    WP_CASE(8) WP_CASE(9) WP_CASE(10) WP_CASE(11) WP_CASE(12) WP_CASE(13) WP_CASE(14) WP_CASE(15)
+#undef WP_CASE
+  }
+}
+
+__global__ __launch_bounds__(256) void merged_u_kernel(int D, const float* __restrict__ cs, const float* __restrict__ part, int nparts,
+                                                       float c, float* __restrict__ u, float* __restrict__ db) {
+#pragma clang fp contract(off)
+  __shared__ float red[8][128 + 4];
+  const int cl = threadIdx.x & 31, rl = threadIdx.x >> 5;
+  const int col4 = blockIdx.x * 128 + cl * 4;
+  float a[4] = {0, 0, 0, 0};
+  if (col4 < D) {
+    for (int i = rl; i < nparts; i += 8) {
+      const float* p = part + (long)i * D + col4;
+#pragma unroll
+      for (int e = 0; e < 4; ++e) a[e] += p[e];
+    }
+  }
+#pragma unroll
+  for (int e = 0; e < 4; ++e) red[rl][cl * 4 + e] = a[e];
+  __syncthreads();
+  if (threadIdx.x < 128) {
+    const int col = blockIdx.x * 128 + threadIdx.x;
+    if (col < D) {
+      float t = 0.f;
+#pragma unroll
+      for (int r = 0; r < 8; ++r) t += red[r][threadIdx.x];
+      t *= -c;
+      const float t1 = 0.f + cs[col];
+      const float u1 = t1 * c;
+      u[col] = u1 + t;
+      if (db != nullptr) db[col] = db[col] + t1;
+    }
+  }
+}
+
+}
+
+using namespace vtx;
+
+extern "C" int vtx_wprod_tiles(const vtx_wprod_desc* d, int* inst) {
+  if (wprod_validate(d) != VTX_OK) return -1;
+  if (inst) *inst = wprod_inst(*d);
+  return cdiv(d->N2, WP_T) * cdiv(d->N1, WP_T);
+}
+
+extern "C" int vtx_wprod_batch(const vtx_wprod_desc* table_dev, const int* tile_start_dev, int n_problems, int n_tiles, void* stream) {
+  VTX_REQUIRE(table_dev && tile_start_dev && n_problems > 0 && n_tiles >= 0, VTX_EINVAL, "wprod_batch: bad arguments");
+  if (n_tiles == 0) return VTX_OK;
+  hipLaunchKernelGGL(wprod_batch_kernel, dim3(n_tiles), dim3(WP_THREADS), 0, as_stream(stream), table_dev, tile_start_dev, n_problems);
+  return check_launch("wprod_batch");
+}
+
+extern "C" int vtx_merged_u(int D, const float* cs, const float* part, int nparts, float c, float* u, float* db, void* stream) {
+  VTX_REQUIRE(D > 0 && D % 4 == 0 && cs && part && nparts > 0 && u, VTX_EINVAL, "merged_u: bad arguments");
+  hipLaunchKernelGGL(merged_u_kernel, dim3(cdiv(D, 128)), dim3(256), 0, as_stream(stream), D, cs, part, nparts, c, u, db);
+  return check_launch("merged_u");
+}
diff --git a/videotransformer-pytorch_amd/csrc/wprod.hip b/videotransformer-pytorch_amd/csrc/wprod.hip
--- a/videotransformer-pytorch_amd/csrc/wprod.hip
+++ b/videotransformer-pytorch_amd/csrc/wprod.hip
@@ -1,145 +1,11 @@
-#include "common.h"
+#include "wprod_tile.h"
 
 namespace vtx {
 
-#ifndef VTX_WP_PAD_KB
-#define VTX_WP_PAD_KB 0
-#endif
-#ifndef VTX_WP_NACC
-#define VTX_WP_NACC 2
-#endif
-#ifndef VTX_WP_D
-#define VTX_WP_D 4
-#endif
-constexpr int WP_T = 32, WP_THREADS = 256, WP_D = VTX_WP_D;
-
-struct WprodParams {
-  int N1, N2, K;
-  const float* A; long a_rs, a_ks;
-  const float* B; long b_ks, b_cs;
-  float alpha;
-  float* C; long ldc; int accumulate;
-  const float* u; const float* v;
-  const float* x; float* y; float alpha_y; const float* z; float beta_z; int y_accumulate;
-  long long* trace;
-};
-
-#ifdef VTX_WP_TRACE
-#define WP_STAMP(e_) if (p.trace != nullptr && lane == 0) { \
-    long long* sl__ = p.trace + ((long)(blockIdx.y * gridDim.x + blockIdx.x) * 4 + h) * 8; \
-    sl__[e_] = (long long)__builtin_amdgcn_s_memrealtime(); if ((e_) == 0 || (e_) == 3) sl__[(e_) == 0 ? 6 : 7] = (long long)__builtin_amdgcn_s_memtime(); }
-#else
-#define WP_STAMP(e_)
-#endif
-
 template <bool A_KCONT, bool B_KCONT, bool FULL, bool WITH_X>
 __global__ __launch_bounds__(WP_THREADS) void wprod_kernel(WprodParams p) {
-  __shared__ float red[3][16][64];
-  __shared__ float yred[4][32];
-  const int tid = threadIdx.x, lane = tid & 63;
-  const int h = __builtin_amdgcn_readfirstlane(tid >> 6);
-  const int li = lane & 31, kh = lane >> 5;
-  WP_STAMP(0)
-  const int i0 = blockIdx.y * WP_T, j0 = blockIdx.x * WP_T;
-  const int row = i0 + li, col = j0 + li;
-  const bool row_ok = row < p.N1, col_ok = col < p.N2;
-  const bool with_y = WITH_X && blockIdx.x == 0;
-  const int nb = (p.K + 7) >> 3;
-  const int per = (((nb + 3) >> 2) + WP_D - 1) / WP_D * WP_D;
-  const int b_lo = 0, b_hi = per;
-  const float* const arow = p.A + (A_KCONT ? (long)(row_ok ? row : 0) * p.a_rs : (long)(row_ok ? row : 0));
-  const float* const bcol = p.B + (B_KCONT ? (long)(col_ok ? col : 0) * p.b_cs : (long)(col_ok ? col : 0));
-
-  const float* const xbase = WITH_X ? p.x : p.A;
-  float a[WP_D][4], b[WP_D][4], xv[WP_D][4];
-  auto load = [&](int blk, float (&va)[4], float (&vb)[4], float (&vx)[4]) {
-    const int kk = (blk * 4 + h) * 8 + kh * 4;
-    const int ks = kk < p.K ? kk : 0;
-    if (A_KCONT) {
-      const float4 t = *reinterpret_cast<const float4*>(arow + ks);
-      va[0] = t.x; va[1] = t.y; va[2] = t.z; va[3] = t.w;
-    } else {
-#pragma unroll
-      for (int s = 0; s < 4; ++s) va[s] = arow[(long)(ks + s) * p.a_ks];
-    }
-    if (B_KCONT) {
-      const float4 t = *reinterpret_cast<const float4*>(bcol + ks);
-      vb[0] = t.x; vb[1] = t.y; vb[2] = t.z; vb[3] = t.w;
-    } else {
-#pragma unroll
-      for (int s = 0; s < 4; ++s) vb[s] = bcol[(long)(ks + s) * p.b_ks];
-    }
-    if constexpr (WITH_X) {
-      const float4 t = *reinterpret_cast<const float4*>(xbase + ks);
-      vx[0] = t.x; vx[1] = t.y; vx[2] = t.z; vx[3] = t.w;
-    }
-  };
-
-  f32x16 accs[VTX_WP_NACC];
-#pragma unroll
-  for (int c = 0; c < VTX_WP_NACC; ++c)
-#pragma unroll
-    for (int r = 0; r < 16; ++r) accs[c][r] = 0.f;
-  float yacc = 0.f;
-#pragma unroll
-  for (int d = 0; d < WP_D; ++d) { load(b_lo + d, a[d], b[d], xv[d]); __builtin_amdgcn_sched_barrier(0); }
-  WP_STAMP(1)
-  bool first_trip = true;
-  for (int blk = b_lo; blk < b_hi; blk += WP_D) {
-#pragma unroll
-    for (int d = 0; d < WP_D; ++d) {
-      const bool kok = FULL || ((blk + d) * 4 + h) * 8 + kh * 4 < p.K;
-      const bool aok = FULL || (kok && row_ok), bok = FULL || (kok && col_ok);
-#pragma unroll
-      for (int s = 0; s < 4; ++s) {
-        const float av = aok ? a[d][s] : 0.f, bv = bok ? b[d][s] : 0.f;
-        accs[s % VTX_WP_NACC] = __builtin_amdgcn_mfma_f32_32x32x2f32(av, bv, accs[s % VTX_WP_NACC], 0, 0, 0);
-        if constexpr (WITH_X) yacc = fmaf(av, xv[d][s], yacc);
-      }
-      load(blk + d + WP_D, a[d], b[d], xv[d]);
-      __builtin_amdgcn_sched_barrier(0);
-    }
-#ifdef VTX_WP_TRACE
-    if (first_trip) { WP_STAMP(2) first_trip = false; }
-#endif
-  }
-  WP_STAMP(3)
-  f32x16 acc = accs[0];
-#pragma unroll
-  for (int c = 1; c < VTX_WP_NACC; ++c)
-#pragma unroll
-    for (int r = 0; r < 16; ++r) acc[r] += accs[c][r];
-  if (h > 0) {
-#pragma unroll
-    for (int r = 0; r < 16; ++r) red[h - 1][r][lane] = acc[r];
-  }
-  if (with_y) {
-    const float other = __shfl_xor(yacc, 32, 64);
-    if (kh == 0) yred[h][li] = yacc + other;
-  }
-  __syncthreads();
-  WP_STAMP(4)
-  if (h == 0) {
-    const float vj = (p.u && col_ok) ? p.v[col] : 0.f;
-#pragma unroll
-    for (int r = 0; r < 16; ++r) {
-      const int orow = i0 + (r & 3) + 8 * (r >> 2) + 4 * kh;
-      if (orow < p.N1 && col_ok) {
-        float val = p.alpha * (((acc[r] + red[0][r][lane]) + red[1][r][lane]) + red[2][r][lane]);
-        if (p.u) val = fmaf(p.u[orow], vj, val);
-        float* dst = p.C + (long)orow * p.ldc + col;
-        if (p.accumulate) val += *dst;
-        *dst = val;
-      }
-    }
-    if (with_y && kh == 0 && row_ok) {
-      float val = p.alpha_y * (((yred[0][li] + yred[1][li]) + yred[2][li]) + yred[3][li]);
-      if (p.z) val = fmaf(p.beta_z, p.z[row], val);
-      if (p.y_accumulate) val += p.y[row];
-      p.y[row] = val;
-    }
-  }
-  WP_STAMP(5)
+  __shared__ WprodLds sm;
+  wprod_tile<A_KCONT, B_KCONT, FULL, WITH_X>(p, blockIdx.x, blockIdx.y, sm);
 }
 
 }
@@ -147,36 +13,16 @@
 using namespace vtx;
 
 extern "C" int vtx_wprod(const vtx_wprod_desc* d, void* stream) {
-  VTX_REQUIRE(d != nullptr, VTX_EINVAL, "wprod: null descriptor");
-  VTX_REQUIRE(d->N1 > 0 && d->N2 > 0 && d->K > 0, VTX_EINVAL, "wprod: bad shape N1=%d N2=%d K=%d", d->N1, d->N2, d->K);
-  VTX_REQUIRE(d->N1 % 4 == 0 && d->N2 % 4 == 0 && d->K % 4 == 0, VTX_EINVAL, "wprod: N1, N2, K must be multiples of 4");
-  VTX_REQUIRE(d->A && d->B && d->C, VTX_EINVAL, "wprod: null operand");
-  VTX_REQUIRE((d->a_rs == 1) != (d->a_ks == 1), VTX_EINVAL, "wprod: exactly one stride of A must be 1 (a_rs=%ld a_ks=%ld)",
-              d->a_rs, d->a_ks);
-  VTX_REQUIRE((d->b_ks == 1) != (d->b_cs == 1), VTX_EINVAL, "wprod: exactly one stride of B must be 1 (b_ks=%ld b_cs=%ld)",
-              d->b_ks, d->b_cs);
-  const long a_ld = d->a_ks == 1 ? d->a_rs : d->a_ks, b_ld = d->b_ks == 1 ? d->b_cs : d->b_ks;
-  VTX_REQUIRE(aligned16(d->A) && aligned16(d->B) && a_ld % 4 == 0 && b_ld % 4 == 0 && (!d->x || aligned16(d->x)), VTX_EALIGN,
-              "wprod: operands (and x) must be 16-byte aligned with leading dimensions that are multiples of 4");
-  VTX_REQUIRE(d->ldc >= d->N2, VTX_EINVAL, "wprod: ldc=%ld < N2=%d", d->ldc, d->N2);
-  VTX_REQUIRE((d->u == nullptr) == (d->v == nullptr), VTX_EINVAL, "wprod: the rank-1 term needs both u and v");
-  VTX_REQUIRE((d->y == nullptr) == (d->x == nullptr), VTX_EINVAL, "wprod: the vector product needs both x and y");
-  WprodParams p;
-  p.N1 = d->N1; p.N2 = d->N2; p.K = d->K;
-  p.A = d->A; p.a_rs = d->a_rs; p.a_ks = d->a_ks;
-  p.B = d->B; p.b_ks = d->b_ks; p.b_cs = d->b_cs;
-  p.alpha = d->alpha; p.C = d->C; p.ldc = d->ldc; p.accumulate = d->accumulate;
-  p.u = d->u; p.v = d->v;
-  p.trace = nullptr;
+  if (const int rc = wprod_validate(d)) return rc;
+  WprodParams p = params_of(*d);
 #ifdef VTX_WP_TRACE
   p.trace = reinterpret_cast<long long*>(options().pp_trace);
 #endif
-  p.x = d->x; p.y = d->y; p.alpha_y = d->alpha_y; p.z = d->z; p.beta_z = d->beta_z; p.y_accumulate = d->y_accumulate;
   const dim3 grid(cdiv(d->N2, WP_T), cdiv(d->N1, WP_T)), block(WP_THREADS);
   hipStream_t st = as_stream(stream);
   const bool ak = d->a_ks == 1, bk = d->b_ks == 1;
   const size_t pad = (size_t)VTX_WP_PAD_KB * 1024;
-  const bool full = d->N1 % 32 == 0 && d->N2 % 32 == 0 && d->K % (32 * WP_D) == 0, wx = d->x != nullptr;
+  const bool full = wprod_full(d->N1, d->N2, d->K), wx = d->x != nullptr;
 #define WP_LAUNCH(AK_, BK_)                                                                                          \
   {                                                                                                                  \
     if (full && wx) hipLaunchKernelGGL((wprod_kernel<AK_, BK_, true, true>), grid, block, pad, st, p);               \
diff --git a/videotransformer-pytorch_amd/csrc/wprod_tile.h b/videotransformer-pytorch_amd/csrc/wprod_tile.h
--- /dev/null
+++ b/videotransformer-pytorch_amd/csrc/wprod_tile.h
@@ -0,0 +1,217 @@
+#pragma once
+#include "common.h"
+
+namespace vtx {
+
+#ifndef VTX_WP_PAD_KB
+#define VTX_WP_PAD_KB 0
+#endif
+#ifndef VTX_WP_NACC
+#define VTX_WP_NACC 2
+#endif
+#ifndef VTX_WP_D
+#define VTX_WP_D 4
+#endif
+constexpr int WP_T = 32, WP_THREADS = 256, WP_D = VTX_WP_D;
+
+struct WprodParams {
+  int N1, N2, K;
+  const float* A; long a_rs, a_ks;
+  const float* B; long b_ks, b_cs;
+  float alpha;
+  float* C; long ldc; int accumulate;
+  const float* u; const float* v;
+  const float* x; float* y; float alpha_y; const float* z; float beta_z; int y_accumulate;
+  void* Cb; void* CbT; int cb_dtype;
+  long long* trace;
+};
+
+struct WprodLds {
+  float red[3][16][64];
+  float yred[4][32];
+  float tile[32][33];
+};
+
+__host__ __device__ inline WprodParams params_of(const vtx_wprod_desc& d) {
+  WprodParams p;
+  p.N1 = d.N1; p.N2 = d.N2; p.K = d.K;
+  p.A = d.A; p.a_rs = d.a_rs; p.a_ks = d.a_ks;
+  p.B = d.B; p.b_ks = d.b_ks; p.b_cs = d.b_cs;
+  p.alpha = d.alpha; p.C = d.C; p.ldc = d.ldc; p.accumulate = d.accumulate;
+  p.u = d.u; p.v = d.v;
+  p.x = d.x; p.y = d.y; p.alpha_y = d.alpha_y; p.z = d.z; p.beta_z = d.beta_z; p.y_accumulate = d.y_accumulate;
+  p.Cb = d.Cb; p.CbT = d.CbT; p.cb_dtype = d.cb_dtype;
+  p.trace = nullptr;
+  return p;
+}
+__host__ __device__ inline bool wprod_full(int N1, int N2, int K) { return N1 % 32 == 0 && N2 % 32 == 0 && K % (32 * WP_D) == 0; }
+
+template <typename T>
+__device__ __forceinline__ void wprod_store_cb(const WprodParams& p, const float (&tile)[32][33], int i0, int j0, int tid) {
+  const int r = tid >> 3, q = (tid & 7) * 4;
+  float v[4];
+  if (p.Cb != nullptr && i0 + r < p.N1 && j0 + q < p.N2) {
+#pragma unroll
+    for (int j = 0; j < 4; ++j) v[j] = tile[r][q + j];
+    ET<T>::st4(reinterpret_cast<T*>(p.Cb) + (long)(i0 + r) * p.N2 + j0 + q, v);
+  }
+  if (p.CbT != nullptr && j0 + r < p.N2 && i0 + q < p.N1) {
+#pragma unroll
+    for (int j = 0; j < 4; ++j) v[j] = tile[q + j][r];
+    ET<T>::st4(reinterpret_cast<T*>(p.CbT) + (long)(j0 + r) * p.N1 + i0 + q, v);
+  }
+}
+
+#ifdef VTX_WP_TRACE
+#define WP_STAMP(e_) if (p.trace != nullptr && lane == 0) { \
+    long long* sl__ = p.trace + ((long)(by * ((p.N2 + WP_T - 1) / WP_T) + bx) * 4 + h) * 8; \
+    sl__[e_] = (long long)__builtin_amdgcn_s_memrealtime(); if ((e_) == 0 || (e_) == 3) sl__[(e_) == 0 ? 6 : 7] = (long long)__builtin_amdgcn_s_memtime(); }
+#else
+#define WP_STAMP(e_)
+#endif
+
+template <bool A_KCONT, bool B_KCONT, bool FULL, bool WITH_X>
+__device__ __forceinline__ void wprod_tile(const WprodParams& p, const int bx, const int by, WprodLds& sm) {
+  float (&red)[3][16][64] = sm.red;
+  float (&yred)[4][32] = sm.yred;
+  const int tid = threadIdx.x, lane = tid & 63;
+  const int h = __builtin_amdgcn_readfirstlane(tid >> 6);
+  const int li = lane & 31, kh = lane >> 5;
+  WP_STAMP(0)
+  const int i0 = by * WP_T, j0 = bx * WP_T;
+  const int row = i0 + li, col = j0 + li;
+  const bool row_ok = row < p.N1, col_ok = col < p.N2;
+  const bool with_y = WITH_X && bx == 0;
+  const int nb = (p.K + 7) >> 3;
+  const int per = (((nb + 3) >> 2) + WP_D - 1) / WP_D * WP_D;
+  const int b_lo = 0, b_hi = per;
+  const float* const arow = p.A + (A_KCONT ? (long)(row_ok ? row : 0) * p.a_rs : (long)(row_ok ? row : 0));
+  const float* const bcol = p.B + (B_KCONT ? (long)(col_ok ? col : 0) * p.b_cs : (long)(col_ok ? col : 0));
+
+  const float* const xbase = WITH_X ? p.x : p.A;
+  float a[WP_D][4], b[WP_D][4], xv[WP_D][4];
+  auto load = [&](int blk, float (&va)[4], float (&vb)[4], float (&vx)[4]) {
+    const int kk = (blk * 4 + h) * 8 + kh * 4;
+    const int ks = kk < p.K ? kk : 0;
+    if (A_KCONT) {
+      const float4 t = *reinterpret_cast<const float4*>(arow + ks);
+      va[0] = t.x; va[1] = t.y; va[2] = t.z; va[3] = t.w;
+    } else {
+#pragma unroll
+      for (int s = 0; s < 4; ++s) va[s] = arow[(long)(ks + s) * p.a_ks];
+    }
+    if (B_KCONT) {
+      const float4 t = *reinterpret_cast<const float4*>(bcol + ks);
+      vb[0] = t.x; vb[1] = t.y; vb[2] = t.z; vb[3] = t.w;
+    } else {
+#pragma unroll
+      for (int s = 0; s < 4; ++s) vb[s] = bcol[(long)(ks + s) * p.b_ks];
+    }
+    if constexpr (WITH_X) {
+      const float4 t = *reinterpret_cast<const float4*>(xbase + ks);
+      vx[0] = t.x; vx[1] = t.y; vx[2] = t.z; vx[3] = t.w;
+    }
+  };
+
+  f32x16 accs[VTX_WP_NACC];
+#pragma unroll
+  for (int c = 0; c < VTX_WP_NACC; ++c)
+#pragma unroll
+    for (int r = 0; r < 16; ++r) accs[c][r] = 0.f;
+  float yacc = 0.f;
+#pragma unroll
+  for (int d = 0; d < WP_D; ++d) { load(b_lo + d, a[d], b[d], xv[d]); __builtin_amdgcn_sched_barrier(0); }
+  WP_STAMP(1)
+  bool first_trip = true;
+  for (int blk = b_lo; blk < b_hi; blk += WP_D) {
+#pragma unroll
+    for (int d = 0; d < WP_D; ++d) {
+      const bool kok = FULL || ((blk + d) * 4 + h) * 8 + kh * 4 < p.K;
+      const bool aok = FULL || (kok && row_ok), bok = FULL || (kok && col_ok);
+#pragma unroll
+      for (int s = 0; s < 4; ++s) {
+        const float av = aok ? a[d][s] : 0.f, bv = bok ? b[d][s] : 0.f;
+        accs[s % VTX_WP_NACC] = __builtin_amdgcn_mfma_f32_32x32x2f32(av, bv, accs[s % VTX_WP_NACC], 0, 0, 0);
+        if constexpr (WITH_X) yacc = fmaf(av, xv[d][s], yacc);
+      }
+      load(blk + d + WP_D, a[d], b[d], xv[d]);
+      __builtin_amdgcn_sched_barrier(0);
+    }
+#ifdef VTX_WP_TRACE
+    if (first_trip) { WP_STAMP(2) first_trip = false; }
+#endif
+  }
+  WP_STAMP(3)
+  f32x16 acc = accs[0];
+#pragma unroll
+  for (int c = 1; c < VTX_WP_NACC; ++c)
+#pragma unroll
+    for (int r = 0; r < 16; ++r) acc[r] += accs[c][r];
+  if (h > 0) {
+#pragma unroll
+    for (int r = 0; r < 16; ++r) red[h - 1][r][lane] = acc[r];
+  }
+  if (with_y) {
+    const float other = __shfl_xor(yacc, 32, 64);
+    if (kh == 0) yred[h][li] = yacc + other;
+  }
+  __syncthreads();
+  WP_STAMP(4)
+  const bool with_cb = p.Cb != nullptr || p.CbT != nullptr;
+  if (h == 0) {
+    const float vj = (p.u && col_ok) ? p.v[col] : 0.f;
+#pragma unroll
+    for (int r = 0; r < 16; ++r) {
+      const int orow = i0 + (r & 3) + 8 * (r >> 2) + 4 * kh;
+      if (orow < p.N1 && col_ok) {
+        float val = p.alpha * (((acc[r] + red[0][r][lane]) + red[1][r][lane]) + red[2][r][lane]);
+        if (p.u) val = fmaf(p.u[orow], vj, val);
+        if (p.C != nullptr) {
+          float* dst = p.C + (long)orow * p.ldc + col;
+          if (p.accumulate) val += *dst;
+          *dst = val;
+        }
+        if (with_cb) sm.tile[orow - i0][li] = val;
+      }
+    }
+    if (with_y && kh == 0 && row_ok) {
+      float val = p.alpha_y * (((yred[0][li] + yred[1][li]) + yred[2][li]) + yred[3][li]);
+      if (p.z) val = fmaf(p.beta_z, p.z[row], val);
+      if (p.y_accumulate) val += p.y[row];
+      p.y[row] = val;
+    }
+  }
+  if (with_cb) {
+    __syncthreads();
+    if (p.cb_dtype == VTX_BF16) wprod_store_cb<bf16raw>(p, sm.tile, i0, j0, tid);
+    else wprod_store_cb<float>(p, sm.tile, i0, j0, tid);
+  }
+  WP_STAMP(5)
+}
+
+__host__ __device__ inline int wprod_inst(const vtx_wprod_desc& d) {
+  return (d.a_ks == 1 ? 8 : 0) | (d.b_ks == 1 ? 4 : 0) | (wprod_full(d.N1, d.N2, d.K) ? 2 : 0) | (d.x != nullptr ? 1 : 0);
+}
+
+inline int wprod_validate(const vtx_wprod_desc* d) {
+  VTX_REQUIRE(d != nullptr, VTX_EINVAL, "wprod: null descriptor");
+  VTX_REQUIRE(d->N1 > 0 && d->N2 > 0 && d->K > 0, VTX_EINVAL, "wprod: bad shape N1=%d N2=%d K=%d", d->N1, d->N2, d->K);
+  VTX_REQUIRE(d->N1 % 4 == 0 && d->N2 % 4 == 0 && d->K % 4 == 0, VTX_EINVAL, "wprod: N1, N2, K must be multiples of 4");
+  VTX_REQUIRE(d->A && d->B && (d->C || d->Cb || d->CbT), VTX_EINVAL, "wprod: null operand");
+  VTX_REQUIRE(d->C || !d->accumulate, VTX_EINVAL, "wprod: accumulate needs C");
+  VTX_REQUIRE((d->a_rs == 1) != (d->a_ks == 1), VTX_EINVAL, "wprod: exactly one stride of A must be 1 (a_rs=%ld a_ks=%ld)",
+              d->a_rs, d->a_ks);
+  VTX_REQUIRE((d->b_ks == 1) != (d->b_cs == 1), VTX_EINVAL, "wprod: exactly one stride of B must be 1 (b_ks=%ld b_cs=%ld)",
+              d->b_ks, d->b_cs);
+  const long a_ld = d->a_ks == 1 ? d->a_rs : d->a_ks, b_ld = d->b_ks == 1 ? d->b_cs : d->b_ks;
+  VTX_REQUIRE(aligned16(d->A) && aligned16(d->B) && a_ld % 4 == 0 && b_ld % 4 == 0 && (!d->x || aligned16(d->x)), VTX_EALIGN,
+              "wprod: operands (and x) must be 16-byte aligned with leading dimensions that are multiples of 4");
+  VTX_REQUIRE(!d->C || d->ldc >= d->N2, VTX_EINVAL, "wprod: ldc=%ld < N2=%d", d->ldc, d->N2);
+  VTX_REQUIRE((d->u == nullptr) == (d->v == nullptr), VTX_EINVAL, "wprod: the rank-1 term needs both u and v");
+  VTX_REQUIRE((d->y == nullptr) == (d->x == nullptr), VTX_EINVAL, "wprod: the vector product needs both x and y");
+  VTX_REQUIRE((!d->Cb && !d->CbT) || d->cb_dtype == VTX_F32 || d->cb_dtype == VTX_BF16, VTX_EINVAL, "wprod: bad cb_dtype %d", d->cb_dtype);
+  VTX_REQUIRE(aligned16(d->Cb) && aligned16(d->CbT), VTX_EALIGN, "wprod: Cb / CbT must be 16-byte aligned");
+  return VTX_OK;
+}
+
+}
diff --git a/videotransformer-pytorch_amd/vtx/_lib.py b/videotransformer-pytorch_amd/vtx/_lib.py
--- a/videotransformer-pytorch_amd/vtx/_lib.py
+++ b/videotransformer-pytorch_amd/vtx/_lib.py
@@ -57,6 +57,7 @@
         ('u', C.c_void_p), ('v', C.c_void_p),
         ('x', C.c_void_p), ('y', C.c_void_p),
         ('alpha_y', C.c_float), ('z', C.c_void_p), ('beta_z', C.c_float), ('y_accumulate', C.c_int),
+        ('Cb', C.c_void_p), ('CbT', C.c_void_p), ('cb_dtype', C.c_int),
     ]
 
 
@@ -232,6 +233,15 @@
                               C.c_ulonglong, cf, C.c_ulonglong, C.c_uint, C.c_ulonglong, vp]),
 }
 
+MSIDE_LIB_PATH = os.environ.get('VTX_MSIDE_LIB', os.path.join(_PKG, 'libvtx_mside.so'))
+MSIDE_SIGNATURES = {
+    'vtx_mside_version': (ci, []),
+    'vtx_mside_last_error_string': (C.c_char_p, []),
+    'vtx_wprod_tiles': (ci, [C.POINTER(WprodDesc), C.POINTER(C.c_int)]),
+    'vtx_wprod_batch': (ci, [vp, vp, ci, ci, vp]),
+    'vtx_merged_u': (ci, [ci, vp, vp, ci, cf, vp, vp, vp]),
+}
+
 _SIDE = {
     'aug': ('AUG_LIB_PATH', AUG_SIGNATURES),
     'randaug': ('RANDAUG_LIB_PATH', RANDAUG_SIGNATURES),
@@ -240,6 +250,7 @@
     'stem': ('STEM_LIB_PATH', STEM_SIGNATURES),
     'ragged': ('RAGGED_LIB_PATH', RAGGED_SIGNATURES),
     'dropout': ('DROPOUT_LIB_PATH', DROPOUT_SIGNATURES),
+    'mside': ('MSIDE_LIB_PATH', MSIDE_SIGNATURES),
 }
 _lib = None
 _side = {}
@@ -289,6 +300,7 @@
 load_stem, stem_call = partial(_load_side, 'stem'), partial(_side_call, 'stem')
 load_ragged, ragged_call = partial(_load_side, 'ragged'), partial(_side_call, 'ragged')
 load_dropout, dropout_call = partial(_load_side, 'dropout'), partial(_side_call, 'dropout')
+load_mside, mside_call, mside_check = partial(_load_side, 'mside'), partial(_side_call, 'mside'), partial(_side_check, 'mside')
 aug_check = partial(_side_check, 'aug')
 
 
@@ -309,6 +321,21 @@
     rc = load().vtx_set_option(str(name).encode(), str(value).encode())
     if rc != 0:
         check(rc, f'vtx_set_option({name}={value})')
+    if name == 'merged_side':
+        _merged_side[0] = _flag(str(value))
+
+
+def _flag(text):
+    import re
+    m = re.match(r'\s*[+-]?\d+', text)
+    return bool(m) and int(m.group()) != 0
+
+
+_merged_side = [_flag(os.environ.get('VTX_MERGED_SIDE') or '1')]
+
+
+def merged_side():
+    return _merged_side[0]
 
 
 _TRACE = os.environ.get('VTX_TRACE_CALLS', '0') == '1'
diff --git a/videotransformer-pytorch_amd/vtx/functions.py b/videotransformer-pytorch_amd/vtx/functions.py
--- a/videotransformer-pytorch_amd/vtx/functions.py
+++ b/videotransformer-pytorch_amd/vtx/functions.py
@@ -5,7 +5,7 @@
 import torch
 
 from . import ops
-from ._lib import IDENT, ATTN_CONTIG, ATTN_SPACE, ATTN_TIME_CLS, ATTN_SPACE_NOCLS
+from ._lib import IDENT, ATTN_CONTIG, ATTN_SPACE, ATTN_TIME_CLS, ATTN_SPACE_NOCLS, merged_side as _lib_merged_side
 
 _wcache = {}
 
@@ -86,10 +86,40 @@
     return wc, wt, bias
 
 
+def restage_merged():
+    if not _lib_merged_side():
+        return
+    groups = {}
+    for key, hit in _mcache.items():
+        ps = tuple(r() for r in hit[0])
+        if any(p is None or not p.is_cuda for p in ps) or any(p.device != ps[0].device for p in ps):
+            continue
+        stamp = tuple((p._version, p.data_ptr(), p.device) for p in ps) + (hit[1][-1],)
+        if stamp == hit[1]:
+            continue
+        groups.setdefault(ps[0].device, []).append((key, hit, ps, stamp))
+    for dev, ents in groups.items():
+        descs = []
+        for key, hit, (proj_w, proj_b, tfc_w, tfc_b), stamp in ents:
+            wc, wt, bias = hit[2], hit[3], hit[4]
+            f32 = key[2] == torch.float32
+            descs.append(ops.wprod_desc(tfc_w.detach(), proj_w.detach(), x=proj_b.detach(), y=bias, z=tfc_b.detach(),
+                                        beta_z=1.0 / stamp[-1], out=wc if f32 else None, cb=None if f32 else wc, cbT=wt,
+                                        want_out=f32)[0])
+        with torch.cuda.device(dev):
+            ops.wprod_batch(('merged', dev), descs, dev)
+        for key, hit, ps, stamp in ents:
+            _mcache[key] = (hit[0], stamp) + hit[2:]
+            for t in hit[2:]:
+                if t is not None:
+                    t.view(-1)[:0].zero_()
+
+
 def clear_weight_cache():
     _wcache.clear()
     _mcache.clear()
     _restage_tables.clear()
+    ops._wprod_tables.clear()
 
 
 _direct = False
@@ -366,24 +396,38 @@
             c = float(keep_scale) if has_scale else 1.0
             G, cs_all = ops.gemm_tn(dout, o, M, D, D, amap=tm, want_colsum=True)
             ops.gemm_nt(dout, wcT, do, M, D, D, amap=tm, row_scale=sv, rs=(T, 1, 1, 0))
+            sinks = [_sink(p) for p in (p_tfc_w, p_tfc_b, p_proj_w, p_proj_b)]
+            direct = all(g is not None for g in sinks)
+            side = _lib_merged_side()
+            db_done = False
             if has_scale:
                 part = ops.dropped_rows_colsum(dout, sv, M, D, T, smap=tm)
-                u = ops.reduce_rows(cs_all, 1, 1, D, D, 0, 1, 0, scale=c)
-                ops.reduce_rows(part, 1, part.shape[0], D, D, 0, 1, 0, out=u, scale=-c, accumulate=True)
-                u = u.view(-1)
+                if side:
+                    u = ops.merged_u(cs_all, part, c, db=sinks[1] if direct else None)
+                    db_done = True
+                else:
+                    u = ops.reduce_rows(cs_all, 1, 1, D, D, 0, 1, 0, scale=c)
+                    ops.reduce_rows(part, 1, part.shape[0], D, D, 0, 1, 0, out=u, scale=-c, accumulate=True)
+                    u = u.view(-1)
             else:
                 u = cs_all
             pw, pb, tw = p_proj_w.detach(), p_proj_b.detach(), p_tfc_w.detach()
-            sinks = [_sink(p) for p in (p_tfc_w, p_tfc_b, p_proj_w, p_proj_b)]
-            if all(g is not None for g in sinks):
-                ops.wprod(G, pw, tb=True, alpha=c, u=u, v=pb, out=sinks[0], accumulate=True)
-                ops.wprod(tw, G, ta=True, alpha=c, out=sinks[2], accumulate=True, x=u, y=sinks[3], y_accumulate=True)
-                ops.reduce_rows(cs_all, 1, 1, D, D, 0, 1, 0, out=sinks[1].view(1, D), accumulate=True)
+            k_tfc = dict(tb=True, alpha=c, u=u, v=pb, out=sinks[0] if direct else None, accumulate=direct)
+            k_proj = dict(ta=True, alpha=c, out=sinks[2] if direct else None, accumulate=direct, x=u,
+                          y=sinks[3] if direct else None, y_accumulate=direct)
+            if side:
+                d1, d_tfc_w, _ = ops.wprod_desc(G, pw, **k_tfc)
+                d2, d_proj_w, d_proj_b = ops.wprod_desc(tw, G, **k_proj)
+                ops.wprod_batch(('time_bwd', id(p_tfc_w), direct), [d1, d2], G.device)
+            else:
+                d_tfc_w = ops.wprod(G, pw, **k_tfc)
+                d_proj_w, d_proj_b = ops.wprod(tw, G, **k_proj)
+            if direct:
+                if not db_done:
+                    ops.reduce_rows(cs_all, 1, 1, D, D, 0, 1, 0, out=sinks[1].view(1, D), accumulate=True)
                 _fire(p_tfc_w, p_tfc_b, p_proj_w, p_proj_b)
                 d_tfc_w = d_tfc_b = d_proj_w = d_proj_b = None
             else:
-                d_tfc_w = ops.wprod(G, pw, tb=True, alpha=c, u=u, v=pb)
-                d_proj_w, d_proj_b = ops.wprod(tw, G, ta=True, alpha=c, x=u)
                 d_tfc_b = cs_all
         else:
             wpT, wtT = wrest
diff --git a/videotransformer-pytorch_amd/vtx/ops.py b/videotransformer-pytorch_amd/vtx/ops.py
--- a/videotransformer-pytorch_amd/vtx/ops.py
+++ b/videotransformer-pytorch_amd/vtx/ops.py
@@ -229,9 +229,9 @@
     return (out, cs) if want_colsum else out
 
 
-def wprod(A, B, ta=False, tb=False, out=None, alpha=1.0, accumulate=False, u=None, v=None, x=None, y=None, alpha_y=1.0,
-          z=None, beta_z=0.0, y_accumulate=False):
-    need_cuda(A, B, out, u, v, x, y, z)
+def wprod_desc(A, B, ta=False, tb=False, out=None, alpha=1.0, accumulate=False, u=None, v=None, x=None, y=None, alpha_y=1.0,
+               z=None, beta_z=0.0, y_accumulate=False, cb=None, cbT=None, want_out=True):
+    need_cuda(A, B, out, u, v, x, y, z, cb, cbT)
     for t in (A, B, out, u, v, x, y, z):
         if t is not None and (t.dtype != torch.float32 or not t.is_contiguous()):
             raise TypeError('wprod: contiguous float32 tensors expected')
@@ -249,7 +249,7 @@
     if K != Kb:
         raise ValueError(f'wprod: inner dimensions differ ({K} vs {Kb})')
     d.K = K
-    if out is None:
+    if out is None and want_out:
         if accumulate:
             raise ValueError('wprod: accumulate needs an output tensor')
         out = torch.empty(d.N1, d.N2, dtype=torch.float32, device=A.device)
@@ -261,6 +261,77 @@
     d.alpha, d.accumulate = float(alpha), int(bool(accumulate))
     d.u, d.v, d.x, d.y, d.z = ptr(u), ptr(v), ptr(x), ptr(y), ptr(z)
     d.alpha_y, d.beta_z, d.y_accumulate = float(alpha_y), float(beta_z), int(bool(y_accumulate))
+    for t, shape in ((cb, (d.N1, d.N2)), (cbT, (d.N2, d.N1))):
+        if t is not None and (tuple(t.shape) != shape or not t.is_contiguous() or t.dtype != (cb if cb is not None else cbT).dtype):
+            raise ValueError('wprod: cb must be [N1,N2], cbT [N2,N1], contiguous and of one dtype')
+    if cb is not None or cbT is not None:
+        d.Cb, d.CbT, d.cb_dtype = ptr(cb), ptr(cbT), dt(cb if cb is not None else cbT)
+    return d, out, y
+
+
+def wprod_table(descs):
+    lib = _lib.load_mside()
+    tiles, forms = [], []
+    for d in descs:
+        form = C.c_int(0)
+        n = lib.vtx_wprod_tiles(C.byref(d), C.byref(form))
+        if n < 0:
+            _lib.mside_check(n, 'vtx_wprod_tiles')
+        tiles.append(n)
+        forms.append(form.value)
+    order = sorted(range(len(descs)), key=lambda i: forms[i])
+    table = (_lib.WprodDesc * len(descs))()
+    tile_start = [0]
+    for k, i in enumerate(order):
+        C.memmove(C.byref(table, k * C.sizeof(_lib.WprodDesc)), C.byref(descs[i]), C.sizeof(_lib.WprodDesc))
+        tile_start.append(tile_start[-1] + tiles[i])
+    return order, table, tile_start, [forms[i] for i in order]
+
+
+def _upload_bytes(blob, device):
+    import numpy as np
+    blob = blob + b'\0' * (-len(blob) % 4)
+    return upload_f32(torch.from_numpy(np.frombuffer(bytearray(blob), dtype=np.float32)), device)
+
+
+_wprod_tables = {}
+_WPROD_KEEP = 4
+
+
+def wprod_table_cached(slot, descs, device, upload=_upload_bytes):
+    import struct
+    _, table, tile_start, _ = wprod_table(descs)
+    key = (bytes(table), str(device))
+    kept = _wprod_tables.setdefault(slot, {})
+    hit = kept.pop(key, None)
+    if hit is None:
+        hit = (upload(key[0], device), upload(struct.pack(f'{len(tile_start)}i', *tile_start), device), len(descs), tile_start[-1])
+        while len(kept) >= _WPROD_KEEP:
+            del kept[next(iter(kept))]
+    kept[key] = hit
+    return hit
+
+
+def wprod_batch(slot, descs, device):
+    tab_dev, starts_dev, n, n_tiles = wprod_table_cached(slot, descs, device)
+    fl = sum(2.0 * d.N1 * d.N2 * d.K for d in descs)
+    nb = sum(4.0 * (d.N1 * d.K + d.K * d.N2 + d.N1 * d.N2) for d in descs)
+    with _timed('wprod', fl, nb, f'batch{n}x{descs[0].N1}x{descs[0].N2}x{descs[0].K}'):
+        _lib.mside_call('vtx_wprod_batch', ptr(tab_dev), ptr(starts_dev), n, n_tiles, stream())
+
+
+def merged_u(cs, part, c, db=None):
+    need_cuda(cs, part, db)
+    D = cs.numel()
+    u = torch.empty(D, dtype=torch.float32, device=cs.device)
+    _lib.mside_call('vtx_merged_u', D, ptr(_f32(cs)), ptr(_f32(part)), part.shape[0], float(c), ptr(u), ptr(_f32(db)), stream())
+    return u
+
+
+def wprod(A, B, ta=False, tb=False, out=None, alpha=1.0, accumulate=False, u=None, v=None, x=None, y=None, alpha_y=1.0,
+          z=None, beta_z=0.0, y_accumulate=False, cb=None, cbT=None, want_out=True):
+    d, out, y = wprod_desc(A, B, ta, tb, out, alpha, accumulate, u, v, x, y, alpha_y, z, beta_z, y_accumulate, cb, cbT, want_out)
+    K = d.K
     with _timed('wprod', 2.0 * d.N1 * d.N2 * K, 4.0 * (d.N1 * K + K * d.N2 + d.N1 * d.N2), f'{d.N1}x{d.N2}x{K}'):
         call('vtx_wprod', C.byref(d), stream())
     return out if x is None else (out, y)
diff --git a/videotransformer-pytorch_amd/vtx/optim.py b/videotransformer-pytorch_amd/vtx/optim.py
--- a/videotransformer-pytorch_amd/vtx/optim.py
+++ b/videotransformer-pytorch_amd/vtx/optim.py
@@ -123,6 +123,7 @@
         from . import functions
         functions.restage_weights([p for g in self.param_groups for p in g['params']
                                    if p.grad is not None and p.ndim >= 2 and id(p) not in self._skipped])
+        functions.restage_merged()
         return loss
 
     def _bump_versions(self):
```
